# rapidsai/cuvs

Measured on AMD Instinct MI355X. Metric: QPS @ recall@10>=0.9, 100Mx128 fp32 IVF-PQ, batch=10k, higher is better.
Workload: dtype u8 codes, f16 LUT, f32 score; 1 GPU; IVF-PQ 100000000x128 fp32, pq_dim=64 pq_bits=8 n_lists=16384 n_probes=128 batch=10000 k=10; rows and held-out queries from bench.gen_rows (seed 1234 / 4321): Gaussian mixture of 65536 modes ~ N(0, I) in a 32-d latent space, spread 0.35 per mode, embedded in R^128 by a fixed random map + N(0, 0.03^2 I) - NOT SURVEY 8d's generator: the same step on that one is the top-level entry contract_corpus (--; parallelism=single GPU, lut_dtype=f16, internal_distance_dtype=f32

## Files before the change

### cuvs_amd/csrc/ivf_common.hpp

```cpp
#pragma once
#include "ops.hpp"
#include "device_utils.hpp"

#include <algorithm>
#include <functional>
#include <vector>

namespace cuvs_amd {
namespace {

struct work_item {
  uint32_t list;
  uint32_t first;
  uint32_t count;
  uint32_t pad;
};

__global__ __launch_bounds__(1024) void count_items_kernel(const uint32_t* __restrict__ pair_off, int n_lists,
                                                           int qpb_lo, uint32_t* __restrict__ item_off, int split,
                                                           int qpb_hi)
{
  __shared__ int smem[17];
  const int per = (n_lists + 1023) / 1024;
  const int b = threadIdx.x * per, e = min(n_lists, b + per);
  auto items_of = [&](int i) {
    const int qpb = i < split ? qpb_lo : qpb_hi;
    return ((int)(pair_off[i + 1] - pair_off[i]) + qpb - 1) / qpb;
  };
  int s = 0;
  for (int i = b; i < e; ++i) s += items_of(i);
  int total;
  int run = block_exclusive_scan(s, smem, &total);
  for (int i = b; i < e; ++i) {
    item_off[i] = (uint32_t)run;
    run += items_of(i);
  }
  if (threadIdx.x == 0) item_off[n_lists] = (uint32_t)total;
}

__global__ void fill_items_kernel(const uint32_t* __restrict__ pair_off, const uint32_t* __restrict__ item_off,
                                  int n_lists, int qpb_lo, work_item* __restrict__ items, int split, int qpb_hi)
{
  int L = blockIdx.x * blockDim.x + threadIdx.x;
  if (L >= n_lists) return;
  const int qpb = L < split ? qpb_lo : qpb_hi;
  uint32_t b = pair_off[L], e = pair_off[L + 1];
  uint32_t w = item_off[L];
  for (uint32_t p = b; p < e; p += qpb, ++w) {
    work_item it;
    it.list  = (uint32_t)L;
    it.first = p;
    it.count = min((uint32_t)qpb, e - p);
    it.pad   = 0;
    items[w] = it;
  }
}

__global__ void phase_labels_kernel(const uint32_t* __restrict__ probes, int64_t n_pairs, uint32_t n_probes,
                                    uint32_t head, uint32_t n_lists, uint32_t* __restrict__ out,
                                    uint32_t shard_world = 1, uint32_t shard_rank = 0, uint32_t skip = 0,
                                    const int32_t* __restrict__ owner = nullptr, bool head_in_tail = false)
{
  for (int64_t p = (int64_t)blockIdx.x * blockDim.x + threadIdx.x; p < n_pairs; p += (int64_t)gridDim.x * blockDim.x) {
    const uint32_t L = probes[p];
    const bool mine  = shard_world <= 1 || (owner != nullptr ? (uint32_t)owner[L] == shard_rank : L % shard_world == shard_rank);
    out[p] = !mine ? skip : L + ((((uint32_t)(p % n_probes) < head && !head_in_tail) || head == 0) ? 0u : n_lists);
  }
}

template <int E>
struct wave_top {
  float d[E];
  uint32_t i[E];
  __device__ inline void init()
  {
#pragma unroll
    for (int e = 0; e < E; ++e) { d[e] = INFINITY; i[e] = 0xffffffffu; }
  }
  __device__ inline float rank_d(int r) const
  {
    float v = 0.f;
#pragma unroll
    for (int e = 0; e < E; ++e)
      if ((r >> 6) == e) v = __uint_as_float(__builtin_amdgcn_readlane(__float_as_uint(d[e]), r & 63));
    return v;
  }
  __device__ inline uint32_t rank_i(int r) const
  {
    uint32_t v = 0;
#pragma unroll
    for (int e = 0; e < E; ++e)
      if ((r >> 6) == e) v = __builtin_amdgcn_readlane(i[e], r & 63);
    return v;
  }
  __device__ inline void insert(float cd, uint32_t ci, int lane)
  {
    int pos = 0;
#pragma unroll
    for (int e = 0; e < E; ++e) {
      bool le = (d[e] < cd) || (d[e] == cd && i[e] <= ci);
      pos += __popcll(__ballot(le));
    }
    uint32_t carry_d = 0, carry_i = 0;
#pragma unroll
    for (int e = 0; e < E; ++e) {
      const uint32_t du   = __float_as_uint(d[e]);
      const uint32_t up_d = (uint32_t)__builtin_amdgcn_update_dpp((int)carry_d, (int)du, 0x138, 0xf, 0xf, false);
      const uint32_t up_i = (uint32_t)__builtin_amdgcn_update_dpp((int)carry_i, (int)i[e], 0x138, 0xf, 0xf, false);
      carry_d = __builtin_amdgcn_readlane(du, 63);
      carry_i = __builtin_amdgcn_readlane(i[e], 63);
      const int rank = e * 64 + lane;
      if (rank > pos) { d[e] = __uint_as_float(up_d); i[e] = up_i; }
      else if (rank == pos) { d[e] = cd; i[e] = ci; }
    }
  }
};


__device__ inline void wave_sort64(float& d, uint32_t& i, const int lane)
{
#pragma unroll
  for (int k2 = 2; k2 <= 64; k2 <<= 1) {
#pragma unroll
    for (int j2 = k2 >> 1; j2 > 0; j2 >>= 1) {
      const float od    = __shfl_xor(d, j2, 64);
      const uint32_t oi = (uint32_t)__shfl_xor((int)i, j2, 64);
      const bool other_less = (od < d) || (od == d && oi < i);
      const bool same       = od == d && oi == i;
      const bool take_min   = ((lane & j2) == 0) == ((lane & k2) == 0);
      if (take_min ? other_less : (!other_less && !same)) { d = od; i = oi; }
    }
  }
}

__global__ void pair_segments_kernel(const uint32_t* __restrict__ probes, const uint32_t* __restrict__ list_sizes,
                                     int64_t nq, uint32_t n_probes, uint32_t* __restrict__ seg)
{
  const int64_t q = (int64_t)blockIdx.x * blockDim.x + threadIdx.x;
  if (q >= nq) return;
  uint32_t off = 0;
  for (uint32_t p = 0; p < n_probes; ++p) {
    seg[q * n_probes + p] = off;
    off += list_sizes[probes[q * n_probes + p]];
  }
}

inline size_t largest_lists_total(const std::vector<uint32_t>& sizes, uint32_t n_probes)
{
  std::vector<uint32_t> s(sizes);
  const size_t m = std::min<size_t>(n_probes, s.size());
  std::partial_sort(s.begin(), s.begin() + m, s.end(), std::greater<uint32_t>());
  size_t t = 0;
  for (size_t i = 0; i < m; ++i) t += s[i];
  return t;
}

constexpr int kSegCap = 2048;

__global__ __launch_bounds__(256) void pair_histogram_kernel(const uint32_t* __restrict__ labels, int64_t n, uint32_t* __restrict__ counts,
                                                             uint32_t n_plain, uint32_t n_labels)
{
  __shared__ uint32_t bulk;
  if (threadIdx.x == 0) bulk = 0u;
  __syncthreads();
  uint32_t mine = 0u;
  for (int64_t i = (int64_t)blockIdx.x * blockDim.x + threadIdx.x; i < n; i += (int64_t)gridDim.x * blockDim.x) {
    const uint32_t L = labels[i];
    if (L < n_plain) atomicAdd(&counts[L], 1u);
    else             ++mine;
  }
  if (n_plain >= n_labels) return;
  for (int o = 32; o > 0; o >>= 1) mine += __shfl_down(mine, o, 64);
  if ((threadIdx.x & 63) == 0 && mine != 0u) atomicAdd(&bulk, mine);
  __syncthreads();
  if (threadIdx.x == 0 && bulk != 0u) atomicAdd(&counts[n_plain], bulk);
}
__global__ __launch_bounds__(1024) void pair_scan_kernel(const uint32_t* __restrict__ counts, int n, uint32_t* __restrict__ offsets)
{
  __shared__ int smem[17];
  const int per = (n + 1023) / 1024;
  const int b = threadIdx.x * per, e = min(n, b + per);
  int s = 0;
  for (int i = b; i < e; ++i) s += (int)counts[i];
  int total;
  int run = block_exclusive_scan(s, smem, &total);
  for (int i = b; i < e; ++i) {
    const int c = (int)counts[i];
    offsets[i] = (uint32_t)run;
    run += c;
  }
  if (threadIdx.x == 0) offsets[n] = (uint32_t)total;
}
__global__ void pair_scatter_kernel(const uint32_t* __restrict__ labels, int64_t n, const uint32_t* __restrict__ offsets,
                                    uint32_t* __restrict__ cursor, uint32_t* __restrict__ out, uint32_t n_plain)
{
  const int64_t i = (int64_t)blockIdx.x * blockDim.x + threadIdx.x;
  if (i >= n) return;
  const uint32_t L = labels[i];
  if (L >= n_plain) return;
  out[offsets[L] + atomicAdd(&cursor[L], 1u)] = (uint32_t)i;
}
__global__ __launch_bounds__(256) void sort_segments_kernel(const uint32_t* __restrict__ offsets, uint32_t n_labels,
                                                            uint32_t* __restrict__ pairs)
{
  __shared__ uint32_t seg_all[4][kSegCap];
  const uint32_t L = blockIdx.x * 4u + (threadIdx.x >> 6);
  if (L >= n_labels) return;
  const int lane   = threadIdx.x & 63;
  const uint32_t b = offsets[L], n = offsets[L + 1] - b;
  if (n <= 1u || n > (uint32_t)kSegCap) return;
  uint32_t* seg = seg_all[threadIdx.x >> 6];
  for (uint32_t i = lane; i < n; i += 64u) seg[i] = pairs[b + i];
  __builtin_amdgcn_fence(__ATOMIC_ACQ_REL, "wavefront");
  __builtin_amdgcn_wave_barrier();
  for (uint32_t i = lane; i < n; i += 64u) {
    const uint32_t v = seg[i];
    uint32_t rank = 0u;
    for (uint32_t j = 0; j < n; ++j) rank += seg[j] < v ? 1u : 0u;
    pairs[b + rank] = v;
  }
}
constexpr uint32_t kBitmapQueries = 1u << 19;

__global__ __launch_bounds__(1024) void sort_big_segments_kernel(const uint32_t* __restrict__ offsets, uint32_t n_labels,
                                                                 uint32_t* __restrict__ pairs, uint32_t* __restrict__ tmp,
                                                                 uint32_t n_probes, uint32_t n_queries)
{
  extern __shared__ __attribute__((aligned(16))) uint32_t sb_smem[];
  __shared__ uint32_t big[1024];
  __shared__ uint32_t n_big;
  __shared__ int scan_smem[17];
  const bool bitmap_ok = n_probes != 0u && n_queries <= kBitmapQueries;
  const uint32_t words = (n_queries + 31u) / 32u;
  const uint32_t per = (n_labels + gridDim.x - 1) / gridDim.x;
  const uint32_t l0 = blockIdx.x * per, l1 = min(n_labels, l0 + per);
  for (uint32_t base = l0; base < l1; base += 1024u) {
    if (threadIdx.x == 0) n_big = 0u;
    __syncthreads();
    const uint32_t Lc = base + threadIdx.x;
    if (Lc < l1 && offsets[Lc + 1] - offsets[Lc] > (uint32_t)kSegCap) big[atomicAdd(&n_big, 1u)] = Lc;
    __syncthreads();
    const uint32_t nb = n_big;
    for (uint32_t w = 0; w < nb; ++w) {
      const uint32_t L = big[w];
      const uint32_t b = offsets[L], n = offsets[L + 1] - b;
      if (bitmap_ok) {
        uint32_t* bits = sb_smem;
        uint32_t* pref = sb_smem + words;
        for (uint32_t i = threadIdx.x; i < words; i += 1024u) bits[i] = 0u;
        __syncthreads();
        for (uint32_t i = threadIdx.x; i < n; i += 1024u) {
          const uint32_t q = pairs[b + i] / n_probes;
          atomicOr(&bits[q >> 5], 1u << (q & 31u));
        }
        __syncthreads();
        const uint32_t run = (words + 1023u) / 1024u, w0 = threadIdx.x * run, w1 = min(words, w0 + run);
        int sum = 0;
        for (uint32_t i = w0; i < w1; ++i) sum += __popc(bits[i]);
        int total;
        int acc = block_exclusive_scan(sum, scan_smem, &total);
        for (uint32_t i = w0; i < w1; ++i) { pref[i] = (uint32_t)acc; acc += __popc(bits[i]); }
        __syncthreads();
        for (uint32_t i = threadIdx.x; i < n; i += 1024u) {
          const uint32_t p = pairs[b + i], q = p / n_probes;
          tmp[b + pref[q >> 5] + (uint32_t)__popc(bits[q >> 5] & ((1u << (q & 31u)) - 1u))] = p;
        }
      } else {
        uint32_t* tile = sb_smem;
        for (uint32_t i0 = 0; i0 < n; i0 += 1024u) {
          const uint32_t i = i0 + threadIdx.x;
          const uint32_t v = i < n ? pairs[b + i] : 0xffffffffu;
          uint32_t rank = 0u;
          for (uint32_t t0 = 0; t0 < n; t0 += 4096u) {
            __syncthreads();
            for (uint32_t t = threadIdx.x; t < 4096u; t += 1024u) tile[t] = t0 + t < n ? pairs[b + t0 + t] : 0xffffffffu;
            __syncthreads();
            const uint32_t m = min(4096u, n - t0);
            for (uint32_t j = 0; j < m; ++j) rank += tile[j] < v ? 1u : 0u;
          }
          if (i < n) tmp[b + rank] = v;
        }
      }
      __syncthreads();
      for (uint32_t i = threadIdx.x; i < n; i += 1024u) pairs[b + i] = tmp[b + i];
      __syncthreads();
    }
    __syncthreads();
  }
}

inline void group_pairs(resources& res, const uint32_t* labels, int64_t n, uint32_t n_labels, uint32_t* sorted_pairs, uint32_t* pair_off,
                        uint32_t* cursor, uint32_t* tmp, uint32_t n_sorted, uint32_t n_probes, int64_t n_queries)
{
  CUVS_EXPECTS(n < (int64_t(1) << 32), "group_pairs: more than 2^32 pairs");
  HIP_TRY(hipMemsetAsync(cursor, 0, (size_t)n_labels * sizeof(uint32_t), res.stream));
  n_sorted = std::min(n_sorted, n_labels);
  CUVS_EXPECTS(n_sorted + 1u >= n_labels, "group_pairs: at most one bulk label");
  hipLaunchKernelGGL(pair_histogram_kernel, dim3((unsigned)std::min<int64_t>(grid_blocks(n, 256), 2048)), dim3(256), 0, res.stream, labels, n,
                     cursor, n_sorted, n_labels);
  hipLaunchKernelGGL(pair_scan_kernel, dim3(1), dim3(1024), 0, res.stream, cursor, (int)n_labels, pair_off);
  HIP_TRY(hipMemsetAsync(cursor, 0, (size_t)n_labels * sizeof(uint32_t), res.stream));
  hipLaunchKernelGGL(pair_scatter_kernel, dim3(grid_blocks(n, 256)), dim3(256), 0, res.stream, labels, n, pair_off, cursor, sorted_pairs, n_sorted);
  hipLaunchKernelGGL(sort_segments_kernel, dim3(grid_blocks(n_sorted, 4)), dim3(256), 0, res.stream, pair_off, n_sorted, sorted_pairs);
  const bool bitmap   = n_probes != 0u && n_queries <= (int64_t)kBitmapQueries;
  const size_t sbytes = bitmap ? (size_t)2 * ((n_queries + 31) / 32) * sizeof(uint32_t) : (size_t)4096 * sizeof(uint32_t);
  HIP_TRY(hipFuncSetAttribute(reinterpret_cast<const void*>(sort_big_segments_kernel), hipFuncAttributeMaxDynamicSharedMemorySize,
                              (int)std::max<size_t>(sbytes, 16384)));
  hipLaunchKernelGGL(sort_big_segments_kernel, dim3(64), dim3(1024), std::max<size_t>(sbytes, 16384), res.stream, pair_off, n_sorted,
                     sorted_pairs, tmp, n_probes, (uint32_t)std::min<int64_t>(n_queries, 0xffffffff));
  HIP_TRY(hipGetLastError());
}

inline void build_work_items(resources& res, const uint32_t* probes, int64_t n_pairs, uint32_t n_lists, int qpb,
                             uint32_t* sorted_pairs, uint32_t* pair_off, uint32_t* item_off, work_item* items,
                             int split = -1, int qpb_hi = 0, uint32_t* group_scratch = nullptr, uint32_t n_sorted = 0xffffffffu,
                             uint32_t n_probes = 0, int64_t n_queries = 0)
{
  if (split < 0) { split = (int)n_lists; qpb_hi = qpb; }
  if (group_scratch != nullptr)
    group_pairs(res, probes, n_pairs, n_lists, sorted_pairs, pair_off, group_scratch, group_scratch + n_lists + 1, n_sorted, n_probes, n_queries);
  else                          group_by_label(res, probes, n_pairs, n_lists, sorted_pairs, pair_off);
  const int n_item_labels = (int)std::min(n_lists, n_sorted);
  hipLaunchKernelGGL(count_items_kernel, dim3(1), dim3(1024), 0, res.stream, pair_off, n_item_labels, qpb, item_off,
                     split, qpb_hi);
  hipLaunchKernelGGL(fill_items_kernel, dim3(grid_blocks(n_item_labels, 256)), dim3(256), 0, res.stream, pair_off,
                     item_off, n_item_labels, qpb, items, split, qpb_hi);
}

}
template <int NT>
__device__ inline void merge_sorted_lists(float* __restrict__ d, uint32_t* __restrict__ id, const int n_l, const int kp2,
                                          const int tid)
{
  auto less = [](const float da, const uint32_t ia, const float db, const uint32_t ib) {
    return da < db || (da == db && ia < ib);
  };
  for (int w = 1; w < n_l; w <<= 1) {
    const int pairs = n_l / (2 * w);
    for (int t = tid; t < pairs * kp2; t += NT) {
      const int pr = t / kp2, r = t % kp2;
      const int ia = pr * 2 * w * kp2 + r, ib = (pr * 2 * w + w) * kp2 + (kp2 - 1 - r);
      const float da = d[ia], db = d[ib];
      const uint32_t xa = id[ia], xb = id[ib];
      if (less(db, xb, da, xa)) { d[ia] = db; id[ia] = xb; }
    }
    __syncthreads();
    for (int stride = kp2 >> 1; stride > 0; stride >>= 1) {
      for (int t = tid; t < pairs * (kp2 >> 1); t += NT) {
        const int pr = t / (kp2 >> 1), x = t % (kp2 >> 1);
        const int lo = pr * 2 * w * kp2 + 2 * x - (x & (stride - 1)), hi = lo + stride;
        const float da = d[lo], db = d[hi];
        const uint32_t xa = id[lo], xb = id[hi];
        if (less(db, xb, da, xa)) { d[lo] = db; id[lo] = xb; d[hi] = da; id[hi] = xa; }
      }
      __syncthreads();
    }
  }
}

}
```

### cuvs_amd/csrc/ivf_pq_filter4.hip

```cpp
#include "ivf_pq_filter_common.hpp"

#include <cfloat>
#include <type_traits>

namespace cuvs_amd {

namespace {

struct bprep_params {
  const uint32_t* sorted_pairs;
  const uint32_t* pair_off;
  uint32_t n_lists;
  uint32_t lbase;
  const uint32_t* probes;
  const float* rot_queries;
  const float* centers_rot;
  const uint32_t* query_kth;
  uint32_t* qflag;
  uint4* bq;
  float* thr;
  uint32_t n_probes, rot_dim;
  float sc, c1, eps, alpha, cbmax, dmax, bound_max;
  int is_ip, flat;
  uint32_t lpl;
  float4* norms;
};

template <int NST, int PART>
__global__ __launch_bounds__(256) void pq_bprep_kernel(const bprep_params a)
{
  constexpr uint32_t LPP = 2 * NST <= 2 ? 2u : 2 * NST <= 4 ? 4u : 2 * NST <= 8 ? 8u : 2 * NST <= 16 ? 16u : 32u;
  constexpr uint32_t PPW = 64u / LPP;
  const uint32_t s_base = a.pair_off[a.lbase], s_end = a.pair_off[a.lbase + a.n_lists];
  const uint32_t lane = threadIdx.x & 63u, slot = lane % LPP, st = slot >> 1, h = slot & 1u;
  const uint32_t w0 = (blockIdx.x * 4u + (threadIdx.x >> 6)) * 32u;
  if (s_base + w0 >= s_end) return;
  const uint32_t d0 = ((16u * (st >> a.lpl) + 8u * h) << a.lpl) + 8u * (st & ((1u << a.lpl) - 1u));
#pragma unroll 2
  for (uint32_t pass = 0; pass < 32u / PPW; ++pass) {
    const uint32_t s  = s_base + w0 + pass * PPW + lane / LPP;
    const bool pair_ok = s < s_end;
    const bool valid  = pair_ok && slot < 2u * NST;
    const uint32_t p  = a.sorted_pairs[pair_ok ? s : s_end - 1u];
    const uint32_t q  = p / a.n_probes, L = a.probes[p];
    float rn = 0.f, big = 0.f, qc = 0.f, cn = 0.f;
    if (valid) {
      const float* rq = a.rot_queries + (size_t)q * a.rot_dim + d0;
      const float* ct = a.centers_rot + (size_t)L * a.rot_dim + d0;
      const float4 q0 = *reinterpret_cast<const float4*>(rq), q1 = *reinterpret_cast<const float4*>(rq + 4);
      float r[8] = {q0.x, q0.y, q0.z, q0.w, q1.x, q1.y, q1.z, q1.w};
      const float4 c0 = *reinterpret_cast<const float4*>(ct), c1 = *reinterpret_cast<const float4*>(ct + 4);
      const float c[8] = {c0.x, c0.y, c0.z, c0.w, c1.x, c1.y, c1.z, c1.w};
      if (!a.is_ip) {
#pragma unroll
        for (int e = 0; e < 8; ++e) r[e] -= c[e];
      } else {
#pragma unroll
        for (int e = 0; e < 8; ++e) { qc = __fmaf_rn(r[e], c[e], qc); cn = __fmaf_rn(c[e], c[e], cn); }
      }
      f16x8_t v;
#pragma unroll
      for (int e = 0; e < 8; ++e) {
        rn   = __fmaf_rn(r[e], r[e], rn);
        const float x = a.sc * r[e];
        big  = fmaxf(big, fabsf(x));
        v[e] = (_Float16)fminf(fmaxf(x, -60000.f), 60000.f);
      }
      a.bq[(size_t)(s - s_base) * NST * 2 + slot] = __builtin_bit_cast(uint4, v);
    }
#pragma unroll
    for (uint32_t o = 1; o < LPP; o <<= 1) {
      rn += __shfl_xor(rn, o); qc += __shfl_xor(qc, o); cn += __shfl_xor(cn, o);
      big = fmaxf(big, __shfl_xor(big, o));
    }
    if (!pair_ok || slot != 0u) continue;
    if constexpr (PART == 1) {
      a.norms[s - s_base] = make_float4(rn, cn, qc, big);
    } else {
      const uint32_t kk = a.query_kth[q];
      const float bound = key_to_float(kk);
      const bool served = kk < 0xff800000u && big < 60000.f && fabsf(bound) <= a.bound_max;
      if (!a.flat && !served) a.qflag[q] = 1u;
      const float t = a.is_ip ? filter_threshold_ip(bound, rn, cn, qc, a) : filter_threshold(bound, rn, a);
      a.thr[s - s_base] = served ? t / a.c1 : (a.flat ? -INFINITY : INFINITY);
    }
  }
}

__global__ __launch_bounds__(256) void pq_thr_kernel(const bprep_params a)
{
  const uint32_t s_base = a.pair_off[a.lbase], s_end = a.pair_off[a.lbase + a.n_lists];
  const uint32_t s = s_base + blockIdx.x * 256u + threadIdx.x;
  if (s >= s_end) return;
  const uint32_t q  = a.sorted_pairs[s] / a.n_probes;
  const float4 nm   = a.norms[s - s_base];
  const float rn = nm.x, cn = nm.y, qc = nm.z, big = nm.w;
  const uint32_t kk = a.query_kth[q];
  const float bound = key_to_float(kk);
  const bool served = kk < 0xff800000u && big < 60000.f && fabsf(bound) <= a.bound_max;
  if (!a.flat && !served) a.qflag[q] = 1u;
  const float t = a.is_ip ? filter_threshold_ip(bound, rn, cn, qc, a) : filter_threshold(bound, rn, a);
  a.thr[s - s_base] = served ? t / a.c1 : (a.flat ? -INFINITY : INFINITY);
}

constexpr int kF4Threads = 256;
constexpr uint32_t kSurvChunk = 256u;

struct filter4_params {
  const filter_unit* units;
  const uint32_t* n_units;
  uint32_t* xcd_ticket;
  const uint32_t* sorted_pairs;
  const uint32_t* pair_off;
  uint32_t n_lists;
  const uint4* bq;
  const float* thr;
  const uint32_t* cb16;
  const uint8_t* codes;
  const uint32_t* list_offsets;
  const uint32_t* list_sizes;
  const float* row_term;
  uint32_t* qflag;
  uint2* surv;
  uint32_t* surv_cnt;
  uint32_t n_chunks, n_probes, unit_rows;
  unsigned long long* stats;
  uint32_t strided;
// ... 485 lines not shown
```

### cuvs_amd/csrc/ivf_pq_scan3.hip

```cpp
#include "ivf_pq.hpp"
#include "ops.hpp"
#include "device_utils.hpp"
#include "ivf_common.hpp"
#include "pq_lut_math.hpp"
#include "ivf_pq_scan3.hpp"
#include "ivf_pq_filter_common.hpp"

#include <cfloat>
#include <cmath>
#include <cstring>
#include <map>
#include <mutex>
#include <type_traits>
#include <utility>

namespace cuvs_amd {

namespace {

constexpr int kFThreads = 512;
constexpr int kFWaves   = kFThreads / 64;



// ... 3 lines not shown
  const uint32_t e = blockIdx.x * blockDim.x + threadIdx.x;
  if (e >= pq_dim * 256u) return;
  const uint32_t s = e >> 8, code = e & 255u;
  for (uint32_t l = 0; l < pq_len; ++l)
    cb16[(size_t)e * pq_len + l] =
      code < book ? __builtin_bit_cast(uint16_t, (_Float16)(sc * pq_centers[(size_t)(s * pq_len + l) * book + code])) : (uint16_t)0;
}

__global__ void cbt_kernel(const float* __restrict__ pq_centers, uint32_t pq_dim, uint32_t pq_len, uint32_t book, float* __restrict__ cbt)
{
  const uint32_t e = blockIdx.x * blockDim.x + threadIdx.x;
  if (e >= pq_dim * 256u) return;
  const uint32_t s = e >> 8, code = e & 255u;
  for (uint32_t l = 0; l < pq_len; ++l) cbt[(size_t)e * pq_len + l] = code < book ? pq_centers[(size_t)(s * pq_len + l) * book + code] : 0.f;
}

__global__ void expand_codes_kernel(const uint8_t* __restrict__ codes, int64_t rows, uint32_t n_chunks, uint32_t cpc, uint32_t bits,
                                    uint32_t pq_dim, uint8_t* __restrict__ out)
{
  const uint32_t nch8 = pq_dim / 16;
  const int64_t i = (int64_t)blockIdx.x * blockDim.x + threadIdx.x;
  if (i >= rows * nch8) return;
  const int64_t row = i / nch8;
  const uint32_t c8 = (uint32_t)(i % nch8);
  uint32_t w[4] = {0u, 0u, 0u, 0u};
#pragma unroll
  for (int b = 0; b < 16; ++b) {
    const uint32_t s = c8 * 16 + b, ch = s / cpc, bit = (s % cpc) * bits;
    const uint8_t* base = codes + ((size_t)(row >> 6) * n_chunks + ch) * 1024 + (size_t)(row & 63) * 16;
    uint32_t v = base[bit >> 3];
    if ((bit & 7) + bits > 8) v |= (uint32_t)base[(bit >> 3) + 1] << 8;
    w[b >> 2] |= ((v >> (bit & 7)) & ((1u << bits) - 1u)) << ((b & 3) * 8);
  }
  reinterpret_cast<uint4*>(out)[((size_t)(row >> 6) * nch8 + c8) * 64 + (row & 63)] = make_uint4(w[0], w[1], w[2], w[3]);
}

__device__ inline float wave_reduce_max_f32(float v)
{
#pragma unroll
  for (int off = 32; off > 0; off >>= 1) v = fmaxf(v, __shfl_xor(v, off));
  return v;
}

__global__ void row_term_kernel(const uint8_t* __restrict__ codes, const float* __restrict__ pq_centers, int64_t rows, float sc,
                                uint32_t* __restrict__ term, uint32_t* __restrict__ dn_max_bits, int n_chunks, int fp32, int pq_len,
                                uint32_t book, const uint32_t* __restrict__ list_offsets, uint32_t n_lists)
{
  const int64_t r0 = (int64_t)blockIdx.x * blockDim.x + threadIdx.x;
  const int64_t r  = min(r0, rows - 1);
  uint32_t L = 0u;
  if (list_offsets != nullptr) {
    uint32_t lo = 0u, hi = n_lists;
    while (hi - lo > 1u) {
      const uint32_t mid = (lo + hi) >> 1;
      if ((int64_t)list_offsets[mid] <= r) lo = mid; else hi = mid;
    }
    L = lo;
  }
  const uint4* cp = reinterpret_cast<const uint4*>(codes) + ((size_t)(r >> 6) * n_chunks) * 64 + (r & 63);
  float dn = 0.f;
  for (int c = 0; c < n_chunks; ++c) {
    const uint4 cw       = cp[c * 64];
    const uint32_t ws[4] = {cw.x, cw.y, cw.z, cw.w};
#pragma unroll
    for (int b = 0; b < 16; ++b) {
      const uint32_t code = (ws[b >> 2] >> ((b & 3) * 8)) & 0xffu;
      const uint32_t s    = c * 16 + b;
      for (int l = 0; l < pq_len; ++l) {
        const float p = pq_centers[(size_t)((list_offsets != nullptr ? L : s) * pq_len + l) * book + code];
        dn = __fmaf_rn(p, p, dn);
      }
    }
  }
  const float wmax = wave_reduce_max_f32(dn);
  if ((threadIdx.x & 63) == 0) atomicMax(dn_max_bits, __float_as_uint(wmax));
  const float x     = -0.5f * sc * sc * (dn * (1.0f - 1.0f / 512.0f));
  const _Float16 hi = (_Float16)x;
  const _Float16 lo = (_Float16)(x - (float)hi);
  if (r0 < rows)
    term[r] = fp32 ? __float_as_uint(x) : ((uint32_t)__builtin_bit_cast(uint16_t, hi) | ((uint32_t)__builtin_bit_cast(uint16_t, lo) << 16));
}


__global__ __launch_bounds__(1024) void count_units_kernel(const uint32_t* __restrict__ pair_off, uint32_t n_lists,
                                                           const uint32_t* __restrict__ list_sizes, uint32_t unit_rows,
                                                           uint32_t* __restrict__ unit_off, uint32_t group, uint32_t lbase)
{
  __shared__ int smem[17];
  const uint32_t per = (n_lists + 1023u) / 1024u;
  const uint32_t b = threadIdx.x * per, e = min(n_lists, b + per);
  auto units_of = [&](uint32_t i) {
    const uint32_t np = pair_off[lbase + i + 1] - pair_off[lbase + i];
    const uint32_t len = list_sizes[i];
    return (int)(((np + group - 1u) / group) * ((len + unit_rows - 1u) / unit_rows));
  };
  int s = 0;
  for (uint32_t i = b; i < e; ++i) s += units_of(i);
  int total;
  int run = block_exclusive_scan(s, smem, &total);
  for (uint32_t i = b; i < e; ++i) {
    unit_off[i] = (uint32_t)run;
    run += units_of(i);
  }
  if (threadIdx.x == 0) unit_off[n_lists] = (uint32_t)total;
}

__global__ void fill_units_kernel(const uint32_t* __restrict__ pair_off, uint32_t n_lists,
                                  const uint32_t* __restrict__ list_offsets, const uint32_t* __restrict__ list_sizes,
                                  uint32_t unit_rows, const uint32_t* __restrict__ unit_off, filter_unit* __restrict__ units,
                                  uint32_t group, uint32_t lbase)
{
  const uint32_t L = blockIdx.x * blockDim.x + threadIdx.x;
  if (L >= n_lists) return;
  const uint32_t b = pair_off[lbase + L], e = pair_off[lbase + L + 1], len = list_sizes[L];
  uint32_t w = unit_off[L];
  if (b == e || len == 0u) return;
  const uint32_t n_ch = (len + unit_rows - 1u) / unit_rows;
  const uint32_t rows = ((len + n_ch - 1u) / n_ch + 63u) & ~63u;
  const uint32_t base = list_offsets[L];
  for (uint32_t c = 0; c < n_ch; ++c) {
    const uint32_t r0 = c * rows, r1 = min(len, r0 + rows);
    if (r0 >= r1) continue;
    for (uint32_t p = b; p < e; p += group) units[w++] = filter_unit{L, p, min(group, e - p), r0, base, r1, 0u, 0u};
  }
  const uint32_t w_end = unit_off[L] + ((e - b + group - 1u) / group) * n_ch;
  for (; w < w_end; ++w) units[w] = filter_unit{L, b, 1u, 0u, base, 0u, 0u, 0u};
}

constexpr uint32_t kOrdWaves = 8u, kOrdThreads = 64u * kOrdWaves;
__global__ __launch_bounds__(512) __attribute__((amdgpu_waves_per_eu(6, 8))) void order_units_kernel(const filter_unit* __restrict__ in, const uint32_t* __restrict__ n_units,
                                                           filter_unit* __restrict__ out, uint32_t unit_rows, int order)
{
  __shared__ uint32_t cnt[kOrdWaves][kUnitKeys];
  __shared__ uint32_t head_pos[kOrdWaves];
  __shared__ int scan_smem[17];
  __shared__ uint32_t k_star_s;
  const uint32_t n = *n_units;
  const uint32_t lane = threadIdx.x & 63u, w = threadIdx.x >> 6;
  const uint32_t per = (n + kOrdWaves * 64u - 1u) / (kOrdWaves * 64u) * 64u;
  const uint32_t b = min(n, w * per), e = min(n, b + per);
  for (uint32_t i = threadIdx.x; i < kOrdWaves * kUnitKeys; i += kOrdThreads) (&cnt[0][0])[i] = 0u;
  if (threadIdx.x == 0) k_star_s = order == 1 ? kUnitKeys : 0u;
  __syncthreads();
  auto key_of = [&](const uint4 d0, const uint2 d1) {
    return unit_cost_key(d1.y > d0.w ? d1.y - d0.w : 0u, (d0.z + 31u) >> 5, unit_rows);
  };
  constexpr uint32_t kOrdAhead = 4u;
  static_assert(kUnitKeys <= kOrdThreads, "a thread per key in the scan of the costs");
  for (uint32_t i0 = b; i0 < e; i0 += 64u * kOrdAhead) {
    uint4 d0[kOrdAhead];
    uint2 d1[kOrdAhead];
#pragma unroll
    for (uint32_t j = 0; j < kOrdAhead; ++j) {
      const uint32_t i = min(i0 + j * 64u + lane, e - 1u);
      d0[j] = *reinterpret_cast<const uint4*>(in + i);
      d1[j] = *reinterpret_cast<const uint2*>(reinterpret_cast<const char*>(in + i) + 16);
    }
#pragma unroll
    for (uint32_t j = 0; j < kOrdAhead; ++j)
      if (i0 + j * 64u + lane < e) atomicAdd(&cnt[w][key_of(d0[j], d1[j])], 1u);
  }
  __syncthreads();
  {
    int v = 0;
    if (threadIdx.x < kUnitKeys)
      for (uint32_t ww = 0; ww < kOrdWaves; ++ww) v += (int)(cnt[ww][threadIdx.x] * threadIdx.x);
    if (n > (1u << 21)) v = 0;
    int total;
    const int below = block_exclusive_scan(v, scan_smem, &total);
    if (order == 2 && n <= (1u << 21) && threadIdx.x < kUnitKeys && (long long)below * 8 <= (long long)total)
      atomicMax(&k_star_s, threadIdx.x);
    __syncthreads();
  }
  const uint32_t k_star = k_star_s;
  {
    uint32_t s = 0;
    for (uint32_t key = lane; key < kUnitKeys; key += 64u) s += key >= k_star ? cnt[w][key] : 0u;
    for (uint32_t o = 32u; o > 0u; o >>= 1) s += __shfl_xor(s, o);
    if (lane == 0) head_pos[w] = s;
  }
  __syncthreads();
  {
    constexpr uint32_t kPer = (kOrdWaves + kOrdWaves * kUnitKeys + kOrdThreads - 1u) / kOrdThreads;
    uint32_t vals[kPer];
    int sum = 0;
#pragma unroll
// ... 1714 lines not shown

struct head_params {
  const work_item* items;
  const uint32_t* item_begin;
  const uint32_t* item_end;
  uint32_t n_lists;
  uint32_t* xcd_ticket;
  const uint32_t* sorted_pairs;
  const float* rot_queries;
  const float* centers_rot;
  const float* pq_centers;
  const uint8_t* codes;
  const uint32_t* list_offsets;
  const uint32_t* list_sizes;
  float* out_d;
  uint32_t* out_i;
  uint32_t* query_kth;
  uint32_t n_probes, rot_dim, k, cap_rows, pq_dim, n_chunks, pq_len, book;
  int is_ip, per_cluster;
  int hcand;
  uint32_t row_limit;
  uint32_t one_shot;
  const uint32_t* filter_bits;
  const int64_t* indices;
  unsigned long long* stats;
};

static inline int head_cand(int k) { return k <= 128 ? 512 : 1024; }

constexpr int kHeadRowsPerThread = 16;
constexpr int kHeadGroups16      = 2;

template <int B>
__device__ __forceinline__ uint32_t code_byte_x2(uint32_t w)
{
  uint32_t r;
  if constexpr (B == 0) asm("v_lshlrev_b32_sdwa %0, %1, %2 dst_sel:DWORD dst_unused:UNUSED_PAD src0_sel:DWORD src1_sel:BYTE_0" : "=v"(r) : "s"(1u), "v"(w));
  if constexpr (B == 1) asm("v_lshlrev_b32_sdwa %0, %1, %2 dst_sel:DWORD dst_unused:UNUSED_PAD src0_sel:DWORD src1_sel:BYTE_1" : "=v"(r) : "s"(1u), "v"(w));
  if constexpr (B == 2) asm("v_lshlrev_b32_sdwa %0, %1, %2 dst_sel:DWORD dst_unused:UNUSED_PAD src0_sel:DWORD src1_sel:BYTE_2" : "=v"(r) : "s"(1u), "v"(w));
  if constexpr (B == 3) asm("v_lshlrev_b32_sdwa %0, %1, %2 dst_sel:DWORD dst_unused:UNUSED_PAD src0_sel:DWORD src1_sel:BYTE_3" : "=v"(r) : "s"(1u), "v"(w));
  return r;
}

template <int LUT, bool ACC_HALF, int NT, int WPE>
__global__ __launch_bounds__(NT) __attribute__((amdgpu_waves_per_eu(WPE, WPE))) void pq_head_kernel(const head_params a)
{
  constexpr bool LUT32 = LUT == 0 || (LUT == 2 && !ACC_HALF);
  using lut_t = std::conditional_t<LUT32, float, _Float16>;
  extern __shared__ __attribute__((aligned(16))) char smem[];
  lut_t* lut      = reinterpret_cast<lut_t*>(smem);
  float* rv       = reinterpret_cast<float*>(smem + (size_t)a.pq_dim * 256 * sizeof(lut_t));
  float* cv       = rv + 256;
  unsigned long long* min64 = reinterpret_cast<unsigned long long*>(cv + 256);
  int* ctrl       = reinterpret_cast<int*>(min64 + 2);
  work_item& cur  = *reinterpret_cast<work_item*>(ctrl + 8);
  uint32_t* tk    = reinterpret_cast<uint32_t*>(ctrl + 12);
  const int kHCand = a.hcand;
  uint2* cand     = reinterpret_cast<uint2*>(tk + NT);
  static_assert(sizeof(work_item) == 16, "work_item");

  const int tid = threadIdx.x;
  const uint32_t item0   = (a.one_shot == 0u && a.item_begin) ? *a.item_begin : 0u;
  const uint32_t n_items = a.one_shot != 0u ? a.one_shot : *a.item_end - item0;
  const uint32_t xcd = blockIdx.x & 7u, chunk = (n_items + 7u) / 8u;
  const uint32_t share0 = min(n_items, xcd * chunk), share_len = min(chunk, n_items - share0);
  const work_item* share = a.items + item0 + share0;
  const uint4* codes16   = reinterpret_cast<const uint4*>(a.codes);
  float one = 1.0f;
  asm("" : "+s"(one));

  for (uint32_t round = 0;; ++round) {
    __syncthreads();
    if (tid == 0) {
      if (a.one_shot != 0u) {
        cur = (round == 0u && blockIdx.x < a.one_shot) ? a.items[blockIdx.x] : work_item{0u, 0u, 0u, 0xffffffffu};
      } else {
        const uint32_t t = atomicAdd(a.xcd_ticket + xcd * 32, 1u);
        cur = t < share_len ? share[t] : work_item{0u, 0u, 0u, 0xffffffffu};
      }
    }
    __syncthreads();
    const work_item item = cur;
    if (item.pad == 0xffffffffu) break;
    if (item.count == 0u) continue;
    unsigned long long t_prev = a.stats != nullptr ? __builtin_readcyclecounter() : 0ull;
    auto phase = [&](int which) {
      if (a.stats != nullptr && tid == 0) {
        const unsigned long long t = __builtin_readcyclecounter();
        atomicAdd(&a.stats[which], t - t_prev);
        t_prev = t;
      }
    };
    const uint32_t L        = item.list >= a.n_lists ? item.list - a.n_lists : item.list;
    const uint32_t base_row = a.list_offsets[L], len = a.row_limit != 0u ? min(a.list_sizes[L], a.row_limit) : a.list_sizes[L];
    const uint32_t pair     = a.sorted_pairs[item.first];
    const uint32_t q        = pair / a.n_probes;
    if (tid < (int)a.rot_dim) {
      const float c = a.centers_rot[(size_t)L * a.rot_dim + tid];
      float v       = a.rot_queries[(size_t)q * a.rot_dim + tid];
      if (!a.is_ip) v -= c;
      rv[tid] = v;
      cv[tid] = c;
    }
    __syncthreads();
    phase(0);
    constexpr int LB = 16;
#pragma unroll 1
    for (uint32_t e0 = tid; e0 < ((a.pq_len == 2u && !a.per_cluster) ? a.pq_dim * 256u : 0u); e0 += (uint32_t)LB * NT) {
      float p0[LB], p1[LB];
#pragma unroll
      for (int j = 0; j < LB; ++j) {
        const uint32_t e = min(e0 + (uint32_t)j * NT, a.pq_dim * 256u - 1u), sb = e >> 8, code = min(e & 255u, a.book - 1u);
        p0[j] = a.pq_centers[(size_t)(sb * 2 + 0) * a.book + code];
        p1[j] = a.pq_centers[(size_t)(sb * 2 + 1) * a.book + code];
      }
#pragma unroll
      for (int j = 0; j < LB; ++j) {
        const uint32_t e = e0 + (uint32_t)j * NT, sb = e >> 8;
        if (e >= a.pq_dim * 256u) break;
        const float q0 = rv[sb * 2], q1 = rv[sb * 2 + 1];
        float v;
        if (!a.is_ip) {
          const float d0 = q0 - p0[j], d1 = q1 - p1[j];
          v = __fmaf_rn(d1, d1, __fmaf_rn(d0, d0, 0.f));
        } else {
          v = __fmaf_rn(-q0, cv[sb * 2], 0.f);
          v = __fmaf_rn(-q0, p0[j], v);
          v = __fmaf_rn(-q1, cv[sb * 2 + 1], v);
          v = __fmaf_rn(-q1, p1[j], v);
        }
        if constexpr (LUT == 2) v = fp8_round_trip<std::conditional_t<ACC_HALF, __half, float>>(v, a.is_ip != 0);
        if constexpr (LUT32) lut[e] = v; else lut[e] = to_lut_half(v);
      }
    }
    if (a.pq_len != 2u || a.per_cluster) {
#pragma unroll 1
      for (uint32_t e0 = tid; e0 < a.pq_dim * 256u; e0 += 4u * NT) {
        float v[4] = {0.f, 0.f, 0.f, 0.f};
        for (uint32_t l = 0; l < a.pq_len; ++l) {
          float p[4];
#pragma unroll
          for (int j = 0; j < 4; ++j) {
            const uint32_t e = min(e0 + (uint32_t)j * NT, a.pq_dim * 256u - 1u), sb = e >> 8, code = min(e & 255u, a.book - 1u);
            p[j] = a.pq_centers[(size_t)((a.per_cluster ? L : sb) * a.pq_len + l) * a.book + code];
          }
#pragma unroll
          for (int j = 0; j < 4; ++j) {
            const uint32_t e = min(e0 + (uint32_t)j * NT, a.pq_dim * 256u - 1u), dd = (e >> 8) * a.pq_len + l;
            const float qv = rv[dd];
            if (!a.is_ip) {
              const float d = qv - p[j];
              v[j] = __fmaf_rn(d, d, v[j]);
            } else {
              v[j] = __fmaf_rn(-qv, cv[dd], v[j]);
              v[j] = __fmaf_rn(-qv, p[j], v[j]);
            }
          }
        }
#pragma unroll
        for (int j = 0; j < 4; ++j) {
          const uint32_t e = e0 + (uint32_t)j * NT;
          if (e >= a.pq_dim * 256u) break;
          float x = v[j];
          if constexpr (LUT == 2) x = fp8_round_trip<std::conditional_t<ACC_HALF, __half, float>>(x, a.is_ip != 0);
          if constexpr (LUT32) lut[e] = x; else lut[e] = to_lut_half(x);
        }
      }
    }
    if (tid == 0) ctrl[0] = 0;
    __syncthreads();
    phase(1);
    const int k = (int)a.k;
    int buf = 0;
    auto key_of = [&](uint32_t v) __attribute__((always_inline)) -> uint32_t {
      const uint32_t fr = base_row + v;
      const uint4* cp   = codes16 + ((size_t)(fr >> 6) * a.n_chunks) * 64 + (fr & 63u);
      float af    = 0.f;
      _Float16 ah = (_Float16)0.f;
// ... 379 lines not shown
}

bool pq3_bound_useful(const ivf_pq_index& idx, int k)
{
  uint64_t rows = 0, lists = 0;
  if (idx.shard_world > 1 && idx.shard_comm != nullptr) {
    if (!idx.shard_stats_valid) return k <= 128;
    rows = idx.shard_global_rows; lists = idx.shard_global_lists;
  } else {
    for (uint32_t v : idx.h_list_sizes) { rows += v; lists += v != 0u; }
  }
  return lists != 0 && (uint64_t)k * 25u * lists <= rows;
}

static std::recursive_mutex g_pq3_mu;

const uint8_t* pq3_codes(resources& res, const ivf_pq_index& idx, uint32_t* n_chunks)
{
  *n_chunks = idx.pq_dim / 16;
  if (idx.pq_bits == 8) return idx.codes.data();
  std::lock_guard<std::recursive_mutex> lock(g_pq3_mu);
  auto& c = idx.scan3;
  if (c.codes8_src != idx.codes.data() || c.codes8_rows != idx.padded_rows || c.codes8_size != idx.size) {
    const int64_t rows = std::max<int64_t>(idx.padded_rows, 1);
    c.codes8 = dev_buf<uint8_t>::persistent((size_t)rows * idx.pq_dim);
    if (idx.padded_rows > 0)
      hipLaunchKernelGGL(expand_codes_kernel, dim3(grid_blocks(idx.padded_rows * (int64_t)(idx.pq_dim / 16), 256)), dim3(256), 0, res.stream,
                         idx.codes.data(), idx.padded_rows, idx.n_chunks, idx.codes_per_chunk, idx.pq_bits, idx.pq_dim, c.codes8.data());
    c.codes8_src = idx.codes.data(); c.codes8_rows = idx.padded_rows; c.codes8_size = idx.size;
  }
  return c.codes8.data();
}

pq3_tables pq3_prepare(resources& res, const ivf_pq_index& idx, const bool term_fp32)
{
  std::lock_guard<std::recursive_mutex> lock(g_pq3_mu);
  auto& c = idx.scan3;
  if (c.codes_ptr != idx.codes.data() || c.rows != idx.padded_rows || c.size != idx.size || c.pq_ptr != idx.pq_centers.data() ||
      c.term_fp32 != term_fp32) {
    std::vector<float> h = to_host(res, idx.pq_centers.data(), idx.pq_centers.size());
    float mx = 0.f;
    for (float v : h) mx = std::max(mx, std::fabs(v));
    c.sc    = mx > 0.f ? std::exp2(std::floor(std::log2(16.0f / mx))) : 1.0f;
    c.cbmax = mx;
    const uint32_t n_tables = idx.codebook_kind == 0 ? idx.pq_dim : idx.n_lists;
    c.cb16  = dev_buf<uint32_t>::persistent((size_t)n_tables * 256 * idx.pq_len / 2 + 1);
    hipLaunchKernelGGL(cb16_kernel, dim3(grid_blocks((int64_t)n_tables * 256, 256)), dim3(256), 0, res.stream,
                       idx.pq_centers.data(), n_tables, idx.pq_len, idx.pq_book, c.sc, reinterpret_cast<uint16_t*>(c.cb16.data()));
    c.row_term = dev_buf<uint32_t>::persistent((size_t)std::max<int64_t>(idx.padded_rows, 1));
    dev_buf<uint32_t> mxd(res, 1);
    HIP_TRY(hipMemsetAsync(mxd.data(), 0, sizeof(uint32_t), res.stream));
    uint32_t nch8 = 0;
    const uint8_t* codes8 = pq3_codes(res, idx, &nch8);
    if (idx.padded_rows > 0)
      hipLaunchKernelGGL(row_term_kernel, dim3(grid_blocks(idx.padded_rows, 256)), dim3(256), 0, res.stream, codes8,
                         idx.pq_centers.data(), idx.padded_rows, c.sc, c.row_term.data(), mxd.data(), (int)nch8, term_fp32 ? 1 : 0,
                         (int)idx.pq_len, idx.pq_book, idx.codebook_kind == 0 ? nullptr : idx.list_offsets.data(), idx.n_lists);
    const uint32_t mbits = to_host(res, mxd.data(), 1)[0];
    float dn_max;
    memcpy(&dn_max, &mbits, 4);
    c.dmax = std::sqrt(dn_max) * 1.0001f;
    c.codes_ptr = idx.codes.data(); c.rows = idx.padded_rows; c.size = idx.size; c.pq_ptr = idx.pq_centers.data();
    c.term_fp32 = term_fp32;
  }
  return pq3_tables{c.cb16.data(), c.row_term.data(), c.sc, c.cbmax, c.dmax};
}

size_t pq3_max_units(const ivf_pq_index& idx, int64_t n_pairs, uint32_t* unit_rows, bool filter4)
{
  uint32_t max_len = 0;
  for (uint32_t v : idx.h_list_sizes) max_len = std::max(max_len, v);
  const uint32_t ur = std::max<uint32_t>(filter4 ? 8192u : 4096u, (uint32_t)round_up((int64_t)(max_len + 15) / 16, 64));
  *unit_rows = ur;
  return (size_t)16 * ((size_t)n_pairs / 32 + idx.n_lists + 1);
}

void pq3_warm(resources& res, const ivf_pq_index& idx, bool filter4)
{
  uint32_t n_chunks = 0;
  (void)pq3_codes(res, idx, &n_chunks);
  (void)pq3_prepare(res, idx, filter4);
}

void pq3_tail(resources& res, const ivf_pq_index& idx, const pq3_run& r)
{
  const bool f4 = r.bq != nullptr;
  CUVS_EXPECTS(r.stage == 0 || f4, "ivf_pq: the two-stream schedule is pq_filter4_kernel's");
  const pq3_tables tb = pq3_prepare(res, idx, f4);
  if (r.stage != 1) profile_begin(res, "pq_scan_kernel");
  const int nch        = (int)idx.pq_dim / 16;
  const int nst        = nch * (int)idx.pq_len;
  const uint32_t group = f4 ? (nst <= 8 ? 128u : 64u) : (nch <= 4 ? 64u : 32u);
  CUVS_EXPECTS(f4 || (idx.pq_len == 2 && idx.codebook_kind == 0), "ivf_pq: pq_filter_kernel decodes pq_len 2, PER_SUBSPACE only");
  auto* units = static_cast<filter_unit*>(r.units);
  if (r.stage != 2) {
    hipLaunchKernelGGL(count_units_kernel, dim3(1), dim3(1024), 0, res.stream, r.pair_off, idx.n_lists, idx.list_sizes.data(),
                       r.unit_rows, r.unit_off, group, idx.n_lists);
    hipLaunchKernelGGL(fill_units_kernel, dim3(grid_blocks(idx.n_lists, 256)), dim3(256), 0, res.stream, r.pair_off, idx.n_lists,
                       idx.list_offsets.data(), idx.list_sizes.data(), r.unit_rows, r.unit_off, units, group, idx.n_lists);
  }
  const bool ordered = r.unit_order != 0 && r.units_ord != nullptr;
  if (ordered) {
    if (r.stage != 2)
      hipLaunchKernelGGL(order_units_kernel, dim3(1), dim3(kOrdThreads), 0, res.stream, units, r.unit_off + idx.n_lists,
                         static_cast<filter_unit*>(r.units_ord), r.unit_rows, r.unit_order);
    units = static_cast<filter_unit*>(r.units_ord);
  }
  filter_params f{};
  f.units = units; f.n_units = r.unit_off + idx.n_lists; f.xcd_ticket = r.xcd_ticket; f.strided = ordered ? 1u : 0u;
  f.sorted_pairs = r.sorted_pairs; f.rot_queries = r.rot_queries; f.centers_rot = idx.centers_rot.data();
  uint32_t nch8 = 0;
  const uint8_t* codes8 = pq3_codes(res, idx, &nch8);
  f.cb16 = tb.cb16; f.codes = codes8; f.list_offsets = idx.list_offsets.data(); f.list_sizes = idx.list_sizes.data();
  f.row_term = r.is_ip ? nullptr : tb.row_term; f.query_kth = r.query_kth; f.qflag = r.qflag;
  const unsigned grid = pq3_grid(res);
  const unsigned regions = grid;
  f.surv = static_cast<uint2*>(r.surv); f.surv_cnt = r.surv_cnt; f.surv_cap = (uint32_t)((uint64_t)r.surv_cap * 3 / 4 / regions);
  f.spill_cap = r.surv_cap - f.surv_cap * regions;
  f.n_probes = r.n_probes; f.rot_dim = idx.rot_dim; f.unit_rows = r.unit_rows;
  f.sc = tb.sc; f.c1 = (r.is_ip ? -1.0f : -2.0f) / (tb.sc * tb.sc);
  f.cbmax = tb.cbmax; f.dmax = tb.dmax; f.is_ip = r.is_ip; f.stats = r.stats; f.dbg = r.filter_dbg;
  f.bound_max = FLT_MAX;
  const float ne = std::max(1.0f, (float)idx.pq_dim / 64.0f);
  if (r.lut_mode == 0)      { f.eps = ne / 65536.0f; f.alpha = 0.f; }
  else if (r.lut_mode == 1) { f.eps = r.acc_half ? 0.04f * ne : 1.0f / 1024.0f; f.alpha = ne * 64.0f / 16777216.0f; f.bound_max = 60000.f; }
  else                      { f.eps = r.acc_half ? 0.07f + 0.04f * ne : 0.07f; f.alpha = ne * 64.0f / 32768.0f; f.bound_max = 30000.f; }
  if (r.is_ip && r.lut_mode == 2) f.eps = r.acc_half ? 0.14f + 0.04f * ne : 0.14f;
  const size_t fsmem = (size_t)nch * 16 * 1024 + 16;
  if (f4) {
    filter4_launch l{};
    l.units = units; l.n_units = f.n_units; l.xcd_ticket = r.xcd_ticket; l.sorted_pairs = r.sorted_pairs; l.pair_off = r.pair_off;
    l.n_lists = idx.n_lists; l.probes = r.probes; l.rot_queries = r.rot_queries; l.centers_rot = f.centers_rot;
    l.query_kth = r.query_kth; l.qflag = r.qflag; l.bq = r.bq; l.thr = r.thr; l.cb16 = tb.cb16; l.codes = f.codes;
    l.list_offsets = f.list_offsets; l.list_sizes = f.list_sizes; l.row_term = reinterpret_cast<const float*>(f.row_term);
    l.surv = f.surv; l.surv_cnt = f.surv_cnt; l.surv_entries = r.surv_cap; l.n_probes = r.n_probes;
    l.rot_dim = idx.rot_dim; l.unit_rows = r.unit_rows; l.sc = f.sc; l.c1 = f.c1; l.eps = f.eps; l.alpha = f.alpha;
    l.cbmax = f.cbmax; l.dmax = f.dmax; l.bound_max = f.bound_max; l.is_ip = r.is_ip; l.dbg = r.filter_dbg; l.nch = nch;
    l.pl = (int)idx.pq_len; l.per_cluster = idx.codebook_kind != 0 ? 1 : 0;
    l.n_pairs = r.nq * (int64_t)r.n_probes; l.stats = r.stats; l.grid = grid;
    l.stage = r.stage; l.pair_norms = r.pair_norms; l.strided = ordered ? 1 : 0;
    pq4_filter(res, l);
    if (r.stage == 1) return;
  } else {
  auto launch_filter = [&](auto kern) {
    HIP_TRY(hipFuncSetAttribute(reinterpret_cast<const void*>(kern), hipFuncAttributeMaxDynamicSharedMemorySize, (int)fsmem));
    profile_begin(res, "pq_filter_kernel");
    hipLaunchKernelGGL(kern, dim3(grid), dim3(kFThreads), fsmem, res.stream, f);
    profile_end(res, "pq_filter_kernel");
  };
  if (nch == 4) {
    switch (r.filter_dbg) {
      case 1:  launch_filter(pq_filter_kernel<4, 1>); break;
      case 2:  launch_filter(pq_filter_kernel<4, 2>); break;
      case 4:  launch_filter(pq_filter_kernel<4, 4>); break;
      default: launch_filter(pq_filter_kernel<4, 0>); break;
    }
  } else {
    switch (nch) {
      case 1: launch_filter(pq_filter_kernel<1, 0>); break;
      case 2: launch_filter(pq_filter_kernel<2, 0>); break;
      case 3: launch_filter(pq_filter_kernel<3, 0>); break;
      case 5: launch_filter(pq_filter_kernel<5, 0>); break;
      case 6: launch_filter(pq_filter_kernel<6, 0>); break;
      case 7: launch_filter(pq_filter_kernel<7, 0>); break;
      default: launch_filter(pq_filter_kernel<8, 0>); break;
    }
  }
  }

  rescore_params s{};
  s.surv = f.surv; s.surv_cnt = r.surv_cnt; s.surv_cap = f.surv_cap; s.spill_cap = f.spill_cap; s.probes = r.probes; s.rot_queries = r.rot_queries;
  s.n_regions = regions; s.sub = f4 ? 0u : 1u;
  if (f4) s.surv_cap = r.surv_cap;
  s.centers_rot = idx.centers_rot.data(); s.pq_centers = idx.pq_centers.data(); s.codes = codes8;
  s.query_kth = r.query_kth; s.qflag = r.qflag; s.qcnt = r.qcnt; s.cand_d = r.cand_d; s.cand_i = r.cand_i; s.cand_r = r.cand_r;
  s.n_probes = r.n_probes; s.rot_dim = idx.rot_dim; s.k = r.k; s.head = r.head; s.is_ip = r.is_ip; s.n_chunks = nch8;
  s.head_rows = r.head_rows; s.list_offsets = idx.list_offsets.data();
  s.filter_bits = r.filter_bits; s.indices = idx.indices.data();
  s.overflow = static_cast<uint4*>(r.overflow); s.overflow_cnt = r.counters + 1; s.overflow_cap = r.overflow_cap; s.fail = nullptr;
  const size_t cb_bytes = (size_t)idx.rot_dim * idx.pq_book * sizeof(float);
  s.pq_len = idx.pq_len; s.book = idx.pq_book; s.per_cluster = idx.codebook_kind != 0 ? 1 : 0;
  s.cb_lds = (cb_bytes <= 128 * 1024 && !s.per_cluster) ? 1 : 0;
  const size_t rsmem = s.cb_lds ? cb_bytes : 16;
  const dim3 rg(f4 && s.cb_lds ? grid : grid + 1, f4 && s.cb_lds ? 1 : 2), rb(kRThreads);
  profile_begin(res, "pq_rescore_kernel");
  auto launch_rescore = [&](auto kern) {
    HIP_TRY(hipFuncSetAttribute(reinterpret_cast<const void*>(kern), hipFuncAttributeMaxDynamicSharedMemorySize, (int)rsmem));
    hipLaunchKernelGGL(kern, rg, rb, rsmem, res.stream, s);
  };
  auto pick_rescore = [&](auto lut_tag, auto acc_tag) {
    constexpr int LUT = decltype(lut_tag)::value;
    constexpr bool ACC = decltype(acc_tag)::value;
    if (s.cb_lds) launch_rescore(pq_rescore_kernel<LUT, ACC, true>); else launch_rescore(pq_rescore_kernel<LUT, ACC, false>);
  };
  using L0 = std::integral_constant<int, 0>; using L1 = std::integral_constant<int, 1>; using L2 = std::integral_constant<int, 2>;
  if (r.lut_mode == 0)      pick_rescore(L0{}, std::false_type{});
  else if (r.lut_mode == 1) { if (r.acc_half) pick_rescore(L1{}, std::true_type{}); else pick_rescore(L1{}, std::false_type{}); }
  else                      { if (r.acc_half) pick_rescore(L2{}, std::true_type{}); else pick_rescore(L2{}, std::false_type{}); }
  profile_end(res, "pq_rescore_kernel");
  hipLaunchKernelGGL(reset_flagged_kernel, dim3((unsigned)r.nq), dim3(256), 0, res.stream, r.qflag, r.nq, r.n_probes, r.k, r.head,
                     r.cand_d, r.cand_i);
  hipLaunchKernelGGL(fallback_items_kernel, dim3(grid * 4), dim3(256), 0, res.stream, r.sorted_pairs, r.pair_off, idx.n_lists,
                     r.probes, r.n_probes, r.qflag, static_cast<work_item*>(r.fb_items), r.counters, 0);
  profile_end(res, "pq_scan_kernel");
}

static size_t head_smem_fixed(const ivf_pq_index& idx, int lut_mode, bool acc_half, int nt, int k)
{
  const bool lut32 = lut_mode == 0 || (lut_mode == 2 && !acc_half);
  return (size_t)idx.pq_dim * 256 * (lut32 ? 4 : 2) + 2 * 256 * 4 + 16 + 32 + 16 + (size_t)nt * 4 + 4 * (size_t)head_cand(k) * 4;
}

static int head_occupancy(const void* fn, int nt, size_t smem)
{
  static std::mutex mu;
  static std::map<std::pair<const void*, size_t>, int> known;
  std::lock_guard<std::mutex> lock(mu);
  auto it = known.find({fn, smem});
  if (it != known.end()) return it->second;
  hipFuncAttributes fa{};
  HIP_TRY(hipFuncGetAttributes(&fa, fn));
  CUVS_EXPECTS(fa.sharedSizeBytes == 0, "ivf_pq: the head kernel's LUT has to sit at LDS address 0");
  int n = 0;
  HIP_TRY(hipOccupancyMaxActiveBlocksPerMultiprocessor(&n, fn, nt, smem));
  CUVS_EXPECTS(n >= 1, "ivf_pq: the head kernel does not fit a CU");
  known[{fn, smem}] = n;
  return n;
}

int pq3_head_scan(resources& res, const ivf_pq_index& idx, const pq3_head& h)
{
  head_params a{};
  a.items = static_cast<const work_item*>(h.items); a.item_begin = h.item_begin; a.item_end = h.item_end; a.n_lists = idx.n_lists;
  a.xcd_ticket = h.xcd_ticket; a.sorted_pairs = h.sorted_pairs; a.rot_queries = h.rot_queries; a.centers_rot = idx.centers_rot.data();
  a.pq_centers = idx.pq_centers.data(); a.codes = pq3_codes(res, idx, &a.n_chunks); a.list_offsets = idx.list_offsets.data();
  a.list_sizes = idx.list_sizes.data(); a.out_d = h.cand_d; a.out_i = h.cand_i; a.query_kth = h.query_kth;
  a.n_probes = h.n_probes; a.rot_dim = idx.rot_dim; a.k = h.k; a.is_ip = h.is_ip; a.pq_dim = idx.pq_dim;
  a.pq_len = idx.pq_len; a.book = idx.pq_book; a.per_cluster = idx.codebook_kind != 0 ? 1 : 0;
  a.filter_bits = h.filter_bits; a.indices = idx.indices.data(); a.stats = h.stats; a.hcand = head_cand((int)h.k);
  const bool lut32 = h.lut_mode == 0 || (h.lut_mode == 2 && !h.acc_half);
  const size_t lut_bytes = (size_t)idx.pq_dim * 256 * (lut32 ? 4 : 2);
  const bool nt512 = lut_bytes <= 64 * 1024;
  const int nt = nt512 ? 512 : 1024;
  const size_t smem = head_smem_fixed(idx, h.lut_mode, h.acc_half != 0, nt, (int)h.k);
  CUVS_EXPECTS(smem <= 160 * 1024 - 64, "ivf_pq: the head-phase LUT does not fit the LDS");
  a.cap_rows = (uint32_t)(kHeadRowsPerThread * nt);
  if (h.max_list_len > 0) a.cap_rows = std::min<uint32_t>(a.cap_rows, (uint32_t)round_up(h.max_list_len, 64));
  a.one_shot          = h.one_shot;
  a.row_limit         = h.row_limit;
  int wgs_per_cu = 0;
  auto go = [&](auto kern) {
    const void* fn = reinterpret_cast<const void*>(kern);
    HIP_TRY(hipFuncSetAttribute(fn, hipFuncAttributeMaxDynamicSharedMemorySize, (int)smem));
    wgs_per_cu = head_occupancy(fn, nt, smem);
    const unsigned grid = h.one_shot != 0u ? h.one_shot : pq3_grid(res) * (unsigned)wgs_per_cu;
    profile_begin(res, "pq_scan_kernel");
    profile_begin(res, "pq_head_kernel");
    hipLaunchKernelGGL(kern, dim3(grid), dim3(nt), smem, res.stream, a);
    profile_end(res, "pq_head_kernel");
    profile_end(res, "pq_scan_kernel");
  };
  auto pick = [&](auto lut_tag, auto acc_tag) {
    constexpr int LUT = decltype(lut_tag)::value;
    constexpr bool ACC = decltype(acc_tag)::value;
    constexpr bool L32 = LUT == 0 || (LUT == 2 && !ACC);
    if (nt512) go(pq_head_kernel<LUT, ACC, 512, L32 ? 4 : 6>); else go(pq_head_kernel<LUT, ACC, 1024, 4>);
  };
  using I0 = std::integral_constant<int, 0>; using I1 = std::integral_constant<int, 1>; using I2 = std::integral_constant<int, 2>;
  if (h.lut_mode == 0)      pick(I0{}, std::false_type{});
  else if (h.lut_mode == 1) { if (h.acc_half) pick(I1{}, std::true_type{}); else pick(I1{}, std::false_type{}); }
  else                      { if (h.acc_half) pick(I2{}, std::true_type{}); else pick(I2{}, std::false_type{}); }
  return wgs_per_cu;
}

bool flat3_wide(uint32_t dim) { return dim > 128 && pqw_shape(dim); }
bool flat3_supported(uint32_t dim, int k) { return ((dim % 32 == 0 && dim >= 32 && dim <= 256) || flat3_wide(dim)) && k <= 128; }

static bool flat3_prepare(resources& res, const flat3_view& v, flat3_cache& c)
{
  static std::mutex mu;
  std::lock_guard<std::mutex> lock(mu);
  if (c.data_ptr == v.data && c.rows == v.padded_rows && c.size == v.size) return true;
  if (c.failed_ptr == v.data && c.failed_rows == v.padded_rows && c.failed_size == v.size) return false;
  const int64_t rows = std::max<int64_t>(v.padded_rows, 64);
  {
    c.rows16   = dev_buf<uint4>();
    c.row_term = dev_buf<uint32_t>();
    c.data_ptr = nullptr;
    size_t free_b = 0, total_b = 0;
    HIP_TRY(hipMemGetInfo(&free_b, &total_b));
    const size_t need = (size_t)rows * v.dim * 2 + (size_t)rows * 16 + (size_t(1) << 30);
    if (free_b < need) {
      scratch_cache_flush_all();
      HIP_TRY(hipMemGetInfo(&free_b, &total_b));
    }
    if (free_b < need) {
      c.failed_ptr = v.data; c.failed_rows = v.padded_rows; c.failed_size = v.size;
      return false;
    }
  }
  dev_buf<uint32_t> row_list(res, (size_t)rows / 64), mxd(res, 2);
  dev_buf<float> dn(res, (size_t)rows), inv_norm(res, v.unit_rows ? (size_t)rows : 0);
  HIP_TRY(hipMemsetAsync(row_list.data(), 0xff, row_list.bytes(), res.stream));
  HIP_TRY(hipMemsetAsync(mxd.data(), 0, 2 * sizeof(uint32_t), res.stream));
  hipLaunchKernelGGL(flat_group_lists_kernel, dim3(v.n_lists), dim3(64), 0, res.stream, v.list_offsets, v.list_sizes, v.n_lists,
                     row_list.data());
  c.rows16   = dev_buf<uint4>::persistent((size_t)rows / 32 * (v.dim / 16) * 64);
  c.row_term = dev_buf<uint32_t>::persistent((size_t)rows);
  const bool wide = flat3_wide(v.dim);
  c.row_term32 = wide ? dev_buf<float>::persistent((size_t)rows) : dev_buf<float>();
  c.zeros      = wide ? dev_buf<float>::persistent(32) : dev_buf<float>();
  if (wide) HIP_TRY(hipMemsetAsync(c.zeros.data(), 0, 32 * sizeof(float), res.stream));
  if (v.padded_rows > 0) {
    auto stats = [&](auto kern) {
      hipLaunchKernelGGL(kern, dim3(grid_blocks(v.padded_rows, 256)), dim3(256), 0, res.stream, v.data, v.centers, row_list.data(),
                         v.padded_rows, v.dim, v.n_chunks, dn.data(), mxd.data(), inv_norm.data());
    };
    switch (v.elem) {
      case 0: stats(flat_residual_stats_kernel<float>); break;
      case 1: stats(flat_residual_stats_kernel<__half>); break;
      case 2: stats(flat_residual_stats_kernel<int8_t>); break;
      default: stats(flat_residual_stats_kernel<uint8_t>); break;
    }
    const auto mbits = to_host(res, mxd.data(), 2);
    float mx, mn2;
    memcpy(&mx, &mbits[0], 4);
    memcpy(&mn2, &mbits[1], 4);
    c.maxnorm = std::sqrt(mn2) * (1.0f + 1e-6f);
    c.maxres = mx;
    c.sc     = mx > 0.f ? std::exp2(std::floor(std::log2(16.0f / mx))) : 1.0f;
    const int64_t n_t = v.padded_rows / 32 * (v.dim / 16) * 64;
    auto rows16 = [&](auto kern) {
      hipLaunchKernelGGL(kern, dim3(grid_blocks(n_t, 256)), dim3(256), 0, res.stream, v.data, v.centers, row_list.data(), dn.data(),
                         v.padded_rows, v.dim, v.n_chunks, c.sc, c.rows16.data(), c.row_term.data(), inv_norm.data(), wide ? 1 : 0,
                         wide ? c.row_term32.data() : nullptr);
    };
    switch (v.elem) {
      case 0: rows16(flat_rows16_kernel<float>); break;
      case 1: rows16(flat_rows16_kernel<__half>); break;
      case 2: rows16(flat_rows16_kernel<int8_t>); break;
      default: rows16(flat_rows16_kernel<uint8_t>); break;
    }
  }
  sync(res);
  c.data_ptr = v.data; c.rows = v.padded_rows; c.size = v.size;
  return true;
}

bool flat3_head_bounds(resources& res, const flat3_view& v, flat3_cache& cache, const pq3_run& r, const flat3_head_bufs& hb)
{
  if (!flat3_prepare(res, v, cache)) return false;
  CUVS_EXPECTS(v.dim <= 128 && r.bq != nullptr && !r.is_ip, "ivf_flat: the bound-only head phase serves L2 up to 128 dimensions");
  profile_begin(res, "ivf_flat_scan_kernel");
  profile_begin(res, "flat_head_kernel");
  const float c1 = -2.0f / (cache.sc * cache.sc);
  hipLaunchKernelGGL(fill_f32_kernel, dim3(1024), dim3(256), 0, res.stream, hb.xbuf, (size_t)r.nq * hb.ldx, -INFINITY);
  filter4_launch l{};
  l.sorted_pairs = r.sorted_pairs; l.pair_off = r.pair_off; l.n_lists = v.n_lists; l.probes = r.probes;
  l.rot_queries = r.rot_queries; l.centers_rot = v.centers; l.query_kth = r.query_kth; l.qflag = r.qflag;
  l.bq = r.bq; l.thr = hb.thr_head; l.n_probes = r.n_probes; l.rot_dim = v.dim;
  l.sc = cache.sc; l.c1 = c1; l.eps = 1.0f / 65536.0f; l.alpha = 0.f; l.cbmax = cache.maxres; l.dmax = 0.f; l.bound_max = FLT_MAX;
  l.is_ip = 0; l.nch = (int)v.dim / 32; l.pl = 2; l.n_pairs = r.nq; l.flat = 1; l.head_labels = 1; l.stage = 1; l.pair_norms = hb.norms;
  pq4_filter(res, l);
  auto* units = static_cast<filter_unit*>(r.units);
  hipLaunchKernelGGL(count_units_kernel, dim3(1), dim3(1024), 0, res.stream, r.pair_off, v.n_lists, v.list_sizes, r.unit_rows, r.unit_off,
                     256u, 0u);
  hipLaunchKernelGGL(fill_units_kernel, dim3(grid_blocks(v.n_lists, 256)), dim3(256), 0, res.stream, r.pair_off, v.n_lists, v.list_offsets,
                     v.list_sizes, r.unit_rows, r.unit_off, units, 256u, 0u);
  filter_params f{};
  f.units = units; f.n_units = r.unit_off + v.n_lists; f.xcd_ticket = hb.tickets; f.sorted_pairs = r.sorted_pairs;
  f.list_offsets = v.list_offsets; f.list_sizes = v.list_sizes; f.row_term = cache.row_term.data(); f.rows16 = cache.rows16.data();
  f.bq = static_cast<const uint4*>(r.bq); f.pair_off = r.pair_off; f.n_lists = v.n_lists; f.lbase = 0u; f.xbuf = hb.xbuf; f.ldx = hb.ldx;
  f.n_probes = r.n_probes; f.rot_dim = v.dim; f.sc = cache.sc; f.c1 = c1;
  const unsigned grid = 2 * pq3_grid(res);
  auto launch_emit = [&](auto kern) {
    const size_t fsmem = (size_t)8 * (v.dim / 16) * 1024 + 2 * 8 * 32 * 4 + 16;
    HIP_TRY(hipFuncSetAttribute(reinterpret_cast<const void*>(kern), hipFuncAttributeMaxDynamicSharedMemorySize, (int)fsmem));
    hipLaunchKernelGGL(kern, dim3(grid), dim3(kF2Threads), fsmem, res.stream, f);
  };
  switch (v.dim / 16) {
    case 2:  launch_emit(flat_filter2_kernel<2, true>); break;
    case 4:  launch_emit(flat_filter2_kernel<4, true>); break;
    case 6:  launch_emit(flat_filter2_kernel<6, true>); break;
    default: launch_emit(flat_filter2_kernel<8, true>); break;
  }
  select_k<uint32_t, uint32_t>(res, hb.xbuf, nullptr, r.nq, (int64_t)hb.ldx, (int64_t)hb.ldx, (int)r.k, hb.kth_val, hb.kth_idx, false);
  head_bound_params b{};
  b.kth_val = hb.kth_val; b.kth_idx = hb.kth_idx; b.norms = static_cast<const float4*>(hb.norms); b.sorted_pairs = r.sorted_pairs;
  b.pair_off = r.pair_off; b.probes = r.probes; b.list_offsets = v.list_offsets; b.data = v.data;
  b.queries = r.rescore_queries != nullptr ? r.rescore_queries : r.rot_queries;
  b.n_lists = v.n_lists; b.n_probes = r.n_probes; b.k = r.k; b.dim = v.dim; b.n_chunks = v.n_chunks;
  b.sc = cache.sc; b.eps = l.eps; b.alpha = l.alpha; b.cbmax = cache.maxres; b.c1 = c1; b.rot_dim = v.dim;
  b.query_kth = const_cast<uint32_t*>(r.query_kth); b.thr_head = hb.thr_head; b.bound_max = FLT_MAX;
  const dim3 bgrid((unsigned)grid_blocks(r.nq, 4));
  switch (v.elem) {
    case 0: hipLaunchKernelGGL(flat_head_bound_kernel<float>, bgrid, dim3(256), 0, res.stream, b); break;
    case 1: hipLaunchKernelGGL(flat_head_bound_kernel<__half>, bgrid, dim3(256), 0, res.stream, b); break;
    case 2: hipLaunchKernelGGL(flat_head_bound_kernel<int8_t>, bgrid, dim3(256), 0, res.stream, b); break;
    default: hipLaunchKernelGGL(flat_head_bound_kernel<uint8_t>, bgrid, dim3(256), 0, res.stream, b); break;
  }
  profile_end(res, "flat_head_kernel");
  profile_end(res, "ivf_flat_scan_kernel");
  HIP_TRY(hipGetLastError());
  return true;
}

bool flat3_tail(resources& res, const flat3_view& v, flat3_cache& cache, const pq3_run& r)
{
  if (!flat3_prepare(res, v, cache)) return false;
  profile_begin(res, "ivf_flat_scan_kernel");
  const int nch        = (int)v.dim / 32;
  const bool f2        = res.tune.flat_filter2 != 0 && r.bq != nullptr && v.dim <= 128;
  const bool wide      = flat3_wide(v.dim);
  CUVS_EXPECTS(!wide || r.bq != nullptr, "ivf_flat: the wide filter needs the pre-pass buffers");
  const uint32_t group = wide ? pqw_group() : f2 ? 256u : (nch <= 4 ? 64u : 32u);
  auto* units = static_cast<filter_unit*>(r.units);
  hipLaunchKernelGGL(count_units_kernel, dim3(1), dim3(1024), 0, res.stream, r.pair_off, v.n_lists, v.list_sizes, r.unit_rows, r.unit_off,
                     group, v.n_lists);
  hipLaunchKernelGGL(fill_units_kernel, dim3(grid_blocks(v.n_lists, 256)), dim3(256), 0, res.stream, r.pair_off, v.n_lists, v.list_offsets,
                     v.list_sizes, r.unit_rows, r.unit_off, units, group, v.n_lists);
  const unsigned grid = (f2 && !wide) ? 2 * pq3_grid(res) : pq3_grid(res);
  filter_params f{};
  f.units = units; f.n_units = r.unit_off + v.n_lists; f.xcd_ticket = r.xcd_ticket;
  f.sorted_pairs = r.sorted_pairs; f.rot_queries = r.rot_queries; f.centers_rot = v.centers;
  f.codes = v.data; f.list_offsets = v.list_offsets; f.list_sizes = v.list_sizes;
  f.row_term = r.is_ip ? nullptr : cache.row_term.data(); f.query_kth = r.query_kth; f.qflag = r.qflag;
  f.surv = static_cast<uint2*>(r.surv); f.surv_cnt = r.surv_cnt; f.surv_cap = (uint32_t)((uint64_t)r.surv_cap * 3 / 4 / grid);
  f.spill_cap = r.surv_cap - f.surv_cap * grid;
  f.n_probes = r.n_probes; f.rot_dim = v.dim; f.unit_rows = r.unit_rows;
  f.sc = cache.sc; f.c1 = (r.is_ip ? -1.0f : -2.0f) / (cache.sc * cache.sc); f.cbmax = cache.maxres; f.dmax = r.is_ip ? cache.maxnorm : 0.f;
  f.is_ip = r.is_ip; f.stats = r.stats; f.dbg = r.filter_dbg;
  f.eps = 1.0f / 65536.0f; f.alpha = 0.f; f.bound_max = FLT_MAX;
  if (r.is_ip) f.eps = (float)v.dim * (1.0f / 4194304.0f);
  f.rows16 = cache.rows16.data(); f.fail = r.fail;
  auto launch_filter = [&](auto kern) {
    profile_begin(res, "flat_filter_kernel");
    hipLaunchKernelGGL(kern, dim3(grid), dim3(kFThreads), 16, res.stream, f);
    profile_end(res, "flat_filter_kernel");
  };
  auto launch_filter2 = [&](auto kern) {
    const size_t fsmem = (size_t)8 * (v.dim / 16) * 1024 + 2 * 8 * 32 * 4 + 16;
    HIP_TRY(hipFuncSetAttribute(reinterpret_cast<const void*>(kern), hipFuncAttributeMaxDynamicSharedMemorySize, (int)fsmem));
    profile_begin(res, "flat_filter_kernel");
    hipLaunchKernelGGL(kern, dim3(grid), dim3(kF2Threads), fsmem, res.stream, f);
    profile_end(res, "flat_filter_kernel");
  };
  if (wide) {
    dev_buf<uint32_t> blk_off(res, (size_t)v.n_lists + 1);
    wide_prep l{};
    l.sorted_pairs = r.sorted_pairs; l.pair_off = r.pair_off; l.n_lists = v.n_lists; l.probes = r.probes; l.rot_queries = r.rot_queries;
    l.centers_rot = v.centers; l.query_kth = r.query_kth; l.qflag = r.qflag; l.bq = r.bq; l.blk_off = blk_off.data(); l.thr = r.thr;
    l.norms = nullptr; l.n_probes = r.n_probes; l.rot_dim = v.dim; l.heads = r.head; l.sc = f.sc; l.c1 = f.c1; l.eps = f.eps; l.alpha = f.alpha;
    l.cbmax = f.cbmax; l.dmax = f.dmax; l.bound_max = f.bound_max; l.head = 0; l.is_ip = r.is_ip; l.flat = 1;
    l.n_pairs = r.nq * (int64_t)r.n_probes;
    pqw_bprep(res, l);
    wide_filter w{};
    w.units = units; w.n_units = f.n_units; w.xcd_ticket = r.xcd_ticket; w.sorted_pairs = r.sorted_pairs; w.pair_off = r.pair_off;
    w.n_lists = v.n_lists; w.bq = r.bq; w.blk_off = blk_off.data(); w.thr = r.thr; w.rows16 = cache.rows16.data();
    w.row_term = r.is_ip ? nullptr : cache.row_term32.data(); w.zeros = cache.zeros.data(); w.filter_bits = nullptr; w.indices = nullptr;
    w.qflag = r.qflag; w.surv = f.surv; w.surv_cnt = r.surv_cnt; w.surv_cap = f.surv_cap; w.spill_cap = f.spill_cap; w.n_probes = r.n_probes;
    w.rot_dim = v.dim; w.xbuf = nullptr; w.ldx = 0; w.heads = r.head; w.emit = 0; w.grid = grid; w.stats = r.stats; w.fail = r.fail;
    w.profile_name = "flat_filter_kernel";
    pqw_filter(res, w);
  } else if (f2) {
    filter4_launch l{};
    l.sorted_pairs = r.sorted_pairs; l.pair_off = r.pair_off; l.n_lists = v.n_lists; l.probes = r.probes;
    l.rot_queries = r.rot_queries; l.centers_rot = v.centers; l.query_kth = r.query_kth; l.qflag = r.qflag;
    l.bq = r.bq; l.thr = r.thr; l.n_probes = r.n_probes; l.rot_dim = v.dim;
    l.sc = f.sc; l.c1 = f.c1; l.eps = f.eps; l.alpha = f.alpha; l.cbmax = f.cbmax; l.dmax = f.dmax; l.bound_max = f.bound_max;
    l.is_ip = r.is_ip; l.nch = (int)v.dim / 32; l.pl = 2; l.n_pairs = r.nq * (int64_t)r.n_probes; l.flat = 1; l.bprep_only = 1;
    pq4_filter(res, l);
    f.bq = static_cast<const uint4*>(r.bq); f.thr_pair = r.thr; f.pair_off = r.pair_off; f.n_lists = v.n_lists;
    switch (v.dim / 16) {
      case 2:  launch_filter2(flat_filter2_kernel<2>); break;
      case 4:  launch_filter2(flat_filter2_kernel<4>); break;
      case 6:  launch_filter2(flat_filter2_kernel<6>); break;
      default: launch_filter2(flat_filter2_kernel<8>); break;
    }
  } else
  switch (nch) {
    case 1: launch_filter(pq_filter_kernel<1, 0, true>); break;
    case 2: launch_filter(pq_filter_kernel<2, 0, true>); break;
    case 3: launch_filter(pq_filter_kernel<3, 0, true>); break;
    case 4: launch_filter(pq_filter_kernel<4, 0, true>); break;
    case 5: launch_filter(pq_filter_kernel<5, 0, true>); break;
    case 6: launch_filter(pq_filter_kernel<6, 0, true>); break;
    case 7: launch_filter(pq_filter_kernel<7, 0, true>); break;
    default: launch_filter(pq_filter_kernel<8, 0, true>); break;
  }
  if (r.hb_xbuf != nullptr)
    hipLaunchKernelGGL(flat_head_survivors_kernel, dim3((unsigned)grid_blocks(r.nq, 4)), dim3(256), 0, res.stream, r.hb_xbuf, r.hb_ldx, r.hb_thr,
                       r.sorted_pairs, r.pair_off, v.n_lists, r.probes, v.list_offsets, v.list_sizes,
                       f.surv, r.surv_cnt, grid, f.surv_cap, f.spill_cap, r.fail);
  rescore_params s{};
  s.surv = f.surv; s.surv_cnt = r.surv_cnt; s.surv_cap = f.surv_cap; s.spill_cap = f.spill_cap; s.probes = r.probes;
  s.n_regions = grid; s.sub = 1;
  s.rot_queries = r.rescore_queries != nullptr ? r.rescore_queries : r.rot_queries; s.codes = v.data; s.query_kth = r.query_kth; s.qflag = r.qflag; s.qcnt = r.qcnt;
  s.cand_d = r.cand_d; s.cand_i = r.cand_i; s.cand_r = r.cand_r; s.n_probes = r.n_probes; s.k = r.k; s.head = r.head;
  s.n_chunks = v.n_chunks; s.dim = v.dim; s.filter_bits = r.filter_bits; s.indices = v.indices; s.is_ip = r.cosine ? 2 : r.is_ip;
  s.overflow = static_cast<uint4*>(r.overflow); s.overflow_cnt = r.counters + 1; s.overflow_cap = r.overflow_cap; s.fail = r.fail;
// ... 20 lines not shown
  uint64_t rows = 0, lists = 0;
  for (uint32_t v : idx.h_list_sizes) { rows += v; lists += v != 0u; }
  if (lists == 0 || rows == 0) return 0u;
  const uint64_t h = std::max<uint64_t>(1, ((uint64_t)40 * (uint64_t)k * lists + rows - 1) / rows);
  return 2 * h <= n_probes ? (uint32_t)h : 0u;
}

static void pqw_margins(const ivf_pq_index& idx, const pq3_run& r, float* eps, float* alpha, float* bound_max)
{
  const float ne = std::max(1.0f, (float)idx.pq_dim / 64.0f) * std::max(1.0f, (float)idx.pq_len / 8.0f);
  *bound_max = FLT_MAX;
  if (r.lut_mode == 0)      { *eps = ne / 65536.0f; *alpha = 0.f; }
  else if (r.lut_mode == 1) { *eps = r.acc_half ? 0.04f * ne : 1.0f / 1024.0f; *alpha = ne * 64.0f / 16777216.0f; *bound_max = 60000.f; }
  else                      { *eps = r.acc_half ? 0.07f + 0.04f * ne : 0.07f; *alpha = ne * 64.0f / 32768.0f; *bound_max = 30000.f; }
  if (r.is_ip && r.lut_mode == 2) *eps = r.acc_half ? 0.14f + 0.04f * ne : 0.14f;
}

static const void* pqw_rows(resources& res, const ivf_pq_index& idx, pq3_tables* tb_out)
{
  std::lock_guard<std::recursive_mutex> lock(g_pq3_mu);
  const pq3_tables tb = pq3_prepare(res, idx, true);
  if (tb_out != nullptr) *tb_out = tb;
  auto& c = idx.scan3;
  if (c.w_codes == idx.codes.data() && c.w_rows == idx.padded_rows && c.w_size == idx.size && c.w_pq == idx.pq_centers.data())
    return c.rows16w.data();
  if (c.w_failed_codes == idx.codes.data() && c.w_failed_rows == idx.padded_rows && c.w_failed_size == idx.size) return nullptr;
  c.rows16w = dev_buf<uint4>();
  c.w_codes = nullptr;
  const int64_t rows = std::max<int64_t>(idx.padded_rows, 64);
  size_t free_b = 0, total_b = 0;
  HIP_TRY(hipMemGetInfo(&free_b, &total_b));
  const size_t need = (size_t)rows * idx.rot_dim * 2 + (size_t(1) << 30);
  if (free_b < need) {
    scratch_cache_flush_all();
    HIP_TRY(hipMemGetInfo(&free_b, &total_b));
  }
  if (free_b < need) {
    c.w_failed_codes = idx.codes.data(); c.w_failed_rows = idx.padded_rows; c.w_failed_size = idx.size;
    return nullptr;
  }
  c.rows16w = dev_buf<uint4>::persistent((size_t)rows * idx.rot_dim / 8);
  c.cbt     = dev_buf<float>::persistent((size_t)idx.pq_dim * 256 * idx.pq_len);
  c.zeros   = dev_buf<float>::persistent(32);
  HIP_TRY(hipMemsetAsync(c.zeros.data(), 0, 32 * sizeof(float), res.stream));
  hipLaunchKernelGGL(cbt_kernel, dim3(grid_blocks((int64_t)idx.pq_dim * 256, 256)), dim3(256), 0, res.stream, idx.pq_centers.data(), idx.pq_dim,
                     idx.pq_len, idx.pq_book, c.cbt.data());
  uint32_t nch8 = 0;
  const uint8_t* codes8 = pq3_codes(res, idx, &nch8);
  pqw_decode(res, codes8, nch8, tb.cb16, idx.pq_len, idx.padded_rows, idx.rot_dim, c.rows16w.data());
  sync(res);
  c.w_codes = idx.codes.data(); c.w_rows = idx.padded_rows; c.w_size = idx.size; c.w_pq = idx.pq_centers.data();
  return c.rows16w.data();
}

bool pqw_ready(resources& res, const ivf_pq_index& idx) { return pqw_rows(res, idx, nullptr) != nullptr; }

static rescore_params pqw_score_inputs(const ivf_pq_index& idx, const pq3_run& r, const uint8_t* codes8, uint32_t nch8)
{
  rescore_params s{};
  s.probes = r.probes; s.rot_queries = r.rot_queries; s.centers_rot = idx.centers_rot.data(); s.pq_centers = idx.pq_centers.data();
  s.codes = codes8; s.n_chunks = nch8; s.rot_dim = idx.rot_dim; s.pq_len = idx.pq_len; s.book = idx.pq_book; s.per_cluster = 0;
  s.is_ip = r.is_ip; s.n_probes = r.n_probes; s.k = r.k; s.head = r.head; s.cbt = idx.scan3.cbt.data();
  return s;
}

bool pqw_head_bounds(resources& res, const ivf_pq_index& idx, const pq3_run& r, const pqw_bufs& hb)
{
  pq3_tables tb{};
  const void* rows16 = pqw_rows(res, idx, &tb);
  if (rows16 == nullptr) return false;
  profile_begin(res, "pq_scan_kernel");
  profile_begin(res, "pq_head_kernel");
  const float c1 = (r.is_ip ? -1.0f : -2.0f) / (tb.sc * tb.sc);
  float eps = 0.f, alpha = 0.f, bound_max = FLT_MAX;
  pqw_margins(idx, r, &eps, &alpha, &bound_max);
  hipLaunchKernelGGL(fill_f32_kernel, dim3(1024), dim3(256), 0, res.stream, hb.xbuf, (size_t)r.nq * r.head * hb.ldx, -INFINITY);
  wide_prep l{};
  l.sorted_pairs = r.sorted_pairs; l.pair_off = r.pair_off; l.n_lists = idx.n_lists; l.probes = r.probes; l.rot_queries = r.rot_queries;
  l.centers_rot = idx.centers_rot.data(); l.query_kth = r.query_kth; l.qflag = r.qflag; l.bq = r.bq; l.thr = hb.head_c; l.norms = hb.norms;
  l.n_probes = r.n_probes; l.rot_dim = idx.rot_dim; l.heads = r.head; l.sc = tb.sc; l.c1 = c1; l.eps = eps; l.alpha = alpha;
  l.cbmax = tb.cbmax; l.dmax = tb.dmax; l.bound_max = bound_max; l.head = 1; l.n_pairs = r.nq * (int64_t)r.head; l.blk_off = hb.blk_off; l.is_ip = r.is_ip;
  pqw_bprep(res, l);
  auto* units = static_cast<filter_unit*>(r.units);
  hipLaunchKernelGGL(count_units_kernel, dim3(1), dim3(1024), 0, res.stream, r.pair_off, idx.n_lists, idx.list_sizes.data(), r.unit_rows,
                     r.unit_off, pqw_group(), 0u);
  hipLaunchKernelGGL(fill_units_kernel, dim3(grid_blocks(idx.n_lists, 256)), dim3(256), 0, res.stream, r.pair_off, idx.n_lists,
                     idx.list_offsets.data(), idx.list_sizes.data(), r.unit_rows, r.unit_off, units, pqw_group(), 0u);
  wide_filter f{};
  f.units = units; f.n_units = r.unit_off + idx.n_lists; f.xcd_ticket = hb.tickets; f.sorted_pairs = r.sorted_pairs; f.pair_off = r.pair_off;
  f.n_lists = idx.n_lists; f.bq = r.bq; f.blk_off = hb.blk_off; f.thr = hb.head_c; f.rows16 = rows16;
  f.row_term = r.is_ip ? nullptr : reinterpret_cast<const float*>(tb.row_term); f.zeros = idx.scan3.zeros.data();
  f.qflag = r.qflag; f.surv = r.surv; f.surv_cnt = r.surv_cnt; f.surv_cap = 0; f.spill_cap = 0; f.n_probes = r.n_probes; f.rot_dim = idx.rot_dim;
  f.xbuf = hb.xbuf; f.ldx = hb.ldx; f.heads = r.head; f.emit = 1; f.grid = pq3_grid(res); f.stats = nullptr;
  f.filter_bits = r.filter_bits; f.indices = idx.indices.data();
  pqw_filter(res, f);
  select_k<uint32_t, uint32_t>(res, hb.xbuf, nullptr, r.nq, (int64_t)r.head * hb.ldx, (int64_t)r.head * hb.ldx, (int)r.k, hb.kth_val, hb.kth_idx,
                               false);
  uint32_t nch8 = 0;
  const uint8_t* codes8 = pq3_codes(res, idx, &nch8);
  wbound_params b{};
  b.rs = pqw_score_inputs(idx, r, codes8, nch8);
  b.kth_val = hb.kth_val; b.kth_idx = hb.kth_idx; b.norms = static_cast<const float4*>(hb.norms); b.probes = r.probes;
  b.list_offsets = idx.list_offsets.data(); b.nq = r.nq; b.k = r.k; b.heads = r.head; b.ldx = hb.ldx; b.n_probes = r.n_probes;
  b.rot_dim = idx.rot_dim; b.query_kth = const_cast<uint32_t*>(r.query_kth); b.qflag = r.qflag; b.thr_head = hb.thr_head;
  b.sc = tb.sc; b.c1 = c1; b.eps = eps; b.alpha = alpha; b.cbmax = tb.cbmax; b.dmax = tb.dmax; b.bound_max = bound_max; b.is_ip = r.is_ip;
  const dim3 bgrid((unsigned)grid_blocks(r.nq, 4));
  const bool bblocks = idx.pq_len == 2 && idx.pq_dim % 64 == 0 && res.tune.pq_wide_blocks != 0 && hb.bound_tmp != nullptr;
  auto bound = [&](auto lut_tag, auto acc_tag) {
    constexpr int LUT = decltype(lut_tag)::value;
    constexpr bool ACC = decltype(acc_tag)::value;
    if (bblocks) {
      HIP_TRY(hipMemsetAsync(hb.bound_tmp, 0, (size_t)2 * r.nq * sizeof(uint32_t), res.stream));
      const size_t smb = (size_t)64 * 2 * idx.pq_book * sizeof(float);
      auto kb = pqw_bound_blocks_kernel<LUT, ACC>;
      HIP_TRY(hipFuncSetAttribute(reinterpret_cast<const void*>(kb), hipFuncAttributeMaxDynamicSharedMemorySize, (int)smb));
      const unsigned gb = (unsigned)std::min<int64_t>(pq3_grid(res), grid_blocks(r.nq * (int64_t)r.k, kRBThreads * kRBItems));
      hipLaunchKernelGGL(kb, dim3(gb), dim3(kRBThreads), smb, res.stream, b, hb.bound_tmp);
      hipLaunchKernelGGL(pqw_bound_finish_kernel, bgrid, dim3(256), 0, res.stream, b, hb.bound_tmp);
      return;
    }
    const size_t sm = 4 * wave_score_tile<LUT, ACC>::kBytes;
    auto kern = pqw_head_bound_kernel<LUT, ACC>;
    HIP_TRY(hipFuncSetAttribute(reinterpret_cast<const void*>(kern), hipFuncAttributeMaxDynamicSharedMemorySize, (int)sm));
    hipLaunchKernelGGL(kern, bgrid, dim3(256), sm, res.stream, b);
  };
  using B0 = std::integral_constant<int, 0>; using B1 = std::integral_constant<int, 1>; using B2 = std::integral_constant<int, 2>;
  if (r.lut_mode == 0)      bound(B0{}, std::false_type{});
  else if (r.lut_mode == 1) { if (r.acc_half) bound(B1{}, std::true_type{}); else bound(B1{}, std::false_type{}); }
  else                      { if (r.acc_half) bound(B2{}, std::true_type{}); else bound(B2{}, std::false_type{}); }
  profile_end(res, "pq_head_kernel");
  profile_end(res, "pq_scan_kernel");
  HIP_TRY(hipGetLastError());
  return true;
}

void pqw_tail(resources& res, const ivf_pq_index& idx, const pq3_run& r, const pqw_bufs& hb)
{
  pq3_tables tb{};
  const void* rows16 = pqw_rows(res, idx, &tb);
  CUVS_EXPECTS(rows16 != nullptr, "ivf_pq: the wide path's decoded rows are gone between the head and the tail phase");
  profile_begin(res, "pq_scan_kernel");
  const float c1 = (r.is_ip ? -1.0f : -2.0f) / (tb.sc * tb.sc);
  float eps = 0.f, alpha = 0.f, bound_max = FLT_MAX;
  pqw_margins(idx, r, &eps, &alpha, &bound_max);
  wide_prep l{};
  l.sorted_pairs = r.sorted_pairs; l.pair_off = r.pair_off; l.n_lists = idx.n_lists; l.probes = r.probes; l.rot_queries = r.rot_queries;
  l.centers_rot = idx.centers_rot.data(); l.query_kth = r.query_kth; l.qflag = r.qflag; l.bq = r.bq; l.thr = r.thr; l.norms = nullptr;
  l.n_probes = r.n_probes; l.rot_dim = idx.rot_dim; l.heads = r.head; l.sc = tb.sc; l.c1 = c1; l.eps = eps; l.alpha = alpha;
  l.cbmax = tb.cbmax; l.dmax = tb.dmax; l.bound_max = bound_max; l.head = 0; l.n_pairs = r.nq * (int64_t)r.n_probes; l.blk_off = hb.blk_off; l.is_ip = r.is_ip;
  profile_begin(res, "pq_bprep_kernel");
  pqw_bprep(res, l);
  profile_end(res, "pq_bprep_kernel");
  auto* units = static_cast<filter_unit*>(r.units);
  hipLaunchKernelGGL(count_units_kernel, dim3(1), dim3(1024), 0, res.stream, r.pair_off, idx.n_lists, idx.list_sizes.data(), r.unit_rows,
                     r.unit_off, pqw_group(), idx.n_lists);
  hipLaunchKernelGGL(fill_units_kernel, dim3(grid_blocks(idx.n_lists, 256)), dim3(256), 0, res.stream, r.pair_off, idx.n_lists,
                     idx.list_offsets.data(), idx.list_sizes.data(), r.unit_rows, r.unit_off, units, pqw_group(), idx.n_lists);
  const unsigned grid = pq3_grid(res);
  wide_filter f{};
  f.units = units; f.n_units = r.unit_off + idx.n_lists; f.xcd_ticket = r.xcd_ticket; f.sorted_pairs = r.sorted_pairs; f.pair_off = r.pair_off;
  f.n_lists = idx.n_lists; f.bq = r.bq; f.blk_off = hb.blk_off; f.thr = r.thr; f.rows16 = rows16;
  f.row_term = r.is_ip ? nullptr : reinterpret_cast<const float*>(tb.row_term); f.zeros = idx.scan3.zeros.data();
  f.qflag = r.qflag; f.surv = r.surv; f.surv_cnt = r.surv_cnt; f.surv_cap = (uint32_t)((uint64_t)r.surv_cap * 3 / 4 / grid);
  f.spill_cap = r.surv_cap - f.surv_cap * grid; f.n_probes = r.n_probes; f.rot_dim = idx.rot_dim; f.xbuf = nullptr; f.ldx = 0; f.heads = r.head;
  f.emit = 0; f.grid = grid; f.stats = r.stats;
  pqw_filter(res, f);
  hipLaunchKernelGGL(pqw_head_survivors_kernel, dim3((unsigned)grid_blocks(r.nq * (int64_t)r.head, 4)), dim3(256), 0, res.stream, hb.xbuf, hb.ldx,
                     hb.thr_head, r.head, r.sorted_pairs, r.pair_off, idx.n_lists, r.probes, r.n_probes, idx.list_offsets.data(),
                     idx.list_sizes.data(), static_cast<uint2*>(r.surv), r.surv_cnt, grid, f.surv_cap, f.spill_cap, r.qflag);
  uint32_t nch8 = 0;
  const uint8_t* codes8 = pq3_codes(res, idx, &nch8);
  rescore_params s = pqw_score_inputs(idx, r, codes8, nch8);
  s.surv = static_cast<const uint2*>(r.surv); s.surv_cnt = r.surv_cnt; s.surv_cap = f.surv_cap; s.spill_cap = f.spill_cap;
  s.n_regions = grid; s.sub = 1u;
  s.query_kth = r.query_kth; s.qflag = r.qflag; s.qcnt = r.qcnt; s.cand_d = r.cand_d; s.cand_i = r.cand_i; s.cand_r = r.cand_r;
  s.head_rows = 0u; s.list_offsets = idx.list_offsets.data(); s.filter_bits = r.filter_bits; s.indices = idx.indices.data();
  s.overflow = static_cast<uint4*>(r.overflow); s.overflow_cnt = r.counters + 1; s.overflow_cap = r.overflow_cap; s.fail = nullptr;
  s.cb_lds = 0;
  const dim3 rg(grid, 8), rb(256);
  profile_begin(res, "pq_rescore_kernel");
  const bool blocks = idx.pq_len == 2 && idx.pq_dim % 64 == 0 && res.tune.pq_wide_blocks != 0;
  auto rescore = [&](auto lut_tag, auto acc_tag) {
    constexpr int LUT = decltype(lut_tag)::value;
    constexpr bool ACC = decltype(acc_tag)::value;
    if (blocks) {
      const size_t sm = (size_t)64 * 2 * idx.pq_book * sizeof(float) + ((size_t)grid + 3) * sizeof(uint32_t);
      auto kern = pq_rescore_blocks_kernel<LUT, ACC>;
      HIP_TRY(hipFuncSetAttribute(reinterpret_cast<const void*>(kern), hipFuncAttributeMaxDynamicSharedMemorySize, (int)sm));
      hipLaunchKernelGGL(kern, dim3(grid), dim3(kRBThreads), sm, res.stream, s);
      return;
    }
    const size_t sm = 4 * wave_score_tile<LUT, ACC>::kBytes + ((size_t)grid + 3) * sizeof(uint32_t);
    auto kern = pq_rescore_wave_kernel<LUT, ACC>;
    HIP_TRY(hipFuncSetAttribute(reinterpret_cast<const void*>(kern), hipFuncAttributeMaxDynamicSharedMemorySize, (int)sm));
    hipLaunchKernelGGL(kern, rg, rb, sm, res.stream, s);
  };
  using R0 = std::integral_constant<int, 0>; using R1 = std::integral_constant<int, 1>; using R2 = std::integral_constant<int, 2>;
  if (r.lut_mode == 0)      rescore(R0{}, std::false_type{});
  else if (r.lut_mode == 1) { if (r.acc_half) rescore(R1{}, std::true_type{}); else rescore(R1{}, std::false_type{}); }
  else                      { if (r.acc_half) rescore(R2{}, std::true_type{}); else rescore(R2{}, std::false_type{}); }
  profile_end(res, "pq_rescore_kernel");
  hipLaunchKernelGGL(reset_flagged_kernel, dim3((unsigned)r.nq), dim3(256), 0, res.stream, r.qflag, r.nq, r.n_probes, r.k, 0u, r.cand_d,
                     r.cand_i);
  hipLaunchKernelGGL(fallback_items_kernel, dim3(grid * 4), dim3(256), 0, res.stream, r.sorted_pairs, r.pair_off, idx.n_lists, r.probes,
                     r.n_probes, r.qflag, static_cast<work_item*>(r.fb_items), r.counters, 1);
  profile_end(res, "pq_scan_kernel");
  HIP_TRY(hipGetLastError());
}

void pq3_merge(resources& res, const pq3_run& r, float* top_d, uint32_t* top_i)
{
  auto* ov = static_cast<uint4*>(r.overflow);
  hipLaunchKernelGGL(ov_count_kernel, dim3(256), dim3(256), 0, res.stream, ov, r.counters + 1, r.overflow_cap, r.ov_cnt);
  hipLaunchKernelGGL(ov_scan_kernel, dim3(1), dim3(1024), 0, res.stream, r.ov_cnt, r.nq, r.ov_off);
  hipLaunchKernelGGL(ov_fill_kernel, dim3(256), dim3(256), 0, res.stream, ov, r.counters + 1, r.overflow_cap, r.ov_off, r.ov_cnt,
                     ov + r.overflow_cap);
  auto go = [&](auto kern) {
    hipLaunchKernelGGL(kern, dim3(grid_blocks(r.nq, 4)), dim3(256), 0, res.stream, r.cand_d, r.cand_i, r.cand_r, r.qcnt, r.qflag, r.nq,
                       r.n_probes, r.k, r.head, top_d, top_i, ov + r.overflow_cap, r.ov_off);
  };
  if (r.k <= 64)       go(pool_merge_kernel<1>);
  else if (r.k <= 128) go(pool_merge_kernel<2>);
  else if (r.k <= 192) go(pool_merge_kernel<3>);
  else                 go(pool_merge_kernel<4>);
}

}

extern "C" __attribute__((visibility("default"))) void cuvsAmdIvfPqUnitOrderHook(uint32_t rows, uint32_t groups, uint32_t unit_rows,
                                                                                 uint32_t n_units, uint32_t xcd, uint32_t t,
                                                                                 int strided, uint32_t out[3])
{
  out[0] = cuvs_amd::unit_cost_key(rows, groups, unit_rows);
  out[1] = cuvs_amd::unit_share_len(n_units, xcd, strided != 0);
  out[2] = cuvs_amd::unit_position(n_units, xcd, t, strided != 0);
}
```

### cuvs_amd/csrc/ivf_pq_scan3.hpp

```cpp
#pragma once
#include "ivf_pq.hpp"

namespace cuvs_amd {

struct pq3_tables {
  const uint32_t* cb16;
  const uint32_t* row_term;
  float sc, cbmax, dmax;
};

constexpr int kPq3Stats = 24;

struct pq3_run {
  int64_t nq;
  uint32_t n_probes, k, head;
  int is_ip, lut_mode , acc_half;
  const uint32_t* sorted_pairs;
  const uint32_t* pair_off;
  const uint32_t* probes;
  const float* rot_queries;
  const float* rescore_queries = nullptr;
  int cosine = 0;
  const uint32_t* query_kth;
  float* cand_d;
  uint32_t* cand_i;
  uint32_t* cand_r;
  uint32_t* qflag;
  uint32_t* qcnt;
  uint32_t* counters;
  void* overflow;
  uint32_t overflow_cap;
  uint32_t* ov_cnt;
  uint32_t* ov_off;
  uint32_t* surv_cnt;
  void* surv;
  uint32_t surv_cap;
  void* units;
  uint32_t* unit_off;
  uint32_t unit_rows;
  int unit_order = 0;
  void* units_ord = nullptr;
  uint32_t* xcd_ticket;
  void* fb_items;
  const uint32_t* filter_bits;
  uint32_t* fail;
  void* bq;
  float* thr;
  int filter_dbg;
  unsigned long long* stats;
  int stage = 0;
  void* pair_norms = nullptr;
  const float* hb_xbuf = nullptr;
  uint32_t hb_ldx = 0;
  const float* hb_thr = nullptr;
  uint32_t head_rows = 0;
};

struct pq3_head {
  const void* items;
  const uint32_t* item_begin;
  const uint32_t* item_end;
  uint32_t* xcd_ticket;
  const uint32_t* sorted_pairs;
  const float* rot_queries;
  float* cand_d;
  uint32_t* cand_i;
  uint32_t* query_kth;
  uint32_t n_probes, k, max_list_len;
  int is_ip, lut_mode, acc_half;
  const uint32_t* filter_bits;
  unsigned long long* stats;
  uint32_t one_shot = 0;
  uint32_t row_limit = 0;
};
int pq3_head_scan(resources& res, const ivf_pq_index& idx, const pq3_head& h);

struct flat3_cache {
  dev_buf<uint4> rows16;
  dev_buf<uint32_t> row_term;
  dev_buf<float> row_term32;
  dev_buf<float> zeros;
  float sc = 1.f, maxres = 0.f, maxnorm = 0.f;
  const void* data_ptr = nullptr;
  int64_t rows = -1, size = -1;
  const void* failed_ptr = nullptr;
  int64_t failed_rows = -1, failed_size = -1;
};
struct flat3_view {
  const uint8_t* data;
  const float* centers;
  const uint32_t* list_offsets;
  const uint32_t* list_sizes;
  const int64_t* indices;
  uint32_t n_lists, dim, n_chunks;
  int64_t padded_rows, size;
  uint32_t max_list_len;
  int elem;
  bool unit_rows = false;
};
bool flat3_supported(uint32_t dim, int k);
bool flat3_wide(uint32_t dim);
bool flat3_tail(resources& res, const flat3_view& v, flat3_cache& cache, const pq3_run& r);
struct flat3_head_bufs {
  float* xbuf; uint32_t ldx;
  float* kth_val; uint32_t* kth_idx;
  float* thr_head;
  void* norms;
  uint32_t* tickets;
};
bool flat3_head_bounds(resources& res, const flat3_view& v, flat3_cache& cache, const pq3_run& r, const flat3_head_bufs& hb);

unsigned pq3_grid(const resources& res);
unsigned pq3_regions(const resources& res);
bool pq3_supported(const ivf_pq_index& idx, int k);
bool pq3_bound_useful(const ivf_pq_index& idx, int k);
size_t pq3_max_units(const ivf_pq_index& idx, int64_t n_pairs, uint32_t* unit_rows, bool filter4);
void pq3_warm(resources& res, const ivf_pq_index& idx, bool filter4);
void pq3_tail(resources& res, const ivf_pq_index& idx, const pq3_run& r);
void pq3_merge(resources& res, const pq3_run& r, float* top_d, uint32_t* top_i);

bool pqw_supported(const ivf_pq_index& idx, int k);
uint32_t pqw_heads(const ivf_pq_index& idx, int k, uint32_t n_probes);
bool pqw_ready(resources& res, const ivf_pq_index& idx);
struct pqw_bufs {
  float* xbuf; uint32_t ldx;
  float* kth_val; uint32_t* kth_idx;
  float* thr_head;
  float* head_c;
  void* norms;
  uint32_t* tickets;
  uint32_t* blk_off;
  uint32_t* bound_tmp;
};
bool pqw_head_bounds(resources& res, const ivf_pq_index& idx, const pq3_run& r, const pqw_bufs& hb);
void pqw_tail(resources& res, const ivf_pq_index& idx, const pq3_run& r, const pqw_bufs& hb);

}
```

### cuvs_amd/csrc/ivf_pq_search.hip

```cpp
#include "ivf_pq.hpp"
#include "ops.hpp"
#include "device_utils.hpp"
#include "ivf_common.hpp"
#include "ivf_lists.hpp"
#include "pq_lut_math.hpp"
#include "ivf_pq_scan3.hpp"

#include <cuvs/neighbors/ivf_pq.h>

#include <cfloat>
#include <cstdlib>
#include <functional>
#include <mutex>
#include <type_traits>

namespace cuvs_amd {
extern unsigned long long g_pq3_last_stats[6];

namespace {

constexpr int kScanThreads = 1024;
constexpr int kScanWaves   = kScanThreads / 64;
constexpr int kQueueRows   = 320;

// ... 1617 lines not shown
                             cc_new.data(), n_el, (int64_t)idx.dim_ext, (int64_t)idx.dim);
          hipLaunchKernelGGL(round_to_half_kernel, dim3(nblk(idx.n_lists, 256)), dim3(256), 0, res.stream,
                             idx.center_norms.data(), ct_new.data(), (int64_t)idx.n_lists, (int64_t)1, (int64_t)1);
        } else {
          hipLaunchKernelGGL(scale_to_int8_kernel, dim3(nblk(n_el, 256)), dim3(256), 0, res.stream, idx.centers.data(),
                             cc_new.data(), n_el, (int64_t)idx.dim_ext, (int64_t)idx.dim);
          const int m = (int)(round_up((int64_t)idx.dim + 2, 16) - idx.dim);
          hipLaunchKernelGGL(int8_norm_term_kernel, dim3(nblk(idx.n_lists, 256)), dim3(256), 0, res.stream,
                             idx.center_norms.data(), (int)idx.n_lists, m, !ip, ct_new.data());
        }
        sync(res);
        ct = std::move(ct_new);
        cc = std::move(cc_new);
      }
    }
    const int64_t nqe = nq * idx.dim;
    if (half_t) hipLaunchKernelGGL(round_to_half_kernel, dim3(nblk(nqe, 256)), dim3(256), 0, res.stream, qf, qc, nqe, (int64_t)idx.dim, (int64_t)idx.dim);
    else        hipLaunchKernelGGL(scale_to_int8_kernel, dim3(nblk(nqe, 256)), dim3(256), 0, res.stream, qf, qc, nqe, (int64_t)idx.dim, (int64_t)idx.dim);
    const float* term = (half_t && ip) ? nullptr : ct.data();
    if (res.tune.coarse_lowp != 0) {
      const size_t row_b = (size_t)coarse_lowp_ksteps(!half_t, idx.dim) * 32;
      dev_buf<uint32_t>& cp = half_t ? idx.coarse_pack_h : idx.coarse_pack_i8;
      {
        std::lock_guard<std::mutex> lock(g_coarse_cache_mu);
        if (cp.data() == nullptr) {
          auto cp_new = dev_buf<uint32_t>::persistent((size_t)idx.n_lists * row_b / 4);
          coarse_lowp_pack(res, !half_t, idx.centers.data(), idx.n_lists, idx.dim_ext, idx.dim, cp_new.data());
          sync(res);
          cp = std::move(cp_new);
        }
      }
      dev_buf<uint32_t> qp(res, (size_t)nq * row_b / 4);
      coarse_lowp_pack(res, !half_t, qf, nq, idx.dim, idx.dim, qp.data());
      coarse_lowp_distances(res, !half_t, qp.data(), nq, cp.data(), idx.n_lists, idx.dim, term, ip ? -1.0f : -2.0f, dist.data(),
                            idx.n_lists);
    } else {
      pairwise_distance<float, float>(res, qc, nq, idx.dim, cc.data(), idx.n_lists, idx.dim, idx.dim, nullptr, nullptr,
                                      M_InnerProduct, dist.data(), idx.n_lists);
      hipLaunchKernelGGL(coarse_finish_kernel, dim3(nblk(nq * idx.n_lists, 256)), dim3(256), 0, res.stream, dist.data(), nq,
                         (int)idx.n_lists, term, ip ? -1.0f : -2.0f, half_t);
    }
    select_k<uint32_t, uint32_t>(res, dist.data(), nullptr, nq, idx.n_lists, idx.n_lists, (int)n_probes, pd.data(),
                                 probes, true);
    return;
  }
  dev_buf<float> qn(res, ip ? 0 : nq), dist;
  coarse_search(res, idx.centers.data(), idx.dim_ext, idx.n_lists, idx.dim, idx.center_norms.data(), nullptr,
                ip ? (int)M_InnerProduct : (int)M_L2Expanded, qf, nq, n_probes, nq, qn.data(), dist, pd.data(), probes);
}

__global__ void scale_kernel(float* __restrict__ x, int64_t n, float a)
{
  const int64_t i = (int64_t)blockIdx.x * blockDim.x + threadIdx.x;
  if (i < n) x[i] *= a;
}
void rotate_queries(resources& res, const ivf_pq_index& idx, const float* qf, const float* qc, int64_t nq, int coarse_dtype,
                    float* rot_q)
{
  if (coarse_dtype == 0) {
    pairwise_distance<float, float>(res, qf, nq, idx.dim, idx.rotation.data(), idx.rot_dim, idx.dim, idx.dim, nullptr,
                                    nullptr, M_InnerProduct, rot_q, idx.rot_dim);
    return;
  }
  const bool half_t  = coarse_dtype == 2;
  dev_buf<float>& rr = half_t ? idx.coarse_rot_h : idx.coarse_rot_i8;
  const int64_t n_el = (int64_t)idx.rot_dim * idx.dim;
  {
    std::lock_guard<std::mutex> lock(g_coarse_cache_mu);
    if (rr.data() == nullptr) {
      auto rr_new = dev_buf<float>::persistent((size_t)n_el);
      if (half_t) hipLaunchKernelGGL(round_to_half_kernel, dim3(nblk(n_el, 256)), dim3(256), 0, res.stream, idx.rotation.data(), rr_new.data(), n_el, (int64_t)idx.dim, (int64_t)idx.dim);
      else        hipLaunchKernelGGL(scale_to_int8_kernel, dim3(nblk(n_el, 256)), dim3(256), 0, res.stream, idx.rotation.data(), rr_new.data(), n_el, (int64_t)idx.dim, (int64_t)idx.dim);
      sync(res);
      rr = std::move(rr_new);
    }
  }
  pairwise_distance<float, float>(res, qc, nq, idx.dim, rr.data(), idx.rot_dim, idx.dim, idx.dim, nullptr, nullptr,
                                  M_InnerProduct, rot_q, idx.rot_dim);
  if (!half_t) hipLaunchKernelGGL(scale_kernel, dim3(nblk(nq * idx.rot_dim, 256)), dim3(256), 0, res.stream, rot_q, nq * idx.rot_dim, 1.0f / 128.0f / 128.0f);
}

__global__ void head_items_kernel(const uint32_t* __restrict__ probes, int64_t nq, uint32_t n_probes, uint32_t shard_world,
                                  uint32_t shard_rank, const int32_t* __restrict__ owner, work_item* __restrict__ items,
                                  uint32_t* __restrict__ pairs, uint32_t* __restrict__ n_items)
{
  const int64_t q = (int64_t)blockIdx.x * blockDim.x + threadIdx.x;
  if (q == 0) *n_items = (uint32_t)nq;
  if (q >= nq) return;
  const uint32_t L = probes[q * n_probes];
  const bool mine  = shard_world <= 1 || (owner != nullptr ? (uint32_t)owner[L] == shard_rank : L % shard_world == shard_rank);
  items[q] = work_item{L, (uint32_t)q, mine ? 1u : 0u, 0u};
  pairs[q] = (uint32_t)(q * n_probes);
}

__global__ void init_head_rows_kernel(float* __restrict__ cand_d, uint32_t* __restrict__ cand_i, int64_t nq, int64_t row_len, uint32_t seg)
{
  const int64_t t = (int64_t)blockIdx.x * blockDim.x + threadIdx.x;
  if (t >= nq * (int64_t)seg) return;
  const int64_t o = (t / seg) * row_len + t % seg;
  cand_d[o] = FLT_MAX;
  cand_i[o] = 0xffffffffu;
}

__global__ void postprocess_kernel(const uint32_t* __restrict__ pos, const float* __restrict__ d_in, int64_t n,
                                   const int64_t* __restrict__ indices, int metric, float scale2,
                                   int64_t* __restrict__ neighbors, float* __restrict__ distances)
{
  int64_t i = (int64_t)blockIdx.x * blockDim.x + threadIdx.x;
  if (i >= n) return;
  uint32_t p   = pos[i];
  neighbors[i] = p == 0xffffffffu ? INT64_MAX : indices[p];
  float d      = d_in[i];
  if (p == 0xffffffffu) {
    d = FLT_MAX;
  } else if (metric == M_InnerProduct) {
    d = -d * scale2;
  } else if (metric == M_CosineExpanded) {
    d = 1.0f + d;
  } else if (metric == M_L2SqrtExpanded || metric == M_L2SqrtUnexpanded) {
    d = sqrtf(d * scale2);
  } else {
    d = d * scale2;
  }
  distances[i] = d;
}

}

static void shard_exchange_stats(resources& res, const ivf_pq_index& idx)
{
  static std::mutex mu;
  std::lock_guard<std::mutex> lock(mu);
  if (idx.shard_stats_valid) return;
  uint64_t rows = 0;
  uint32_t lists = 0;
  for (uint32_t v : idx.h_list_sizes) { rows += v; lists += v != 0u; }
  const size_t world = (size_t)std::max(1, idx.shard_world);
  std::vector<uint32_t> h(3 * world, 0u);
  h[3 * idx.shard_rank + 0] = (uint32_t)rows; h[3 * idx.shard_rank + 1] = (uint32_t)(rows >> 32); h[3 * idx.shard_rank + 2] = lists;
  dev_buf<uint32_t> d(res, h.size());
  copy_async(res, d.data(), h.data(), h.size() * sizeof(uint32_t));
  sync(res);
  shard_allgather_inplace_u32(res, idx.shard_comm, d.data(), 3);
  h = to_host(res, d.data(), h.size());
  idx.shard_global_rows = 0; idx.shard_global_lists = 0;
  for (size_t r = 0; r < world; ++r) {
    idx.shard_global_rows += (uint64_t)h[3 * r] | ((uint64_t)h[3 * r + 1] << 32);
    idx.shard_global_lists += h[3 * r + 2];
  }
  idx.shard_stats_valid = true;
}

namespace {

enum class pq_path : int {
  lut_one_phase    = 0,
  lut_two_phase    = 1,
  scan2_tail       = 2,
  matrix_core_tail = 3,
  wide             = 4,
  all_scores       = 5,
};

struct pq_search_plan {
  pq_path path      = pq_path::lut_one_phase;
  uint32_t n_probes = 0;
  bool lut_fp8 = false, acc_half = false, lut_half = false, bits8 = false;
  bool glut         = false;
  bool head1        = false;
  bool overlap      = false;
  bool big_k        = false;
// ... 225 lines not shown
{
  std::vector<unsigned long long> hw(stats.n);
  HIP_TRY(hipMemcpyAsync(hw.data(), stats.data(), stats.bytes(), hipMemcpyDeviceToHost, res.stream));
  HIP_TRY(hipStreamSynchronize(res.stream));
  unsigned long long h[ST_COUNT] = {};
  for (size_t i = 0; i < hw.size(); ++i) h[i % ST_COUNT] += hw[i];
  const double w = 1.0 / (16.0 * grid);
  if (dbg & 4096) {
    for (int which : {(int)ST_SCAN, (int)ST_ALIVE2, (int)ST_F_GATHER, (int)ST_F_FLUSH, (int)ST_STAGE2, (int)ST_CAND, (int)ST_S2_CALLS}) {
      fprintf(stderr, "[pq_scan per-wave stat %d, Mcycles]", which);
      for (int wv = 0; wv < kScanWaves; ++wv) {
        unsigned long long t = 0;
        for (unsigned b = 0; b < grid; ++b) t += hw[((size_t)b * kScanWaves + wv) * ST_COUNT + which];
        fprintf(stderr, " %.2f", (double)t / grid * 1e-6);
      }
      fprintf(stderr, "\n");
    }
  }
  fprintf(stderr,
          "[pq_scan stats] items %llu rows %llu queued %llu (%.2f%%) stage2 calls %llu alive after chunk1/2/3 %llu/%llu/%llu"
          " | cycles per wave: header %.3g lut %.3g scan %.3g (stage2 %.3g) merge+sync %.3g\n",
          h[ST_ITEMS], h[ST_ROWS], h[ST_QUEUED], 100.0 * h[ST_QUEUED] / (double)std::max<unsigned long long>(1, h[ST_ROWS]),
          h[ST_S2_CALLS], h[ST_ALIVE1], h[ST_ALIVE2], h[ST_ALIVE3], h[ST_HEADER] * w, h[ST_LUT] * w, h[ST_SCAN] * w,
          h[ST_STAGE2] * w, (double)(h[ST_MERGE] - h[ST_HEADER] - h[ST_LUT] - h[ST_SCAN]) * w);
  fprintf(stderr, "[pq_scan2 waits, cycles per wave] after filter LUT %.3g, after filter pass %.3g, before LUT B %.3g, after exact LUT "
          "%.3g, after exact pass %.3g, merge %.3g | filter pass: code-load wait %.3g, gather block %.3g, flush %.3g\n",
          h[ST_ALIVE1] * w, h[ST_ALIVE2] * w, h[ST_S2_CALLS] * w, h[ST_ALIVE3] * w, h[ST_CAND] * w, h[ST_MERGE] * w,
          h[ST_F_LOAD] * w, h[ST_F_GATHER] * w, h[ST_F_FLUSH] * w);
}

void launch_lut_scan(resources& res, const pq_search_plan& pl, const scan_args& a, bool tail = false)
{
  const unsigned grid = pl.grid;
  if (tail && pl.path == pq_path::scan2_tail) {
    if (!pl.lut_half)      launch_scan2<float, float, 2, 4>(res, a, grid);
    else if (!pl.acc_half) launch_scan2<__half, float, 4, 2>(res, a, grid);
    else                   launch_scan2<__half, __half, 4, 2>(res, a, grid);
    return;
  }
  const size_t smem = pl.smem;
  const bool bits8 = pl.bits8, big_k = pl.big_k;
  if (pl.glut) {
    if (!pl.lut_half)      launch_scan_glut<float, float, 2>(res, a, smem, grid, big_k);
    else if (!pl.acc_half) launch_scan_glut<__half, float, 4>(res, a, smem, grid, big_k);
    else                   launch_scan_glut<__half, __half, 4>(res, a, smem, grid, big_k);
    return;
  }
  if (!pl.lut_half) {
    if (pl.qpb == 2) launch_scan_qpb<float, float, 2>(res, a, smem, grid, bits8, big_k);
    else             launch_scan_qpb<float, float, 1>(res, a, smem, grid, bits8, big_k);
  } else if (!pl.acc_half) {
    if (pl.qpb == 4)      launch_scan_qpb<__half, float, 4>(res, a, smem, grid, bits8, big_k);
    else if (pl.qpb == 2) launch_scan_qpb<__half, float, 2>(res, a, smem, grid, bits8, big_k);
    else                  launch_scan_qpb<__half, float, 1>(res, a, smem, grid, bits8, big_k);
  } else {
    if (pl.qpb == 4)      launch_scan_qpb<__half, __half, 4>(res, a, smem, grid, bits8, big_k);
    else if (pl.qpb == 2) launch_scan_qpb<__half, __half, 2>(res, a, smem, grid, bits8, big_k);
    else                  launch_scan_qpb<__half, __half, 1>(res, a, smem, grid, bits8, big_k);
  }
}

void launch_head_scan(const pq_search_ctx& c, const scan_args& sa)
{
  pq3_head h{};
  h.items = sa.items; h.item_begin = sa.item_begin; h.item_end = sa.item_end; h.xcd_ticket = sa.xcd_ticket;
  h.sorted_pairs = sa.sorted_pairs; h.rot_queries = sa.rot_queries; h.cand_d = sa.out_d; h.cand_i = sa.out_i;
  h.query_kth = sa.query_kth; h.n_probes = c.pl.n_probes; h.k = (uint32_t)c.k; h.max_list_len = c.pl.max_list_len; h.is_ip = sa.is_ip;
  h.lut_mode = c.pl.lut_mode(); h.acc_half = c.pl.acc_half ? 1 : 0; h.filter_bits = c.filter_bits;
  h.one_shot = sa.one_shot; h.row_limit = sa.row_limit;
  dev_buf<unsigned long long> hst(c.res, (sa.dbg & 2048) ? 8 : 0);
  if (sa.dbg & 2048) HIP_TRY(hipMemsetAsync(hst.data(), 0, hst.bytes(), c.res.stream));
  h.stats = hst.data();
  const int wgs_per_cu = pq3_head_scan(c.res, c.idx, h);
  if (sa.dbg & 2048) report_head_stats(c.res, hst.data(), wgs_per_cu);
}

void run_filter_tail(const pq_search_ctx& c, scan_args a, int64_t nq)
{
  resources& res = c.res;
  const pq_search_plan& pl = c.pl;
  pq_search_scratch& s = c.s;
  const int64_t bs = pl.bs_alloc;
  const bool wide = pl.path == pq_path::wide;
  HIP_TRY(hipMemsetAsync(s.qstate.data(), 0, s.qstate.bytes(), res.stream));
  pq3_run r{};
  r.pair_norms = s.pair_norms.data(); r.head_rows = pl.head_rows;
  r.nq = nq; r.n_probes = pl.n_probes; r.k = (uint32_t)c.k; r.head = pl.head; r.is_ip = a.is_ip;
  r.lut_mode = pl.lut_mode(); r.acc_half = pl.acc_half ? 1 : 0;
  r.sorted_pairs = s.sorted_pairs.data(); r.pair_off = s.pair_off.data(); r.probes = s.probes.data();
  r.rot_queries = s.rot_q.data(); r.query_kth = s.query_kth.data();
  r.cand_d = s.cand_d.data(); r.cand_i = s.cand_i.data(); r.cand_r = s.cand_r.data();
  r.qflag = s.qstate.data(); r.qcnt = s.qstate.data() + bs; r.counters = s.qstate.data() + 2 * bs;
  r.surv_cnt = s.qstate.data() + 2 * bs + 2;
  r.ov_cnt = s.qstate.data() + 2 * bs + 4 + pq3_regions(res); r.ov_off = r.ov_cnt + bs;
  r.surv = s.surv.data(); r.surv_cap = pl.surv_cap; r.units = s.units3.data(); r.unit_off = s.unit_off.data();
  r.unit_rows = pl.unit_rows; r.xcd_ticket = s.tickets.data() + 2 * 8 * 32; r.fb_items = s.fb_items.data();
  r.filter_bits = c.filter_bits; r.overflow = s.overflow3.data(); r.overflow_cap = pl.overflow_cap;
  r.bq = (pl.filter4 || wide) ? s.bq3.data() : nullptr; r.thr = s.thr3.data();
  if (res.tune.pq_unit_order != 0 && !wide) {
    r.unit_order = res.tune.pq_unit_order;
    r.units_ord  = s.units3.data() + 2 * pl.max_units;
  }
  dev_buf<unsigned long long> st3(res, (a.dbg & 1024) ? kPq3Stats : 0);
  if (a.dbg & 1024) {
    HIP_TRY(hipMemsetAsync(st3.data(), 0, st3.bytes(), res.stream));
    HIP_TRY(hipMemsetAsync(st3.data() + 16, 0xff, sizeof(unsigned long long), res.stream));
  }
  r.stats = st3.data(); r.filter_dbg = (a.dbg >> 16) & 255;
  if (pl.overlap) {
    r.stage = 1;
    pq3_tail(c.gres, c.idx, r);
    HIP_TRY(hipEventRecord(res.aux_events[1], c.gres.stream));
    HIP_TRY(hipStreamWaitEvent(res.stream, res.aux_events[1], 0));
    c.fork_guard.armed = false;
    r.stage = 2;
  }
  if (wide) {
    const pqw_bufs hb{s.w_x.data(), pl.w_ldx, s.w_kv.data(), s.w_ki.data(), s.w_thr.data(), s.w_c.data(), s.w_nm.data(),
                      s.tickets.data(), s.w_blk.data(), s.w_bt.data()};
    const bool ok = pqw_head_bounds(res, c.idx, r, hb);
    CUVS_EXPECTS(ok, "ivf_pq: the wide path's decoded rows are gone");
    pqw_tail(res, c.idx, r, hb);
  } else {
    pq3_tail(res, c.idx, r);
  }
  a.items = s.fb_items.data(); a.item_begin = nullptr; a.item_end = r.counters;
  a.xcd_ticket = s.tickets.data() + 3 * 8 * 32;
  if (pl.head1) launch_head_scan(c, a); else launch_lut_scan(res, pl, a);
  pq3_merge(res, r, s.top_d.data(), s.top_i.data());
  if (a.dbg & 1024) report_filter_stats(res, st3.data(), r.counters);
  if ((a.dbg & 1024) && (a.dbg & (1 << 24))) {
    const auto off = to_host(res, r.pair_off + c.idx.n_lists, (size_t)c.idx.n_lists + 1);
    fprintf(stderr, "[pq_units] unit_rows %u\n", pl.unit_rows);
    for (uint32_t L = 0; L < c.idx.n_lists; ++L) fprintf(stderr, "[pq_units] %u %u\n", c.idx.h_list_sizes[L], off[L + 1] - off[L]);
  }
}

void pq_search_batch(const pq_search_ctx& c, const void* queries, elem_t et, int64_t q0, int64_t nq, int64_t* neighbors,
                            float* distances)
{
  resources& res = c.res;
  const ivf_pq_index& idx = c.idx;
  const pq_search_plan& pl = c.pl;
  pq_search_scratch& s = c.s;
  const int k = c.k;
  const uint32_t n_probes = pl.n_probes;
  const int64_t n_pairs = nq * n_probes;
  load_range_as_float(res, queries, et, false , idx.dim, q0, nq, s.qf.data());
  if (idx.metric == M_CosineExpanded) normalize_rows(res, s.qf.data(), nq, idx.dim);
  if (pl.shard_coarse) {
    const int64_t slice = (nq + idx.shard_world - 1) / idx.shard_world;
    const int64_t s0    = std::min<int64_t>(nq, (int64_t)idx.shard_rank * slice);
    const int64_t s1    = std::min<int64_t>(nq, s0 + slice);
    if (s1 > s0)
      select_clusters(res, idx, s.qf.data() + s0 * idx.dim, s1 - s0, n_probes,
                      s.probes.data() + (size_t)idx.shard_rank * slice * n_probes, 0, s.qc.data());
    shard_allgather_inplace_u32(res, idx.shard_comm, s.probes.data(), (size_t)slice * n_probes);
  } else {
    select_clusters(res, idx, s.qf.data(), nq, n_probes, s.probes.data(), c.p.coarse_search_dtype, s.qc.data());
  }
  rotate_queries(res, idx, s.qf.data(), s.qc.data(), nq, c.p.coarse_search_dtype, s.rot_q.data());
  if (c.p.coarse_search_dtype != 0 && idx.metric == M_CosineExpanded) normalize_rows(res, s.rot_q.data(), nq, idx.rot_dim);
  const uint32_t* labels = s.probes.data();
  if (pl.overlap) {
    pq3_warm(res, idx, true);
    HIP_TRY(hipEventRecord(res.aux_events[0], res.stream));
    HIP_TRY(hipStreamWaitEvent(c.gres.stream, res.aux_events[0], 0));
    c.fork_guard.armed = true;
  }
  if (pl.head > 0 || idx.shard_world > 1) {
    hipLaunchKernelGGL(phase_labels_kernel, dim3(nblk(n_pairs, 256)), dim3(256), 0, c.gres.stream, s.probes.data(),
                       n_pairs, n_probes, pl.head, idx.n_lists, s.phase_labels.data(), (uint32_t)idx.shard_world,
                       (uint32_t)idx.shard_rank, pl.n_ranges, idx.list_owner.data(), pl.head_rows != 0u);
    labels = s.phase_labels.data();
  }
  build_work_items(c.gres, labels, n_pairs, pl.n_labels, pl.head1 ? 1 : pl.qpb, s.sorted_pairs.data(), s.pair_off.data(),
                   s.item_off.data(), s.items.data(), (int)idx.n_lists, pl.path == pq_path::scan2_tail ? 8 : pl.qpb,
                   pl.overlap ? s.group_scratch.data() : nullptr,
                   pl.n_ranges , n_probes, nq);
  if (pl.overlap)
    hipLaunchKernelGGL(head_items_kernel, dim3(nblk(nq, 256)), dim3(256), 0, res.stream, s.probes.data(), nq, n_probes,
                       (uint32_t)idx.shard_world, (uint32_t)idx.shard_rank, idx.list_owner.data(), s.hitems.data(), s.hpairs.data(),
                       s.hpairs.data() + pl.bs_alloc);
  HIP_TRY(hipMemsetAsync(s.query_kth.data(), 0xff, (size_t)nq * sizeof(uint32_t), res.stream));
  HIP_TRY(hipMemsetAsync(s.tickets.data(), 0, s.tickets.bytes(), res.stream));
  const size_t scores_ld = pl.largest_total;
  if (pl.mc_tail()) {
    hipLaunchKernelGGL(init_head_rows_kernel, dim3(nblk(nq * (int64_t)pl.head * k, 256)), dim3(256), 0, res.stream, s.cand_d.data(),
                       s.cand_i.data(), nq, (int64_t)n_probes * k, (uint32_t)(pl.head * k));
  } else if (!pl.all_scores()) {
    HIP_TRY(hipMemsetD32Async(reinterpret_cast<hipDeviceptr_t>(s.cand_d.data()), 0x7f7fffff, (size_t)n_pairs * k, res.stream));
    HIP_TRY(hipMemsetAsync(s.cand_i.data(), 0xff, (size_t)n_pairs * k * sizeof(uint32_t), res.stream));
  } else {
    HIP_TRY(hipMemsetD32Async(reinterpret_cast<hipDeviceptr_t>(s.cand_d.data()), 0x7f7fffff, (size_t)nq * scores_ld, res.stream));
    HIP_TRY(hipMemsetAsync(s.cand_i.data(), 0xff, (size_t)nq * scores_ld * sizeof(uint32_t), res.stream));
    hipLaunchKernelGGL(pair_segments_kernel, dim3(nblk(nq, 256)), dim3(256), 0, res.stream, s.probes.data(),
                       idx.list_sizes.data(), nq, n_probes, s.pair_seg.data());
  }
  scan_args a;
  a.query_kth = s.query_kth.data();
  a.items = s.items.data(); a.sorted_pairs = s.sorted_pairs.data(); a.n_lists = idx.n_lists;
  a.rot_queries = s.rot_q.data(); a.centers_rot = idx.centers_rot.data(); a.pq_centers = idx.pq_centers.data();
  a.per_cluster = idx.codebook_kind == 1;
  a.codes = idx.codes.data(); a.list_offsets = idx.list_offsets.data(); a.list_sizes = idx.list_sizes.data();
  a.out_d = s.cand_d.data(); a.out_i = s.cand_i.data();
  a.all_scores = pl.all_scores() ? s.cand_d.data() : nullptr; a.all_rows = s.cand_i.data(); a.pair_seg = s.pair_seg.data();
  a.scores_ld = scores_ld;
  a.n_probes = n_probes; a.rot_dim = idx.rot_dim; a.pq_dim = idx.pq_dim; a.pq_len = idx.pq_len;
  a.pq_bits = idx.pq_bits; a.n_chunks = idx.n_chunks; a.cpc = idx.codes_per_chunk; a.k = (uint32_t)pl.k_scan;
  a.is_ip = idx.metric == M_InnerProduct || idx.metric == M_CosineExpanded;
  a.lut_fp8 = pl.lut_fp8 ? 1 : 0;
  a.dbg   = res.tune.scan_debug;
  a.qcap  = (uint32_t)std::max(0, res.tune.pq_qcap);
  a.filter_bits = c.filter_bits; a.indices = idx.indices.data();
  a.stats = s.stats.data();
  if (a.dbg & (128 | 512)) HIP_TRY(hipMemsetAsync(s.stats.data(), 0, s.stats.bytes(), res.stream));
  a.global_lut_stride = pl.glut_stride;
  a.global_lut = pl.glut ? s.glut_buf.data() : nullptr;
  a.xcd_ticket = s.tickets.data();
  a.item_begin = nullptr; a.item_end = s.item_off.data() + idx.n_lists;
  if (pl.head > 0) {
    if (pl.path == pq_path::wide) {
    } else if (pl.overlap) {
      scan_args ah = a;
      ah.items = s.hitems.data(); ah.sorted_pairs = s.hpairs.data(); ah.item_end = s.hpairs.data() + pl.bs_alloc;
      ah.one_shot = (uint32_t)nq;
      ah.row_limit = pl.head_rows;
      launch_head_scan(c, ah);
    } else if (pl.head1) launch_head_scan(c, a); else launch_lut_scan(res, pl, a);
    if (idx.shard_comm != nullptr) shard_allreduce_min_u32(res, idx.shard_comm, s.query_kth.data(), (size_t)nq);
    a.xcd_ticket = s.tickets.data() + 8 * 32;
    a.item_begin = s.item_off.data() + idx.n_lists;  a.item_end = s.item_off.data() + 2 * idx.n_lists;
    if (pl.mc_tail()) run_filter_tail(c, a, nq);
    else              launch_lut_scan(res, pl, a, true);
  } else {
    launch_lut_scan(res, pl, a);
  }
  if (a.dbg & (128 | 512)) report_scan_stats(res, s.stats, pl.grid, a.dbg);
  if (!pl.mc_tail()) {
    const int64_t row = pl.all_scores() ? (int64_t)scores_ld : (int64_t)n_probes * k;
    select_k<uint32_t, uint32_t>(res, s.cand_d.data(), s.cand_i.data(), nq, row, row, k, s.top_d.data(), s.top_i.data(), true);
  }
  const float sc = ivf_pq_index::scale(et);
  hipLaunchKernelGGL(postprocess_kernel, dim3(nblk(nq * k, 256)), dim3(256), 0, res.stream, s.top_i.data(),
                     s.top_d.data(), nq * k, idx.indices.data(), idx.metric, sc * sc, neighbors + q0 * k,
                     distances + q0 * k);
}

}

void ivf_pq_search(resources& res, const ivf_pq_search_params& p, const ivf_pq_index& idx, const void* queries,
                   elem_t et, int64_t n_queries, int k, int64_t* neighbors, float* distances, const uint32_t* filter_bits)
{
  CUVS_EXPECTS(k > 0, "parameter `k` in top-k must be positive.");
  CUVS_EXPECTS((int64_t)k <= idx.size || idx.shard_world > 1,
               "parameter `k` (%d) in top-k must not be larger that the total size of the index (%ld)", k,
               (long)idx.size);
  CUVS_EXPECTS(p.n_probes > 0, "n_probes (number of clusters to probe in the search) must be positive.");
  CUVS_EXPECTS(p.internal_distance_dtype == 0 || p.internal_distance_dtype == 2,
               "internal_distance_dtype must be either CUDA_R_16F or CUDA_R_32F");
  CUVS_EXPECTS(p.lut_dtype == 0 || p.lut_dtype == 2 || p.lut_dtype == 8 || p.lut_dtype == 3,
               "lut_dtype must be CUDA_R_16F, CUDA_R_32F, CUDA_R_8U or CUDA_R_8I");
  CUVS_EXPECTS(p.coarse_search_dtype == 0 || p.coarse_search_dtype == 2 || p.coarse_search_dtype == 3,
               "Unsupported coarse_search_dtype (only CUDA_R_32F, CUDA_R_16F, and CUDA_R_8I are supported)");
  CUVS_EXPECTS(!idx.dtype_known || et == idx.dtype, "queries dtype differs from the index dtype");
  if (n_queries == 0) return;
  if (idx.shard_comm != nullptr && !idx.shard_stats_valid) shard_exchange_stats(res, idx);
  const bool large_k   = k > 256;
  size_t largest_total = large_k ? largest_lists_total(idx.h_list_sizes, std::min<uint32_t>(p.n_probes, idx.n_lists)) : 0;
  if (large_k && idx.shard_comm != nullptr) {
    dev_buf<uint32_t> key(res, 1);
    const uint32_t mine = ~(uint32_t)std::min<size_t>(largest_total, 0xfffffffeu);
    copy_async(res, key.data(), &mine, sizeof(mine));
    shard_allreduce_min_u32(res, idx.shard_comm, key.data(), 1);
    largest_total = (size_t)~to_host(res, key.data(), 1)[0];
  }
  const pq_search_plan pl = make_pq_search_plan(idx, p, k, n_queries, res.tune, res.num_cus, res.ivf_batch_limit, largest_total,
                                                [&] { return pqw_ready(res, idx); });
  if (res.tune.scan_debug & 1024)
    fprintf(stderr, "[pq_wide] heads %u (supported %d, matrix-core tail of the narrow shapes %d, probes %u, queries %ld, k %d)\n", pl.wheads,
            (int)pqw_supported(idx, k), (int)(pq3_supported(idx, k) && pq3_bound_useful(idx, k)), pl.n_probes, (long)n_queries, k);
  pq_search_scratch scratch(res, idx, p, pl, k);
  resources aux = res;
  if (pl.overlap) {
    ensure_aux_stream(res);
    aux.aux_stream = res.aux_stream;
    aux.stream     = res.aux_stream;
  }
  aux_fork_guard fork_guard;
  fork_guard.s = pl.overlap ? aux.stream : nullptr;
  const pq_search_ctx c{res, pl.overlap ? aux : res, p, idx, pl, scratch, fork_guard, k, filter_bits};
  for (int64_t q0 = 0; q0 < n_queries; q0 += pl.max_batch)
    pq_search_batch(c, queries, et, q0, std::min(pl.max_batch, n_queries - q0), neighbors, distances);
  HIP_TRY(hipGetLastError());
}

}

extern "C" __attribute__((visibility("default"))) int cuvsAmdIvfPqSearchPlan(
  uint32_t dim, uint32_t rot_dim, uint32_t pq_dim, uint32_t pq_len, uint32_t pq_bits, uint32_t shard_world, int codebook_kind,
  int metric, uint32_t n_lists, const uint32_t* list_sizes, cuvsIvfPqSearchParams_t params, int k, int64_t n_queries, int num_cus,
  uint64_t batch_limit_bytes, int wide_rows_ready, int64_t out[24])
{
  return cuvs_amd::translate_exceptions([=] {
    using namespace cuvs_amd;
    CUVS_EXPECTS(params != nullptr && list_sizes != nullptr && n_lists > 0 && pq_bits >= 4 && pq_bits <= 8, "invalid argument");
    ivf_pq_index idx;
    idx.metric = metric; idx.codebook_kind = codebook_kind; idx.n_lists = n_lists; idx.dim = dim; idx.rot_dim = rot_dim;
    idx.pq_dim = pq_dim; idx.pq_len = pq_len; idx.pq_bits = pq_bits; idx.pq_book = 1u << pq_bits;
    idx.codes_per_chunk = 128 / pq_bits; idx.n_chunks = (uint32_t)ceil_div(pq_dim, idx.codes_per_chunk);
    idx.shard_world = (int)std::max(1u, shard_world);
    idx.h_list_sizes.assign(list_sizes, list_sizes + n_lists);
    for (uint32_t v : idx.h_list_sizes) idx.size += v;
    ivf_pq_search_params sp;
    sp.n_probes = params->n_probes; sp.lut_dtype = (int)params->lut_dtype; sp.internal_distance_dtype = (int)params->internal_distance_dtype;
    sp.coarse_search_dtype = (int)params->coarse_search_dtype; sp.max_internal_batch_size = params->max_internal_batch_size;
    const size_t largest_total = k > 256 ? largest_lists_total(idx.h_list_sizes, std::min<uint32_t>(sp.n_probes, n_lists)) : 0;
    const pq_search_plan pl = make_pq_search_plan(idx, sp, k, n_queries, tuning{}, num_cus, (size_t)batch_limit_bytes, largest_total,
                                                  [=] { return wide_rows_ready != 0; });
    const int64_t v[24] = {(int64_t)pl.path, pl.glut, pl.head1, pl.overlap, pl.big_k, pl.filter4, pl.qpb, (int64_t)pl.smem, pl.k_scan,
                           pl.head, pl.wheads, pl.head_rows, pl.max_list_len, pl.w_ldx, pl.n_ranges, pl.n_labels, pl.max_batch,
                           pl.bs_alloc, pl.surv_cap, pl.overflow_cap, (int64_t)pl.max_units, pl.unit_rows, pl.max_items,
                           pl.shard_coarse};
    std::copy(v, v + 24, out);
  });
}
```

### cuvs_amd/csrc/ivf_rabitq.hip

```cpp
#include "ivf_common.hpp"
#include "ivf_lists.hpp"
#include "ivf_rabitq_host.hpp"

#include <cuvs_amd/ivf_rabitq.h>

#include <cfloat>
#include <map>
#include <mutex>

namespace cuvs_amd {

struct ivf_rabitq_index {
  int metric       = 0;
  uint32_t n_lists = 0, dim = 0;
  uint32_t D = 0, W = 0;
  uint32_t ex = 0;
  uint32_t exb = 0;
  float t = 0.f;
  int64_t size = 0, padded_rows = 0;
  dev_buf<float> centers;
  dev_buf<float> centers_rot;
  dev_buf<float> center_rot_norms;
  dev_buf<float> rotation;
  dev_buf<uint32_t> bits;
// ... 600 lines not shown
    dev_buf<float> cpad(res, (size_t)p.n_lists * D);
    hipLaunchKernelGGL(rbq_pad_rows_kernel, dim3(grid_blocks((int64_t)p.n_lists * D, 256)), dim3(256), 0, res.stream, idx->centers.data(),
                       (int64_t)p.n_lists, (uint32_t)dim, D, cpad.data());
    pairwise_distance<float, float>(res, cpad.data(), p.n_lists, D, idx->rotation.data(), D, D, D, nullptr, nullptr, M_InnerProduct,
                                    idx->centers_rot.data(), D);
    row_norms<float>(res, idx->centers_rot.data(), p.n_lists, D, D, idx->center_rot_norms.data(), false);
    sync(res);
  }

  const int64_t batch = streaming ? std::min<int64_t>(n, p.streaming_batch_size)
                                  : std::min<int64_t>(n, std::max<int64_t>(1024, (int64_t(1) << 26) / D));
  dev_buf<uint32_t> labels(res, n), slot(res, n);
  dev_buf<float> xb(res, (size_t)batch * dim);
  for (int64_t r0 = 0; r0 < n; r0 += batch) {
    const int64_t cnt = std::min(batch, n - r0);
    load_range_as_float(res, data, elem_t::f32, is_host, dim, r0, cnt, xb.data());
    fused_l2_argmin<float>(res, xb.data(), cnt, dim, idx->centers.data(), p.n_lists, dim, center_norms.data(), labels.data() + r0, nullptr);
  }
  {
    dev_buf<uint32_t> perm(res, n), grp_off(res, p.n_lists + 1);
    group_by_label(res, labels.data(), n, p.n_lists, perm.data(), grp_off.data());
    const std::vector<uint32_t> h_off = to_host(res, grp_off.data(), p.n_lists + 1);
    idx->h_list_sizes.resize(p.n_lists);
    idx->h_list_offsets.resize(p.n_lists + 1);
    int64_t total = 0;
    for (uint32_t L = 0; L < p.n_lists; ++L) {
      idx->h_list_sizes[L]   = h_off[L + 1] - h_off[L];
      idx->h_list_offsets[L] = (uint32_t)total;
      total += round_up(idx->h_list_sizes[L], 32);
    }
    idx->h_list_offsets[p.n_lists] = (uint32_t)total;
    idx->padded_rows  = total;
    idx->list_sizes   = dev_buf<uint32_t>::persistent(p.n_lists);
    idx->list_offsets = dev_buf<uint32_t>::persistent(p.n_lists + 1);
    copy_async(res, idx->list_sizes.data(), idx->h_list_sizes.data(), p.n_lists * sizeof(uint32_t));
    copy_async(res, idx->list_offsets.data(), idx->h_list_offsets.data(), (p.n_lists + 1) * sizeof(uint32_t));
    hipLaunchKernelGGL(rbq_slots_kernel, dim3(grid_blocks(n, 256)), dim3(256), 0, res.stream, perm.data(), labels.data(), grp_off.data(),
                       idx->list_offsets.data(), n, slot.data());
    sync(res);
  }
  const size_t rows = (size_t)idx->padded_rows;
  idx->bits      = dev_buf<uint32_t>::persistent(rows * idx->W);
  idx->short_fac = dev_buf<float4>::persistent(rows);
  idx->ex_codes  = dev_buf<uint8_t>::persistent(rows * idx->exb);
  idx->ex_fac    = dev_buf<float2>::persistent(rows);
  idx->ids       = dev_buf<uint32_t>::persistent(rows);
  HIP_TRY(hipMemsetAsync(idx->bits.data(), 0, idx->bits.bytes(), res.stream));
  HIP_TRY(hipMemsetAsync(idx->short_fac.data(), 0, idx->short_fac.bytes(), res.stream));
  if (idx->ex_codes.bytes()) HIP_TRY(hipMemsetAsync(idx->ex_codes.data(), 0, idx->ex_codes.bytes(), res.stream));
  HIP_TRY(hipMemsetAsync(idx->ex_fac.data(), 0, idx->ex_fac.bytes(), res.stream));
  HIP_TRY(hipMemsetAsync(idx->ids.data(), 0xff, idx->ids.bytes(), res.stream));

  {
    dev_buf<float> xpad(res, (size_t)batch * D), xr(res, (size_t)batch * D);
    HIP_TRY(hipFuncSetAttribute(reinterpret_cast<const void*>(rbq_encode_kernel), hipFuncAttributeMaxDynamicSharedMemorySize, (int)(4 * D)));
    for (int64_t r0 = 0; r0 < n; r0 += batch) {
      const int64_t cnt = std::min(batch, n - r0);
      load_range_as_float(res, data, elem_t::f32, is_host, dim, r0, cnt, xb.data());
      hipLaunchKernelGGL(rbq_pad_rows_kernel, dim3(grid_blocks(cnt * D, 256)), dim3(256), 0, res.stream, xb.data(), cnt, (uint32_t)dim, D,
                         xpad.data());
      pairwise_distance<float, float>(res, xpad.data(), cnt, D, idx->rotation.data(), D, D, D, nullptr, nullptr, M_InnerProduct, xr.data(), D);
      rbq_encode_args a{};
      a.xr = xr.data(); a.labels = labels.data() + r0; a.slot = slot.data() + r0; a.centers_rot = idx->centers_rot.data();
      a.cnt = cnt; a.r0 = r0; a.D = D; a.W = idx->W; a.ex = idx->ex; a.exb = idx->exb; a.t = idx->t;
      a.bits = idx->bits.data(); a.short_fac = idx->short_fac.data(); a.ex_codes = idx->ex_codes.data(); a.ex_fac = idx->ex_fac.data();
      a.ids = idx->ids.data();
      hipLaunchKernelGGL(rbq_encode_kernel, dim3(grid_blocks(cnt, 4)), dim3(256), 4 * D, res.stream, a);
      HIP_TRY(hipGetLastError());
      sync(res);
    }
  }
  idx->size = n;
  sync(res);
  return idx;
}

namespace {

void rbq_collect(resources& res, const ivf_rabitq_index& idx, const uint32_t* mask, size_t ldw, const uint32_t* probes, const uint32_t* seg,
                 int64_t nq, uint32_t n_probes, const float* qr, const float* S, const float* pd, dev_buf<uint32_t>& counts, rbq_entries& out)
{
  out.off = dev_buf<uint32_t>(res, nq + 1);
  hipLaunchKernelGGL(rbq_count_kernel, dim3(grid_blocks(nq, 4)), dim3(256), 0, res.stream, mask, nq, ldw, counts.data());
  hipLaunchKernelGGL(pair_scan_kernel, dim3(1), dim3(1024), 0, res.stream, counts.data(), (int)nq, out.off.data());
  HIP_TRY(hipGetLastError());
  out.n = (int64_t)read_word(res, out.off.data() + nq);
  const size_t cap = (size_t)std::max<int64_t>(out.n, 1);
  out.row  = dev_buf<uint32_t>(res, cap);
  out.pair = dev_buf<uint32_t>(res, cap);
  out.id   = dev_buf<uint32_t>(res, cap);
  out.d    = dev_buf<float>(res, cap);
  if (out.n == 0) return;
  hipLaunchKernelGGL(rbq_fill_kernel, dim3(grid_blocks(nq, 4)), dim3(256), 0, res.stream, mask, probes, idx.list_sizes.data(),
                     idx.list_offsets.data(), seg, out.off.data(), nq, n_probes, ldw, out.row.data(), out.pair.data());
  rbq_rescore_args a{};
  a.ent_row = out.row.data(); a.ent_pair = out.pair.data(); a.n_ent = out.n; a.qr = qr; a.S = S; a.pd = pd;
  a.bits = idx.bits.data(); a.short_fac = idx.short_fac.data(); a.ex_codes = idx.ex_codes.data(); a.ex_fac = idx.ex_fac.data();
  a.ids = idx.ids.data(); a.n_probes = n_probes; a.D = idx.D; a.W = idx.W; a.ex = idx.ex; a.exb = idx.exb;
  a.ent_d = out.d.data(); a.ent_id = out.id.data();
  const unsigned grid = (unsigned)std::min<int64_t>((out.n + 3) / 4, 1 << 20);
  profile_begin(res, "rbq_rescore_kernel");
  hipLaunchKernelGGL(rbq_rescore_kernel, dim3(grid), dim3(256), 0, res.stream, a);
  profile_end(res, "rbq_rescore_kernel");
  HIP_TRY(hipGetLastError());
}

}

void ivf_rabitq_search(resources& res, const ivf_rabitq_index& idx, uint32_t n_probes, int mode, const float* queries, int64_t n_queries,
                       int k, int64_t* neighbors, float* distances)
{
  if (k == 0 || n_queries == 0 || n_probes == 0) return;
  CUVS_EXPECTS(k > 0, "ivf_rabitq::search: k must not be negative");
  CUVS_EXPECTS(k <= 1024, "ivf_rabitq::search: k=%d exceeds the maximum 1024", k);
  CUVS_EXPECTS(n_probes <= idx.n_lists, "ivf_rabitq::search: n_probes (%u) must not exceed n_lists (%u)", n_probes, idx.n_lists);
  CUVS_EXPECTS(mode >= CUVS_AMD_IVF_RABITQ_LUT16 && mode <= CUVS_AMD_IVF_RABITQ_QUANT8, "ivf_rabitq::search: unknown mode %d", mode);
  const bool quant  = mode == CUVS_AMD_IVF_RABITQ_QUANT4 || mode == CUVS_AMD_IVF_RABITQ_QUANT8;
  const uint32_t D  = idx.D;
  size_t ldw = 0, ld_rows = 0;
  {
    std::vector<uint32_t> s(idx.h_list_sizes);
    std::partial_sort(s.begin(), s.begin() + n_probes, s.end(), std::greater<uint32_t>());
    for (uint32_t i = 0; i < n_probes; ++i) { ldw += (s[i] + 31) / 32; ld_rows += s[i]; }
    ldw = std::max<size_t>(ldw, 1);
  }
  int64_t max_batch = 1 << 15;
  {
    const int64_t per_q = (int64_t)idx.n_lists * 4 + (int64_t)ldw * 4 + (int64_t)D * 16 + (int64_t)n_probes * 32 + (int64_t)ld_rows * 16 + 64;
    max_batch = std::min(max_batch, std::max<int64_t>(1, (int64_t)res.ivf_batch_limit / per_q));
    max_batch = std::min(max_batch, std::max<int64_t>(1, ((int64_t(1) << 31) - 1) / (int64_t)std::max<size_t>(ld_rows, 1)));
    max_batch = std::min(max_batch, std::max<int64_t>(1, ((int64_t(1) << 32) - 1) / (int64_t)ldw));
    max_batch = balanced_batch(n_queries, max_batch);
  }
  const int64_t bs = std::min<int64_t>(max_batch, n_queries), np_max = bs * n_probes;
  dev_buf<float> qpad(res, (size_t)bs * D), qr(res, (size_t)bs * D), qn(res, bs), dist(res, (size_t)bs * idx.n_lists), pd(res, np_max),
    S(res, bs), w(res, bs), T(res, bs), qlut(res, quant ? 0 : (size_t)bs * D);
  dev_buf<int8_t> qhat(res, quant ? (size_t)bs * D : 0);
  dev_buf<uint32_t> probes(res, np_max), head_len(res, bs), seg(res, np_max), labels(res, np_max), mask(res, (size_t)bs * ldw), counts(res, bs),
    sorted_pairs(res, np_max), pair_off(res, idx.n_lists + 2), item_off(res, idx.n_lists + 2);
  const size_t max_items = (size_t)(np_max / kRbqQPB + idx.n_lists + 2);
  dev_buf<work_item> items(res, max_items);
  dev_buf<unsigned long long> stats(res, 3);
  HIP_TRY(hipMemsetAsync(stats.data(), 0, stats.bytes(), res.stream));
  uint64_t n_survivors = 0;
  const size_t screen_smem = (size_t)kRbqQPB * (D + 16) + 7 * kRbqQPB * 4;
  if (quant)
    HIP_TRY(hipFuncSetAttribute(reinterpret_cast<const void*>(rbq_screen_mfma_kernel), hipFuncAttributeMaxDynamicSharedMemorySize, (int)screen_smem));

  for (int64_t q0 = 0; q0 < n_queries; q0 += max_batch) {
    const int64_t nq = std::min(max_batch, n_queries - q0), n_pairs = nq * n_probes;
    hipLaunchKernelGGL(rbq_pad_rows_kernel, dim3(grid_blocks(nq * D, 256)), dim3(256), 0, res.stream, queries + q0 * idx.dim, nq, idx.dim, D,
                       qpad.data());
    pairwise_distance<float, float>(res, qpad.data(), nq, D, idx.rotation.data(), D, D, D, nullptr, nullptr, M_InnerProduct, qr.data(), D);
    row_norms<float>(res, qr.data(), nq, D, D, qn.data(), false);
    pairwise_distance<float, float>(res, qr.data(), nq, D, idx.centers_rot.data(), idx.n_lists, D, D, qn.data(), idx.center_rot_norms.data(),
                                    M_L2Expanded, dist.data(), idx.n_lists);
    select_k<uint32_t, uint32_t>(res, dist.data(), nullptr, nq, idx.n_lists, idx.n_lists, (int)n_probes, pd.data(), probes.data(), true);
    hipLaunchKernelGGL(rbq_query_prep_kernel, dim3(grid_blocks(nq, 4)), dim3(256), 0, res.stream, qr.data(), nq, D, mode, S.data(), w.data(),
                       qhat.data(), qlut.data());
    hipLaunchKernelGGL(rbq_head_kernel, dim3(grid_blocks(nq, 256)), dim3(256), 0, res.stream, probes.data(), idx.list_sizes.data(), nq, n_probes,
                       (uint32_t)k, idx.n_lists, head_len.data(), seg.data(), labels.data(), stats.data());
    HIP_TRY(hipMemsetAsync(mask.data(), 0, (size_t)nq * ldw * sizeof(uint32_t), res.stream));
    hipLaunchKernelGGL(rbq_head_mask_kernel, dim3(grid_blocks(n_pairs, 256)), dim3(256), 0, res.stream, probes.data(), idx.list_sizes.data(),
                       head_len.data(), seg.data(), n_pairs, n_probes, ldw, mask.data());
    rbq_entries head;
    rbq_collect(res, idx, mask.data(), ldw, probes.data(), seg.data(), nq, n_probes, qr.data(), S.data(), pd.data(), counts, head);
    rbq_select(res, head.off.data(), head.d.data(), head.id.data(), nullptr, nullptr, nullptr, nq, k, T.data(), nullptr, nullptr, 0);
// ... 324 lines not shown
```

Measured before the change: 1.926 million queries/s.

## Fold grouping memsets and unit counting into fewer kernels on the overlap path

```diff
diff --git a/cuvs_amd/csrc/ivf_common.hpp b/cuvs_amd/csrc/ivf_common.hpp
--- a/cuvs_amd/csrc/ivf_common.hpp
+++ b/cuvs_amd/csrc/ivf_common.hpp
@@ -16,25 +16,57 @@
   uint32_t pad;
 };
 
-__global__ __launch_bounds__(1024) void count_items_kernel(const uint32_t* __restrict__ pair_off, int n_lists,
-                                                           int qpb_lo, uint32_t* __restrict__ item_off, int split,
-                                                           int qpb_hi)
+constexpr int kOneWgThreads = 256;
+constexpr int kOneWgPer     = 8;
+
+template <int NT, int PER, typename F, typename G>
+__device__ inline int block_scan_tiles(const int n, int* smem, F value_of, G put)
+{
+  const int tid = (int)threadIdx.x;
+  int v[PER], nv[PER];
+  auto load = [&](const int t0, int* o) {
+#pragma unroll
+    for (int j = 0; j < PER; ++j) {
+      const int i = t0 + tid * PER + j;
+      o[j] = i < n ? value_of(i) : 0;
+    }
+  };
+  int carry = 0;
+  load(0, v);
+  for (int t0 = 0; t0 < n; t0 += NT * PER) {
+#pragma unroll
+    for (int j = 0; j < PER; ++j) nv[j] = 0;
+    if (t0 + NT * PER < n) load(t0 + NT * PER, nv);
+    int s = 0;
+#pragma unroll
+    for (int j = 0; j < PER; ++j) s += v[j];
+    int total;
+    int run = carry + block_exclusive_scan(s, smem, &total);
+#pragma unroll
+    for (int j = 0; j < PER; ++j) {
+      const int i = t0 + tid * PER + j;
+      if (i < n) put(i, run);
+      run += v[j];
+    }
+    carry += total;
+#pragma unroll
+    for (int j = 0; j < PER; ++j) v[j] = nv[j];
+  }
+  return carry;
+}
+
+__global__ __launch_bounds__(kOneWgThreads) void count_items_kernel(const uint32_t* __restrict__ pair_off, int n_lists,
+                                                                   int qpb_lo, uint32_t* __restrict__ item_off, int split,
+                                                                   int qpb_hi)
 {
   __shared__ int smem[17];
-  const int per = (n_lists + 1023) / 1024;
-  const int b = threadIdx.x * per, e = min(n_lists, b + per);
-  auto items_of = [&](int i) {
-    const int qpb = i < split ? qpb_lo : qpb_hi;
-    return ((int)(pair_off[i + 1] - pair_off[i]) + qpb - 1) / qpb;
-  };
-  int s = 0;
-  for (int i = b; i < e; ++i) s += items_of(i);
-  int total;
-  int run = block_exclusive_scan(s, smem, &total);
-  for (int i = b; i < e; ++i) {
-    item_off[i] = (uint32_t)run;
-    run += items_of(i);
-  }
+  const int total = block_scan_tiles<kOneWgThreads, kOneWgPer>(
+    n_lists, smem,
+    [&](int i) {
+      const int qpb = i < split ? qpb_lo : qpb_hi;
+      return ((int)(pair_off[i + 1] - pair_off[i]) + qpb - 1) / qpb;
+    },
+    [&](int i, int run) { item_off[i] = (uint32_t)run; });
   if (threadIdx.x == 0) item_off[n_lists] = (uint32_t)total;
 }
 
@@ -175,21 +207,36 @@
   __syncthreads();
   if (threadIdx.x == 0 && bulk != 0u) atomicAdd(&counts[n_plain], bulk);
 }
-__global__ __launch_bounds__(1024) void pair_scan_kernel(const uint32_t* __restrict__ counts, int n, uint32_t* __restrict__ offsets)
+struct unit_count_spec {
+  const uint32_t* list_sizes = nullptr;
+  uint32_t* unit_off         = nullptr;
+  uint32_t n_lists = 0, unit_rows = 1, group = 1, lbase = 0;
+};
+
+__device__ inline int units_of_list(const uint32_t n_pairs, const uint32_t len, const uint32_t group, const uint32_t unit_rows)
+{
+  return (int)(((n_pairs + group - 1u) / group) * ((len + unit_rows - 1u) / unit_rows));
+}
+
+__global__ __launch_bounds__(kOneWgThreads) void pair_scan_kernel(uint32_t* __restrict__ counts, int n, uint32_t* offsets,
+                                                                 const bool zero, const unit_count_spec u)
 {
   __shared__ int smem[17];
-  const int per = (n + 1023) / 1024;
-  const int b = threadIdx.x * per, e = min(n, b + per);
-  int s = 0;
-  for (int i = b; i < e; ++i) s += (int)counts[i];
-  int total;
-  int run = block_exclusive_scan(s, smem, &total);
-  for (int i = b; i < e; ++i) {
-    const int c = (int)counts[i];
-    offsets[i] = (uint32_t)run;
-    run += c;
-  }
+  const int total = block_scan_tiles<kOneWgThreads, kOneWgPer>(
+    n, smem, [&](int i) { return (int)counts[i]; },
+    [&](int i, int run) {
+      offsets[i] = (uint32_t)run;
+      if (zero) counts[i] = 0u;
+    });
   if (threadIdx.x == 0) offsets[n] = (uint32_t)total;
+  if (u.unit_off == nullptr) return;
+  __syncthreads();
+  const uint32_t* off = offsets;
+  const int n_units = block_scan_tiles<kOneWgThreads, kOneWgPer>(
+    (int)u.n_lists, smem,
+    [&](int i) { return units_of_list(off[u.lbase + i + 1] - off[u.lbase + i], u.list_sizes[i], u.group, u.unit_rows); },
+    [&](int i, int run) { u.unit_off[i] = (uint32_t)run; });
+  if (threadIdx.x == 0) u.unit_off[u.n_lists] = (uint32_t)n_units;
 }
 __global__ void pair_scatter_kernel(const uint32_t* __restrict__ labels, int64_t n, const uint32_t* __restrict__ offsets,
                                     uint32_t* __restrict__ cursor, uint32_t* __restrict__ out, uint32_t n_plain)
@@ -200,89 +247,96 @@
   if (L >= n_plain) return;
   out[offsets[L] + atomicAdd(&cursor[L], 1u)] = (uint32_t)i;
 }
+constexpr uint32_t kBitmapQueries = 1u << 19;
+constexpr uint32_t kSegCapBitmap  = 512;
+constexpr uint32_t kBigBlocks     = 64;
+constexpr uint32_t kBigTile       = 4096;
+
+template <bool BITMAP>
 __global__ __launch_bounds__(256) void sort_segments_kernel(const uint32_t* __restrict__ offsets, uint32_t n_labels,
-                                                            uint32_t* __restrict__ pairs)
-{
-  __shared__ uint32_t seg_all[4][kSegCap];
-  const uint32_t L = blockIdx.x * 4u + (threadIdx.x >> 6);
-  if (L >= n_labels) return;
-  const int lane   = threadIdx.x & 63;
-  const uint32_t b = offsets[L], n = offsets[L + 1] - b;
-  if (n <= 1u || n > (uint32_t)kSegCap) return;
-  uint32_t* seg = seg_all[threadIdx.x >> 6];
-  for (uint32_t i = lane; i < n; i += 64u) seg[i] = pairs[b + i];
-  __builtin_amdgcn_fence(__ATOMIC_ACQ_REL, "wavefront");
-  __builtin_amdgcn_wave_barrier();
-  for (uint32_t i = lane; i < n; i += 64u) {
-    const uint32_t v = seg[i];
-    uint32_t rank = 0u;
-    for (uint32_t j = 0; j < n; ++j) rank += seg[j] < v ? 1u : 0u;
-    pairs[b + rank] = v;
-  }
-}
-constexpr uint32_t kBitmapQueries = 1u << 19;
-
-__global__ __launch_bounds__(1024) void sort_big_segments_kernel(const uint32_t* __restrict__ offsets, uint32_t n_labels,
-                                                                 uint32_t* __restrict__ pairs, uint32_t* __restrict__ tmp,
-                                                                 uint32_t n_probes, uint32_t n_queries)
-{
+                                                            uint32_t* __restrict__ pairs, uint32_t* __restrict__ tmp,
+                                                            uint32_t n_probes, uint32_t n_queries, uint32_t n_small)
+{
+  constexpr uint32_t CAP = BITMAP ? kSegCapBitmap : (uint32_t)kSegCap;
+  constexpr uint32_t NT  = 256u;
+  constexpr uint32_t kTileWords = BITMAP ? 0u : kBigTile;
+  static_assert(4u * CAP >= kTileWords + NT + 1u + 17u, "the long segments' LDS fits the small segments' region");
+  __shared__ __attribute__((aligned(16))) uint32_t stat[4u * CAP];
   extern __shared__ __attribute__((aligned(16))) uint32_t sb_smem[];
-  __shared__ uint32_t big[1024];
-  __shared__ uint32_t n_big;
-  __shared__ int scan_smem[17];
-  const bool bitmap_ok = n_probes != 0u && n_queries <= kBitmapQueries;
+  if (blockIdx.x < n_small) {
+    const uint32_t L = blockIdx.x * 4u + (threadIdx.x >> 6);
+    if (L >= n_labels) return;
+    const uint32_t lane = threadIdx.x & 63u;
+    const uint32_t b = offsets[L], n = offsets[L + 1] - b;
+    if (n <= 1u || n > CAP) return;
+    uint32_t* seg = stat + (threadIdx.x >> 6) * CAP;
+    for (uint32_t i = lane; i < n; i += 64u) seg[i] = pairs[b + i];
+    __builtin_amdgcn_fence(__ATOMIC_ACQ_REL, "wavefront");
+    __builtin_amdgcn_wave_barrier();
+    for (uint32_t i = lane; i < n; i += 64u) {
+      const uint32_t v = seg[i];
+      uint32_t rank = 0u;
+      for (uint32_t j = 0; j < n; ++j) rank += seg[j] < v ? 1u : 0u;
+      pairs[b + rank] = v;
+    }
+    return;
+  }
+  uint32_t* tile  = stat;
+  uint32_t* big   = stat + kTileWords;
+  uint32_t& n_big = stat[kTileWords + NT];
+  int* scan_smem  = reinterpret_cast<int*>(stat + kTileWords + NT + 1u);
   const uint32_t words = (n_queries + 31u) / 32u;
-  const uint32_t per = (n_labels + gridDim.x - 1) / gridDim.x;
-  const uint32_t l0 = blockIdx.x * per, l1 = min(n_labels, l0 + per);
-  for (uint32_t base = l0; base < l1; base += 1024u) {
+  const uint32_t wg = blockIdx.x - n_small, n_wg = gridDim.x - n_small;
+  const uint32_t per = (n_labels + n_wg - 1u) / n_wg;
+  const uint32_t l0 = min(n_labels, wg * per), l1 = min(n_labels, l0 + per);
+  for (uint32_t base = l0; base < l1; base += NT) {
     if (threadIdx.x == 0) n_big = 0u;
     __syncthreads();
     const uint32_t Lc = base + threadIdx.x;
-    if (Lc < l1 && offsets[Lc + 1] - offsets[Lc] > (uint32_t)kSegCap) big[atomicAdd(&n_big, 1u)] = Lc;
+    if (Lc < l1 && offsets[Lc + 1] - offsets[Lc] > CAP) big[atomicAdd(&n_big, 1u)] = Lc;
     __syncthreads();
     const uint32_t nb = n_big;
     for (uint32_t w = 0; w < nb; ++w) {
       const uint32_t L = big[w];
       const uint32_t b = offsets[L], n = offsets[L + 1] - b;
-      if (bitmap_ok) {
+      if constexpr (BITMAP) {
         uint32_t* bits = sb_smem;
         uint32_t* pref = sb_smem + words;
-        for (uint32_t i = threadIdx.x; i < words; i += 1024u) bits[i] = 0u;
+        for (uint32_t i = threadIdx.x; i < words; i += NT) bits[i] = 0u;
         __syncthreads();
-        for (uint32_t i = threadIdx.x; i < n; i += 1024u) {
+        for (uint32_t i = threadIdx.x; i < n; i += NT) {
           const uint32_t q = pairs[b + i] / n_probes;
           atomicOr(&bits[q >> 5], 1u << (q & 31u));
         }
         __syncthreads();
-        const uint32_t run = (words + 1023u) / 1024u, w0 = threadIdx.x * run, w1 = min(words, w0 + run);
+        const uint32_t run = (words + NT - 1u) / NT, w0 = min(words, threadIdx.x * run), w1 = min(words, w0 + run);
         int sum = 0;
         for (uint32_t i = w0; i < w1; ++i) sum += __popc(bits[i]);
         int total;
         int acc = block_exclusive_scan(sum, scan_smem, &total);
         for (uint32_t i = w0; i < w1; ++i) { pref[i] = (uint32_t)acc; acc += __popc(bits[i]); }
         __syncthreads();
-        for (uint32_t i = threadIdx.x; i < n; i += 1024u) {
+        for (uint32_t i = threadIdx.x; i < n; i += NT) {
           const uint32_t p = pairs[b + i], q = p / n_probes;
           tmp[b + pref[q >> 5] + (uint32_t)__popc(bits[q >> 5] & ((1u << (q & 31u)) - 1u))] = p;
         }
       } else {
-        uint32_t* tile = sb_smem;
-        for (uint32_t i0 = 0; i0 < n; i0 += 1024u) {
+        for (uint32_t i0 = 0; i0 < n; i0 += NT) {
           const uint32_t i = i0 + threadIdx.x;
           const uint32_t v = i < n ? pairs[b + i] : 0xffffffffu;
           uint32_t rank = 0u;
-          for (uint32_t t0 = 0; t0 < n; t0 += 4096u) {
+          for (uint32_t t0 = 0; t0 < n; t0 += kBigTile) {
             __syncthreads();
-            for (uint32_t t = threadIdx.x; t < 4096u; t += 1024u) tile[t] = t0 + t < n ? pairs[b + t0 + t] : 0xffffffffu;
+            for (uint32_t t = threadIdx.x; t < kBigTile; t += NT) tile[t] = t0 + t < n ? pairs[b + t0 + t] : 0xffffffffu;
             __syncthreads();
-            const uint32_t m = min(4096u, n - t0);
+            const uint32_t m = min(kBigTile, n - t0);
             for (uint32_t j = 0; j < m; ++j) rank += tile[j] < v ? 1u : 0u;
           }
           if (i < n) tmp[b + rank] = v;
         }
       }
       __syncthreads();
-      for (uint32_t i = threadIdx.x; i < n; i += 1024u) pairs[b + i] = tmp[b + i];
+      for (uint32_t i = threadIdx.x; i < n; i += NT) pairs[b + i] = tmp[b + i];
       __syncthreads();
     }
     __syncthreads();
@@ -290,38 +344,48 @@
 }
 
 inline void group_pairs(resources& res, const uint32_t* labels, int64_t n, uint32_t n_labels, uint32_t* sorted_pairs, uint32_t* pair_off,
-                        uint32_t* cursor, uint32_t* tmp, uint32_t n_sorted, uint32_t n_probes, int64_t n_queries)
+                        uint32_t* cursor, uint32_t* tmp, uint32_t n_sorted, uint32_t n_probes, int64_t n_queries,
+                        const unit_count_spec& units = unit_count_spec{})
 {
   CUVS_EXPECTS(n < (int64_t(1) << 32), "group_pairs: more than 2^32 pairs");
   HIP_TRY(hipMemsetAsync(cursor, 0, (size_t)n_labels * sizeof(uint32_t), res.stream));
   n_sorted = std::min(n_sorted, n_labels);
   CUVS_EXPECTS(n_sorted + 1u >= n_labels, "group_pairs: at most one bulk label");
+  CUVS_EXPECTS(units.unit_off == nullptr || units.lbase + units.n_lists <= n_labels, "group_pairs: unit labels beyond the labels");
   hipLaunchKernelGGL(pair_histogram_kernel, dim3((unsigned)std::min<int64_t>(grid_blocks(n, 256), 2048)), dim3(256), 0, res.stream, labels, n,
                      cursor, n_sorted, n_labels);
-  hipLaunchKernelGGL(pair_scan_kernel, dim3(1), dim3(1024), 0, res.stream, cursor, (int)n_labels, pair_off);
-  HIP_TRY(hipMemsetAsync(cursor, 0, (size_t)n_labels * sizeof(uint32_t), res.stream));
+  hipLaunchKernelGGL(pair_scan_kernel, dim3(1), dim3(kOneWgThreads), 0, res.stream, cursor, (int)n_labels, pair_off, true, units);
   hipLaunchKernelGGL(pair_scatter_kernel, dim3(grid_blocks(n, 256)), dim3(256), 0, res.stream, labels, n, pair_off, cursor, sorted_pairs, n_sorted);
-  hipLaunchKernelGGL(sort_segments_kernel, dim3(grid_blocks(n_sorted, 4)), dim3(256), 0, res.stream, pair_off, n_sorted, sorted_pairs);
-  const bool bitmap   = n_probes != 0u && n_queries <= (int64_t)kBitmapQueries;
-  const size_t sbytes = bitmap ? (size_t)2 * ((n_queries + 31) / 32) * sizeof(uint32_t) : (size_t)4096 * sizeof(uint32_t);
-  HIP_TRY(hipFuncSetAttribute(reinterpret_cast<const void*>(sort_big_segments_kernel), hipFuncAttributeMaxDynamicSharedMemorySize,
-                              (int)std::max<size_t>(sbytes, 16384)));
-  hipLaunchKernelGGL(sort_big_segments_kernel, dim3(64), dim3(1024), std::max<size_t>(sbytes, 16384), res.stream, pair_off, n_sorted,
-                     sorted_pairs, tmp, n_probes, (uint32_t)std::min<int64_t>(n_queries, 0xffffffff));
+  const bool bitmap      = n_probes != 0u && n_queries <= (int64_t)kBitmapQueries;
+  const unsigned n_small = (unsigned)grid_blocks(n_sorted, 4);
+  const uint32_t nq32    = (uint32_t)std::min<int64_t>(n_queries, 0xffffffff);
+  if (bitmap) {
+    const size_t sbytes = (size_t)2 * ((n_queries + 31) / 32) * sizeof(uint32_t);
+    HIP_TRY(hipFuncSetAttribute(reinterpret_cast<const void*>(sort_segments_kernel<true>), hipFuncAttributeMaxDynamicSharedMemorySize,
+                                (int)sbytes));
+    hipLaunchKernelGGL(sort_segments_kernel<true>, dim3(n_small + kBigBlocks), dim3(256), sbytes, res.stream, pair_off, n_sorted,
+                       sorted_pairs, tmp, n_probes, nq32, n_small);
+  } else {
+    hipLaunchKernelGGL(sort_segments_kernel<false>, dim3(n_small + kBigBlocks), dim3(256), 0, res.stream, pair_off, n_sorted,
+                       sorted_pairs, tmp, n_probes, nq32, n_small);
+  }
   HIP_TRY(hipGetLastError());
 }
 
 inline void build_work_items(resources& res, const uint32_t* probes, int64_t n_pairs, uint32_t n_lists, int qpb,
                              uint32_t* sorted_pairs, uint32_t* pair_off, uint32_t* item_off, work_item* items,
                              int split = -1, int qpb_hi = 0, uint32_t* group_scratch = nullptr, uint32_t n_sorted = 0xffffffffu,
-                             uint32_t n_probes = 0, int64_t n_queries = 0)
+                             uint32_t n_probes = 0, int64_t n_queries = 0, const unit_count_spec& units = unit_count_spec{})
 {
   if (split < 0) { split = (int)n_lists; qpb_hi = qpb; }
+  CUVS_EXPECTS(units.unit_off == nullptr || group_scratch != nullptr, "build_work_items: unit offsets come from group_pairs");
   if (group_scratch != nullptr)
-    group_pairs(res, probes, n_pairs, n_lists, sorted_pairs, pair_off, group_scratch, group_scratch + n_lists + 1, n_sorted, n_probes, n_queries);
+    group_pairs(res, probes, n_pairs, n_lists, sorted_pairs, pair_off, group_scratch, group_scratch + n_lists + 1, n_sorted, n_probes, n_queries,
+                units);
   else                          group_by_label(res, probes, n_pairs, n_lists, sorted_pairs, pair_off);
+  if (items == nullptr) return;
   const int n_item_labels = (int)std::min(n_lists, n_sorted);
-  hipLaunchKernelGGL(count_items_kernel, dim3(1), dim3(1024), 0, res.stream, pair_off, n_item_labels, qpb, item_off,
+  hipLaunchKernelGGL(count_items_kernel, dim3(1), dim3(kOneWgThreads), 0, res.stream, pair_off, n_item_labels, qpb, item_off,
                      split, qpb_hi);
   hipLaunchKernelGGL(fill_items_kernel, dim3(grid_blocks(n_item_labels, 256)), dim3(256), 0, res.stream, pair_off,
                      item_off, n_item_labels, qpb, items, split, qpb_hi);
diff --git a/cuvs_amd/csrc/ivf_pq_filter4.hip b/cuvs_amd/csrc/ivf_pq_filter4.hip
--- a/cuvs_amd/csrc/ivf_pq_filter4.hip
+++ b/cuvs_amd/csrc/ivf_pq_filter4.hip
@@ -36,13 +36,16 @@
   const uint32_t w0 = (blockIdx.x * 4u + (threadIdx.x >> 6)) * 32u;
   if (s_base + w0 >= s_end) return;
   const uint32_t d0 = ((16u * (st >> a.lpl) + 8u * h) << a.lpl) + 8u * (st & ((1u << a.lpl) - 1u));
-#pragma unroll 2
+  const uint32_t p_mine = a.sorted_pairs[min(s_base + w0 + (lane & 31u), s_end - 1u)];
+  const uint32_t L_mine = a.probes[p_mine];
+#pragma unroll 4
   for (uint32_t pass = 0; pass < 32u / PPW; ++pass) {
-    const uint32_t s  = s_base + w0 + pass * PPW + lane / LPP;
+    const uint32_t j  = pass * PPW + lane / LPP;
+    const uint32_t s  = s_base + w0 + j;
     const bool pair_ok = s < s_end;
     const bool valid  = pair_ok && slot < 2u * NST;
-    const uint32_t p  = a.sorted_pairs[pair_ok ? s : s_end - 1u];
-    const uint32_t q  = p / a.n_probes, L = a.probes[p];
+    const uint32_t p  = (uint32_t)__shfl((int)p_mine, (int)j, 64);
+    const uint32_t q  = p / a.n_probes, L = (uint32_t)__shfl((int)L_mine, (int)j, 64);
     float rn = 0.f, big = 0.f, qc = 0.f, cn = 0.f;
     if (valid) {
       const float* rq = a.rot_queries + (size_t)q * a.rot_dim + d0;
diff --git a/cuvs_amd/csrc/ivf_pq_scan3.hip b/cuvs_amd/csrc/ivf_pq_scan3.hip
--- a/cuvs_amd/csrc/ivf_pq_scan3.hip
+++ b/cuvs_amd/csrc/ivf_pq_scan3.hip
@@ -109,26 +109,17 @@
 }
 
 
-__global__ __launch_bounds__(1024) void count_units_kernel(const uint32_t* __restrict__ pair_off, uint32_t n_lists,
-                                                           const uint32_t* __restrict__ list_sizes, uint32_t unit_rows,
-                                                           uint32_t* __restrict__ unit_off, uint32_t group, uint32_t lbase)
+__global__ __launch_bounds__(kOneWgThreads) void count_units_kernel(const uint32_t* __restrict__ pair_off, uint32_t n_lists,
+                                                                   const uint32_t* __restrict__ list_sizes, uint32_t unit_rows,
+                                                                   uint32_t* __restrict__ unit_off, uint32_t group, uint32_t lbase)
 {
   __shared__ int smem[17];
-  const uint32_t per = (n_lists + 1023u) / 1024u;
-  const uint32_t b = threadIdx.x * per, e = min(n_lists, b + per);
-  auto units_of = [&](uint32_t i) {
-    const uint32_t np = pair_off[lbase + i + 1] - pair_off[lbase + i];
-    const uint32_t len = list_sizes[i];
-    return (int)(((np + group - 1u) / group) * ((len + unit_rows - 1u) / unit_rows));
-  };
-  int s = 0;
-  for (uint32_t i = b; i < e; ++i) s += units_of(i);
-  int total;
-  int run = block_exclusive_scan(s, smem, &total);
-  for (uint32_t i = b; i < e; ++i) {
-    unit_off[i] = (uint32_t)run;
-    run += units_of(i);
-  }
+  const int total = block_scan_tiles<kOneWgThreads, kOneWgPer>(
+    (int)n_lists, smem,
+    [&](int i) {
+      return units_of_list(pair_off[lbase + i + 1] - pair_off[lbase + i], list_sizes[i], group, unit_rows);
+    },
+    [&](int i, int run) { unit_off[i] = (uint32_t)run; });
   if (threadIdx.x == 0) unit_off[n_lists] = (uint32_t)total;
 }
 
@@ -2009,6 +2000,12 @@
     __syncthreads();
     const work_item item = cur;
     if (item.pad == 0xffffffffu) break;
+    const uint32_t pair = a.sorted_pairs[item.first];
+    if (tid < (int)a.k) {
+      const size_t o = (size_t)pair * a.k + tid;
+      a.out_d[o]     = FLT_MAX;
+      a.out_i[o]     = 0xffffffffu;
+    }
     if (item.count == 0u) continue;
     unsigned long long t_prev = a.stats != nullptr ? __builtin_readcyclecounter() : 0ull;
     auto phase = [&](int which) {
@@ -2020,7 +2017,6 @@
     };
     const uint32_t L        = item.list >= a.n_lists ? item.list - a.n_lists : item.list;
     const uint32_t base_row = a.list_offsets[L], len = a.row_limit != 0u ? min(a.list_sizes[L], a.row_limit) : a.list_sizes[L];
-    const uint32_t pair     = a.sorted_pairs[item.first];
     const uint32_t q        = pair / a.n_probes;
     if (tid < (int)a.rot_dim) {
       const float c = a.centers_rot[(size_t)L * a.rot_dim + tid];
@@ -2566,6 +2562,13 @@
   (void)pq3_prepare(res, idx, filter4);
 }
 
+uint32_t pq3_unit_group(const ivf_pq_index& idx, bool filter4)
+{
+  const int nch = (int)idx.pq_dim / 16;
+  const int nst = nch * (int)idx.pq_len;
+  return filter4 ? (nst <= 8 ? 128u : 64u) : (nch <= 4 ? 64u : 32u);
+}
+
 void pq3_tail(resources& res, const ivf_pq_index& idx, const pq3_run& r)
 {
   const bool f4 = r.bq != nullptr;
@@ -2573,12 +2576,12 @@
   const pq3_tables tb = pq3_prepare(res, idx, f4);
   if (r.stage != 1) profile_begin(res, "pq_scan_kernel");
   const int nch        = (int)idx.pq_dim / 16;
-  const int nst        = nch * (int)idx.pq_len;
-  const uint32_t group = f4 ? (nst <= 8 ? 128u : 64u) : (nch <= 4 ? 64u : 32u);
+  const uint32_t group = pq3_unit_group(idx, f4);
   CUVS_EXPECTS(f4 || (idx.pq_len == 2 && idx.codebook_kind == 0), "ivf_pq: pq_filter_kernel decodes pq_len 2, PER_SUBSPACE only");
   auto* units = static_cast<filter_unit*>(r.units);
   if (r.stage != 2) {
-    hipLaunchKernelGGL(count_units_kernel, dim3(1), dim3(1024), 0, res.stream, r.pair_off, idx.n_lists, idx.list_sizes.data(),
+    if (!r.units_counted)
+      hipLaunchKernelGGL(count_units_kernel, dim3(1), dim3(kOneWgThreads), 0, res.stream, r.pair_off, idx.n_lists, idx.list_sizes.data(),
                        r.unit_rows, r.unit_off, group, idx.n_lists);
     hipLaunchKernelGGL(fill_units_kernel, dim3(grid_blocks(idx.n_lists, 256)), dim3(256), 0, res.stream, r.pair_off, idx.n_lists,
                        idx.list_offsets.data(), idx.list_sizes.data(), r.unit_rows, r.unit_off, units, group, idx.n_lists);
@@ -2728,6 +2731,7 @@
   const int nt = nt512 ? 512 : 1024;
   const size_t smem = head_smem_fixed(idx, h.lut_mode, h.acc_half != 0, nt, (int)h.k);
   CUVS_EXPECTS(smem <= 160 * 1024 - 64, "ivf_pq: the head-phase LUT does not fit the LDS");
+  CUVS_EXPECTS((int)h.k <= nt, "ivf_pq: a thread of the head kernel writes one slot of the candidate row");
   a.cap_rows = (uint32_t)(kHeadRowsPerThread * nt);
   if (h.max_list_len > 0) a.cap_rows = std::min<uint32_t>(a.cap_rows, (uint32_t)round_up(h.max_list_len, 64));
   a.one_shot          = h.one_shot;
@@ -2847,7 +2851,7 @@
   l.is_ip = 0; l.nch = (int)v.dim / 32; l.pl = 2; l.n_pairs = r.nq; l.flat = 1; l.head_labels = 1; l.stage = 1; l.pair_norms = hb.norms;
   pq4_filter(res, l);
   auto* units = static_cast<filter_unit*>(r.units);
-  hipLaunchKernelGGL(count_units_kernel, dim3(1), dim3(1024), 0, res.stream, r.pair_off, v.n_lists, v.list_sizes, r.unit_rows, r.unit_off,
+  hipLaunchKernelGGL(count_units_kernel, dim3(1), dim3(kOneWgThreads), 0, res.stream, r.pair_off, v.n_lists, v.list_sizes, r.unit_rows, r.unit_off,
                      256u, 0u);
   hipLaunchKernelGGL(fill_units_kernel, dim3(grid_blocks(v.n_lists, 256)), dim3(256), 0, res.stream, r.pair_off, v.n_lists, v.list_offsets,
                      v.list_sizes, r.unit_rows, r.unit_off, units, 256u, 0u);
@@ -2899,7 +2903,7 @@
   CUVS_EXPECTS(!wide || r.bq != nullptr, "ivf_flat: the wide filter needs the pre-pass buffers");
   const uint32_t group = wide ? pqw_group() : f2 ? 256u : (nch <= 4 ? 64u : 32u);
   auto* units = static_cast<filter_unit*>(r.units);
-  hipLaunchKernelGGL(count_units_kernel, dim3(1), dim3(1024), 0, res.stream, r.pair_off, v.n_lists, v.list_sizes, r.unit_rows, r.unit_off,
+  hipLaunchKernelGGL(count_units_kernel, dim3(1), dim3(kOneWgThreads), 0, res.stream, r.pair_off, v.n_lists, v.list_sizes, r.unit_rows, r.unit_off,
                      group, v.n_lists);
   hipLaunchKernelGGL(fill_units_kernel, dim3(grid_blocks(v.n_lists, 256)), dim3(256), 0, res.stream, r.pair_off, v.n_lists, v.list_offsets,
                      v.list_sizes, r.unit_rows, r.unit_off, units, group, v.n_lists);
@@ -3086,7 +3090,7 @@
   l.cbmax = tb.cbmax; l.dmax = tb.dmax; l.bound_max = bound_max; l.head = 1; l.n_pairs = r.nq * (int64_t)r.head; l.blk_off = hb.blk_off; l.is_ip = r.is_ip;
   pqw_bprep(res, l);
   auto* units = static_cast<filter_unit*>(r.units);
-  hipLaunchKernelGGL(count_units_kernel, dim3(1), dim3(1024), 0, res.stream, r.pair_off, idx.n_lists, idx.list_sizes.data(), r.unit_rows,
+  hipLaunchKernelGGL(count_units_kernel, dim3(1), dim3(kOneWgThreads), 0, res.stream, r.pair_off, idx.n_lists, idx.list_sizes.data(), r.unit_rows,
                      r.unit_off, pqw_group(), 0u);
   hipLaunchKernelGGL(fill_units_kernel, dim3(grid_blocks(idx.n_lists, 256)), dim3(256), 0, res.stream, r.pair_off, idx.n_lists,
                      idx.list_offsets.data(), idx.list_sizes.data(), r.unit_rows, r.unit_off, units, pqw_group(), 0u);
@@ -3156,7 +3160,7 @@
   pqw_bprep(res, l);
   profile_end(res, "pq_bprep_kernel");
   auto* units = static_cast<filter_unit*>(r.units);
-  hipLaunchKernelGGL(count_units_kernel, dim3(1), dim3(1024), 0, res.stream, r.pair_off, idx.n_lists, idx.list_sizes.data(), r.unit_rows,
+  hipLaunchKernelGGL(count_units_kernel, dim3(1), dim3(kOneWgThreads), 0, res.stream, r.pair_off, idx.n_lists, idx.list_sizes.data(), r.unit_rows,
                      r.unit_off, pqw_group(), idx.n_lists);
   hipLaunchKernelGGL(fill_units_kernel, dim3(grid_blocks(idx.n_lists, 256)), dim3(256), 0, res.stream, r.pair_off, idx.n_lists,
                      idx.list_offsets.data(), idx.list_sizes.data(), r.unit_rows, r.unit_off, units, pqw_group(), idx.n_lists);
diff --git a/cuvs_amd/csrc/ivf_pq_scan3.hpp b/cuvs_amd/csrc/ivf_pq_scan3.hpp
--- a/cuvs_amd/csrc/ivf_pq_scan3.hpp
+++ b/cuvs_amd/csrc/ivf_pq_scan3.hpp
@@ -38,6 +38,7 @@
   void* units;
   uint32_t* unit_off;
   uint32_t unit_rows;
+  bool units_counted = false;
   int unit_order = 0;
   void* units_ord = nullptr;
   uint32_t* xcd_ticket;
@@ -74,6 +75,7 @@
   uint32_t row_limit = 0;
 };
 int pq3_head_scan(resources& res, const ivf_pq_index& idx, const pq3_head& h);
+uint32_t pq3_unit_group(const ivf_pq_index& idx, bool filter4);
 
 struct flat3_cache {
   dev_buf<uint4> rows16;
diff --git a/cuvs_amd/csrc/ivf_pq_search.hip b/cuvs_amd/csrc/ivf_pq_search.hip
--- a/cuvs_amd/csrc/ivf_pq_search.hip
+++ b/cuvs_amd/csrc/ivf_pq_search.hip
@@ -1723,11 +1723,15 @@
 
 __global__ void head_items_kernel(const uint32_t* __restrict__ probes, int64_t nq, uint32_t n_probes, uint32_t shard_world,
                                   uint32_t shard_rank, const int32_t* __restrict__ owner, work_item* __restrict__ items,
-                                  uint32_t* __restrict__ pairs, uint32_t* __restrict__ n_items)
+                                  uint32_t* __restrict__ pairs, uint32_t* __restrict__ n_items, uint32_t* __restrict__ query_kth,
+                                  uint32_t* __restrict__ tickets, uint32_t n_tickets, uint32_t* __restrict__ qstate, uint32_t n_qstate)
 {
   const int64_t q = (int64_t)blockIdx.x * blockDim.x + threadIdx.x;
   if (q == 0) *n_items = (uint32_t)nq;
+  if (q < (int64_t)n_tickets) tickets[q] = 0u;
+  if (q < (int64_t)n_qstate) qstate[q] = 0u;
   if (q >= nq) return;
+  query_kth[q] = 0xffffffffu;
   const uint32_t L = probes[q * n_probes];
   const bool mine  = shard_world <= 1 || (owner != nullptr ? (uint32_t)owner[L] == shard_rank : L % shard_world == shard_rank);
   items[q] = work_item{L, (uint32_t)q, mine ? 1u : 0u, 0u};
@@ -2119,8 +2123,9 @@
   pq_search_scratch& s = c.s;
   const int64_t bs = pl.bs_alloc;
   const bool wide = pl.path == pq_path::wide;
-  HIP_TRY(hipMemsetAsync(s.qstate.data(), 0, s.qstate.bytes(), res.stream));
+  if (!pl.overlap) HIP_TRY(hipMemsetAsync(s.qstate.data(), 0, s.qstate.bytes(), res.stream));
   pq3_run r{};
+  r.units_counted = pl.overlap;
   r.pair_norms = s.pair_norms.data(); r.head_rows = pl.head_rows;
   r.nq = nq; r.n_probes = pl.n_probes; r.k = (uint32_t)c.k; r.head = pl.head; r.is_ip = a.is_ip;
   r.lut_mode = pl.lut_mode(); r.acc_half = pl.acc_half ? 1 : 0;
@@ -2147,8 +2152,10 @@
   if (pl.overlap) {
     r.stage = 1;
     pq3_tail(c.gres, c.idx, r);
-    HIP_TRY(hipEventRecord(res.aux_events[1], c.gres.stream));
-    HIP_TRY(hipStreamWaitEvent(res.stream, res.aux_events[1], 0));
+    if (c.gres.stream != res.stream) {
+      HIP_TRY(hipEventRecord(res.aux_events[1], c.gres.stream));
+      HIP_TRY(hipStreamWaitEvent(res.stream, res.aux_events[1], 0));
+    }
     c.fork_guard.armed = false;
     r.stage = 2;
   }
@@ -2201,9 +2208,11 @@
   const uint32_t* labels = s.probes.data();
   if (pl.overlap) {
     pq3_warm(res, idx, true);
-    HIP_TRY(hipEventRecord(res.aux_events[0], res.stream));
-    HIP_TRY(hipStreamWaitEvent(c.gres.stream, res.aux_events[0], 0));
-    c.fork_guard.armed = true;
+    if (c.gres.stream != res.stream) {
+      HIP_TRY(hipEventRecord(res.aux_events[0], res.stream));
+      HIP_TRY(hipStreamWaitEvent(c.gres.stream, res.aux_events[0], 0));
+      c.fork_guard.armed = true;
+    }
   }
   if (pl.head > 0 || idx.shard_world > 1) {
     hipLaunchKernelGGL(phase_labels_kernel, dim3(nblk(n_pairs, 256)), dim3(256), 0, c.gres.stream, s.probes.data(),
@@ -2211,18 +2220,28 @@
                        (uint32_t)idx.shard_rank, pl.n_ranges, idx.list_owner.data(), pl.head_rows != 0u);
     labels = s.phase_labels.data();
   }
+  unit_count_spec units{};
+  if (pl.overlap) {
+    units.list_sizes = idx.list_sizes.data(); units.unit_off = s.unit_off.data(); units.n_lists = idx.n_lists;
+    units.unit_rows = pl.unit_rows; units.group = pq3_unit_group(idx, pl.filter4); units.lbase = idx.n_lists;
+  }
   build_work_items(c.gres, labels, n_pairs, pl.n_labels, pl.head1 ? 1 : pl.qpb, s.sorted_pairs.data(), s.pair_off.data(),
-                   s.item_off.data(), s.items.data(), (int)idx.n_lists, pl.path == pq_path::scan2_tail ? 8 : pl.qpb,
-                   pl.overlap ? s.group_scratch.data() : nullptr,
-                   pl.n_ranges , n_probes, nq);
-  if (pl.overlap)
-    hipLaunchKernelGGL(head_items_kernel, dim3(nblk(nq, 256)), dim3(256), 0, res.stream, s.probes.data(), nq, n_probes,
-                       (uint32_t)idx.shard_world, (uint32_t)idx.shard_rank, idx.list_owner.data(), s.hitems.data(), s.hpairs.data(),
-                       s.hpairs.data() + pl.bs_alloc);
-  HIP_TRY(hipMemsetAsync(s.query_kth.data(), 0xff, (size_t)nq * sizeof(uint32_t), res.stream));
-  HIP_TRY(hipMemsetAsync(s.tickets.data(), 0, s.tickets.bytes(), res.stream));
+                   s.item_off.data(), pl.overlap ? nullptr : s.items.data(), (int)idx.n_lists,
+                   pl.path == pq_path::scan2_tail ? 8 : pl.qpb, pl.overlap ? s.group_scratch.data() : nullptr,
+                   pl.n_ranges , n_probes, nq, units);
+  if (pl.overlap) {
+    const int64_t n_tickets = (int64_t)s.tickets.size(), n_qstate = (int64_t)s.qstate.size();
+    hipLaunchKernelGGL(head_items_kernel, dim3(nblk(std::max(nq, std::max(n_tickets, n_qstate)), 256)), dim3(256), 0, res.stream,
+                       s.probes.data(), nq, n_probes, (uint32_t)idx.shard_world, (uint32_t)idx.shard_rank, idx.list_owner.data(),
+                       s.hitems.data(), s.hpairs.data(), s.hpairs.data() + pl.bs_alloc, s.query_kth.data(), s.tickets.data(),
+                       (uint32_t)n_tickets, s.qstate.data(), (uint32_t)n_qstate);
+  } else {
+    HIP_TRY(hipMemsetAsync(s.query_kth.data(), 0xff, (size_t)nq * sizeof(uint32_t), res.stream));
+    HIP_TRY(hipMemsetAsync(s.tickets.data(), 0, s.tickets.bytes(), res.stream));
+  }
   const size_t scores_ld = pl.largest_total;
-  if (pl.mc_tail()) {
+  if (pl.overlap) {
+  } else if (pl.mc_tail()) {
     hipLaunchKernelGGL(init_head_rows_kernel, dim3(nblk(nq * (int64_t)pl.head * k, 256)), dim3(256), 0, res.stream, s.cand_d.data(),
                        s.cand_i.data(), nq, (int64_t)n_probes * k, (uint32_t)(pl.head * k));
   } else if (!pl.all_scores()) {
@@ -2319,13 +2338,14 @@
             (int)pqw_supported(idx, k), (int)(pq3_supported(idx, k) && pq3_bound_useful(idx, k)), pl.n_probes, (long)n_queries, k);
   pq_search_scratch scratch(res, idx, p, pl, k);
   resources aux = res;
-  if (pl.overlap) {
+  const bool two_streams = pl.overlap && res.tune.pq_overlap != 2;
+  if (two_streams) {
     ensure_aux_stream(res);
     aux.aux_stream = res.aux_stream;
     aux.stream     = res.aux_stream;
   }
   aux_fork_guard fork_guard;
-  fork_guard.s = pl.overlap ? aux.stream : nullptr;
+  fork_guard.s = two_streams ? aux.stream : nullptr;
   const pq_search_ctx c{res, pl.overlap ? aux : res, p, idx, pl, scratch, fork_guard, k, filter_bits};
   for (int64_t q0 = 0; q0 < n_queries; q0 += pl.max_batch)
     pq_search_batch(c, queries, et, q0, std::min(pl.max_batch, n_queries - q0), neighbors, distances);
diff --git a/cuvs_amd/csrc/ivf_rabitq.hip b/cuvs_amd/csrc/ivf_rabitq.hip
--- a/cuvs_amd/csrc/ivf_rabitq.hip
+++ b/cuvs_amd/csrc/ivf_rabitq.hip
@@ -706,7 +706,8 @@
 {
   out.off = dev_buf<uint32_t>(res, nq + 1);
   hipLaunchKernelGGL(rbq_count_kernel, dim3(grid_blocks(nq, 4)), dim3(256), 0, res.stream, mask, nq, ldw, counts.data());
-  hipLaunchKernelGGL(pair_scan_kernel, dim3(1), dim3(1024), 0, res.stream, counts.data(), (int)nq, out.off.data());
+  hipLaunchKernelGGL(pair_scan_kernel, dim3(1), dim3(kOneWgThreads), 0, res.stream, counts.data(), (int)nq, out.off.data(), false,
+                     unit_count_spec{});
   HIP_TRY(hipGetLastError());
   out.n = (int64_t)read_word(res, out.off.data() + nq);
   const size_t cap = (size_t)std::max<int64_t>(out.n, 1);
```

Measured after the change: 1.943 million queries/s, median of 3. Within noise of the previous version (+0.9%).
